# Kyaw-Thiha/animal-vision

Measured on AMD Instinct MI355X. Metric: megapixels/sec per-frame pipeline, higher is better.
Workload: dtype f16

## Files before the change

animal-vision_amd/_lib.py:

```python
from __future__ import annotations

import ctypes
import os

_HERE = os.path.dirname(os.path.abspath(__file__))
LIB_PATH = os.path.join(_HERE, "libavx.so")

AVX_OK = 0
AVX_ERR_INVALID, AVX_ERR_NO_DEVICE, AVX_ERR_HIP, AVX_ERR_UNSUPPORTED, AVX_ERR_NOMEM = -1, -2, -3, -4, -5
AVX_COLOR_MATRIX, AVX_COLOR_CAT_MERGE = 0, 1
AVX_POST_NONE, AVX_POST_GAUSS, AVX_POST_ROWGAIN, AVX_POST_STREAK = 0, 1, 2, 3
AVX_MAX_KSIZE = 33
AVX_PIX_FMTS = {"yuv420p": 0, "nv12": 1, "yuv422p": 2, "yuv444p": 3, "gray": 4, "yuv420p10le": 5, "yuv422p10le": 6, "yuv444p10le": 7,
                "p010le": 8}
AVX_TRANSFERS = {"pq": 1, "hlg": 2}
AVX_TONEMAPS = {"clip": 0, "mobius": 1}


class AvxError(RuntimeError):
    def __init__(self, code: int, msg: str):
        super().__init__(f"libavx error {code}: {msg}")
        self.code = code


# ... 163 lines not shown

class EwPlane(ctypes.Structure):
    _fields_ = [("ptr", ctypes.c_void_p), ("stride", ctypes.c_int32), ("kind", ctypes.c_int32)]


class EwProgram(ctypes.Structure):

    _fields_ = [
        ("struct_size", ctypes.c_uint32),
        ("H", ctypes.c_int32),
        ("W", ctypes.c_int32),
        ("n_insn", ctypes.c_int32),
        ("insn_host", ctypes.POINTER(EwInsn)),
        ("n_planes", ctypes.c_int32),
        ("planes_host", ctypes.POINTER(EwPlane)),
        ("n_acc", ctypes.c_int32),
        ("acc_host", ctypes.POINTER(ctypes.c_int32)),
        ("scalars_dev", ctypes.c_void_p),
        ("n_scalars", ctypes.c_int32),
    ]


AVX_EW_MAX_INSN, AVX_EW_MAX_PLANES, AVX_EW_MAX_REGS, AVX_EW_MAX_ACC = 384, 24, 32, 16
AVX_EW_MAX_FRAMES = 16
_EW_OPS = ("CONST SCALAR LOAD STORE ADD SUB MUL DIV MIN MAX POW ATAN2 NEG ABS SQRT EXP LOG SIN COS FLOOR CEIL CLIP01 TANH "
           "LT LE GT GE EQ AND OR NOT SELECT ACCMIN ACCMAX ACCSUM").split()
EW = {name: i + 1 for i, name in enumerate(_EW_OPS)}
EW_PLANE = {"f32": 0, "u8": 1, "u8_lut": 2, "col": 3, "row": 4, "u8_enc": 5}
EW_ACC = {"min": 0, "max": 1, "sum": 2, "mean": 3}

AVX_MAP = {"falsecolor": 0, "custom_matrix": 1, "opponent": 2, "uv_purple_yellow": 3, "falsecolor_uv_mixed": 4}

if not os.path.exists(LIB_PATH):
    raise ImportError(
        f"{LIB_PATH} not found: build it with `python -c 'import __graft_entry__ as g; g.build()'` "
        "or `make -C animal-vision_amd/csrc` (hipcc --offload-arch=gfx950). There is no CPU fallback."
    )


def _preload_torch_hip_runtime():
    import importlib.util

    try:
        spec = importlib.util.find_spec("torch")
    except (ImportError, ValueError):
        spec = None
    if spec is None or not spec.submodule_search_locations:
        return
    cand = os.path.join(list(spec.submodule_search_locations)[0], "lib", "libamdhip64.so")
    if os.path.exists(cand):
        try:
            ctypes.CDLL(cand, mode=ctypes.RTLD_GLOBAL)
        except OSError:
            pass


_preload_torch_hip_runtime()
lib = ctypes.CDLL(LIB_PATH)

_vp, _i, _sz = ctypes.c_void_p, ctypes.c_int, ctypes.c_size_t
_SIGS = {
    "avx_abi_version": (_i, []),
    "avx_device_count": (_i, []),
    "avx_init": (_i, [_i, ctypes.POINTER(_vp)]),
    "avx_destroy": (None, [_vp]),
    "avx_last_error": (ctypes.c_char_p, [_vp]),
    "avx_malloc": (_i, [_vp, _sz, ctypes.POINTER(_vp)]),
    "avx_free": (_i, [_vp, _vp]),
    "avx_host_alloc": (_i, [_vp, _sz, ctypes.POINTER(_vp)]),
    "avx_host_free": (_i, [_vp, _vp]),
    "avx_memcpy_h2d": (_i, [_vp, _vp, _vp, _sz, _vp]),
    "avx_memcpy_d2h": (_i, [_vp, _vp, _vp, _sz, _vp]),
    "avx_memcpy_d2d": (_i, [_vp, _vp, _vp, _sz, _vp]),
    "avx_memset": (_i, [_vp, _vp, _i, _sz, _vp]),
    "avx_stream_create": (_i, [_vp, ctypes.POINTER(_vp)]),
    "avx_stream_destroy": (_i, [_vp, _vp]),
    "avx_sync": (_i, [_vp, _vp]),
    "avx_stream_wait": (_i, [_vp, _vp, _vp]),
    "avx_device_sync": (_i, [_vp]),
    "avx_timer_start": (_i, [_vp, _vp]),
    "avx_timer_stop": (_i, [_vp, _vp, ctypes.POINTER(ctypes.c_float)]),
    "avx_dichromat_u8": (_i, [_vp, _vp, _vp, _i, _i, _i, ctypes.POINTER(DichromatDesc), _vp]),
    "avx_dichromat_last_launch": (_i, [_vp, ctypes.POINTER(DichromatLaunchInfo)]),
    "avx_get_table": (_i, [_i, _vp, _sz]),
    "avx_percentile": (_i, [_vp, _vp, _sz, ctypes.c_double, ctypes.POINTER(ctypes.c_double), _vp]),
    "avx_spectral_integrate": (_i, [_vp, _vp, _i, _i, _i, _i, _i, _vp, _i, _vp, _vp, _vp]),
    "avx_plane_stats": (_i, [_vp, _vp, _i, _sz, _i, ctypes.c_float, _vp, _vp]),
    "avx_planes_gaussian_blur": (_i, [_vp, _vp, _vp, _i, _i, _i, _i, _vp, _i, _vp]),
    "avx_planes_gaussian_blur_batch": (_i, [_vp, _vp, _sz, _vp, _sz, _i, _i, _i, _i, _i, _vp, _i, _vp]),
    "avx_streak_planes_f32": (_i, [_vp, _vp, _vp, _i, _i, _vp, _i, _vp]),
    "avx_rgb_to_hsi_lobes": (_i, [_vp, _vp, _i, _i, _i, _i, _vp, ctypes.c_float, _vp, _vp]),
    "avx_honeybee_u8": (_i, [_vp, _vp, _vp, _i, _i, _i, ctypes.POINTER(HoneybeeDesc), _vp, _vp]),
    "avx_catch_planes_up": (_i, [_vp, _vp, _i, _i, _vp, _i, _i, _vp, ctypes.POINTER(ctypes.c_int), _vp]),
    "avx_uv_front_u8": (_i, [_vp, _vp, _i, _i, _i, _vp, _vp, _vp]),
    "avx_uv_front_u8_batch": (_i, [_vp, _vp, _i, _sz, _i, _i, _i, _vp, _sz, _vp, _sz, _vp]),
    "avx_panorama_warp_f32": (_i, [_vp, _vp, _i, _i, _i, _vp, _vp]),
    "avx_band_stack": (_i, [_vp, _vp, _i, _i, ctypes.POINTER(BandStackDesc), _vp, _vp]),
    "avx_band_stack_batch": (_i, [_vp, _vp, _i, _sz, _i, _i, ctypes.POINTER(BandStackDesc), _vp, _sz, _vp]),
    "avx_percentile_dev": (_i, [_vp, _vp, _sz, ctypes.c_double, _vp, _vp]),
    "avx_percentiles_dev": (_i, [_vp, _i, ctypes.POINTER(ctypes.c_void_p), ctypes.POINTER(ctypes.c_size_t), ctypes.POINTER(ctypes.c_double),
                                 ctypes.POINTER(ctypes.c_void_p), _vp]),
    "avx_ew_run": (_i, [_vp, ctypes.POINTER(EwProgram), _vp]),
    "avx_ew_run_batch": (_i, [_vp, ctypes.POINTER(EwProgram), _i, ctypes.POINTER(ctypes.c_size_t), _sz, _vp]),
    "avx_ew_spec_stats": (_i, [ctypes.POINTER(ctypes.c_ulonglong), ctypes.POINTER(ctypes.c_ulonglong)]),
    "avx_mantis_u8": (_i, [_vp, _vp, _vp, _vp, _i, _i, ctypes.POINTER(MantisDesc), _vp]),
    "avx_mantis_u8_batch": (_i, [_vp, _vp, _vp, _vp, _i, _i, _i, ctypes.POINTER(MantisDesc), _vp]),
    "avx_resize_hwc": (_i, [_vp, _vp, _i, _i, _i, _i, _vp, _i, _i, _i, _vp]),
    "avx_binocular_warp_u8": (_i, [_vp, _vp, _i, _i, _vp, _vp, _vp, _vp, _vp, _i, _i, _vp, _vp]),
    "avx_cat_wide_u8": (_i, [_vp, _vp, _vp, _i, _i, _i, ctypes.POINTER(DichromatDesc), _vp, _vp, _vp, _vp, _vp, _vp]),
    "avx_center_zoom_u8": (_i, [_vp, _vp, _vp, _i, _i, _i, _i, _i, _i, _i, _vp]),
    "avx_split_compose_u8": (_i, [_vp, _vp, _vp, _vp, _i, _i, _i, _vp]),
    "avx_draw_label_u8": (_i, [_vp, _vp, _i, _i, ctypes.POINTER(ctypes.c_int), _fp, _i, ctypes.c_float, ctypes.c_float, _i, _vp]),
    "avx_gallery_compose_u8": (_i, [_vp, ctypes.POINTER(GalleryTile), _i, _fp, _i, _i, _i, _i, ctypes.POINTER(ctypes.c_int), _vp, _i, _i, _vp]),
    "avx_wall_max_tiles": (_i, []),
    "avx_wall_layout_create": (_i, [_vp, _i, _i, _i, _i, _i, ctypes.POINTER(ctypes.c_int), ctypes.POINTER(ctypes.c_int), _fp, _i, _i, _i, _i,
                                    ctypes.POINTER(ctypes.c_int), ctypes.POINTER(_vp)]),
    "avx_wall_layout_destroy": (_i, [_vp, _vp]),
    "avx_wall_canvas_size": (_i, [_vp, ctypes.POINTER(_i), ctypes.POINTER(_i)]),
    "avx_wall_layout_info": (_i, [_vp, ctypes.POINTER(_i), ctypes.POINTER(_i), ctypes.POINTER(_i), ctypes.POINTER(_sz)]),
    "avx_wall_compose_u8": (_i, [_vp, _vp, ctypes.POINTER(_vp), _sz, _i, _vp, _sz, _vp]),
    "avx_i420_to_rgb_u8": (_i, [_vp, _vp, _vp, _i, _i, _i, _i, _i, _vp]),
    "avx_rgb_to_i420_u8": (_i, [_vp, _vp, _vp, _i, _i, _i, _i, _i, _vp]),
    "avx_yuv_coefficients": (_i, [_i, _i, ctypes.POINTER(ctypes.c_int), ctypes.POINTER(ctypes.c_int)]),
    "avx_yuv_coefficients_d": (_i, [_i, _i, _i, ctypes.POINTER(ctypes.c_int), ctypes.POINTER(ctypes.c_int)]),
    "avx_yuv_frame_size": (_sz, [_i, _i, _i]),
    "avx_yuv_to_rgb_u8": (_i, [_vp, _i, _vp, _vp, _i, _i, _i, _i, _i, _vp]),
    "avx_rgb_to_yuv_u8": (_i, [_vp, _i, _vp, _vp, _i, _i, _i, _i, _i, _vp]),
    "avx_yuv_hdr_to_rgb_u8": (_i, [_vp, _i, _vp, _vp, _i, _i, _i, _i, _i, _i, ctypes.c_double, ctypes.c_double, _vp]),
    "avx_yuv_to_rgb_scaled_u8": (_i, [_vp, _i, _vp, _vp, _i, _i, _i, _i, _i, _i, _i, _vp]),
    "avx_yuv_hdr_to_rgb_scaled_u8": (_i, [_vp, _i, _vp, _vp, _i, _i, _i, _i, _i, _i, _i, _i, ctypes.c_double, ctypes.c_double, _vp]),
    "avx_frame_metrics_u8": (_i, [_vp, _vp, _vp, _i, _i, _i, _i, _vp, _vp]),
    "avx_plane_metrics": (_i, [_vp, _i, _vp, _i, _vp, _i, _i, _i, _i, _vp, _vp]),
    "avx_frame_metrics_ms_u8": (_i, [_vp, _vp, _vp, _i, _i, _i, _vp, _vp, _vp]),
    "avx_remap_linear_planes": (_i, [_vp, _vp, _i, _i, _i, _vp, _vp, _vp, ctypes.c_float, _vp]),
    "avx_sobel3_plane": (_i, [_vp, _vp, _i, _i, _vp, _vp, _vp]),
    "avx_mst_gram": (_i, [_vp, _vp, _i, _sz, _i, _i, _vp, _vp, _vp, _vp]),
    "avx_mst_qkv_gram": (_i, [_vp, _vp, _vp, _sz, _i, _vp, _vp, _vp, _vp, _vp]),
    "avx_mst_qkv_gram16": (_i, [_vp, _vp, _vp, _sz, _i, _vp, _vp, _vp, _vp, _vp]),
    "avx_mst_ln_gemm_gelu": (_i, [_vp, _vp, _vp, _vp, ctypes.c_float, _vp, _sz, _i, _vp, _vp]),
    "avx_mst_convt2x2": (_i, [_vp, _vp, _vp, _vp, _vp, _i, _i, _i, _i, _vp]),
    "avx_mst_convt2x2_fuse": (_i, [_vp, _vp, _vp, _vp, _vp, _vp, _vp, _i, _i, _i, _i, _vp]),
    "avx_mst_posemb": (_i, [_vp, _vp, _vp, _vp, _vp, _vp, _vp, _i, _i, _i, _i, _vp]),
    "avx_mst_conv3x3_add": (_i, [_vp, _vp, _vp, _vp, _vp, _i, _i, _i, _i, _vp]),
    "avx_mst_attn_pack": (_i, [_vp, _vp, _vp, _vp, _vp, _vp, _i, _vp, _vp]),
    "avx_mst_rowgemm_add": (_i, [_vp, _vp, _vp, _vp, _vp, _vp, _vp, _sz, _i, _vp]),
    "avx_mst_conv_in_u8": (_i, [_vp, _vp, _i, _i, _i, _i, _i, _i, _vp, _vp, _vp]),
    "avx_mst_conv3x3_lds": (_i, [_vp, _vp, _vp, _vp, _vp, _i, _i, _i, _i, _vp]),
    "avx_mst_down4x4": (_i, [_vp, _vp, _vp, _vp, _i, _i, _i, _i, _vp]),
    "avx_mst_conv3x3_lds_gram": (_i, [_vp, _vp, _vp, _vp, _vp, _i, _i, _i, _vp, _vp, _vp, _vp, _vp]),
    "avx_mst_convt2x2_fuse_gram": (_i, [_vp, _vp, _vp, _vp, _vp, _vp, _vp, _i, _i, _i, _vp, _vp, _vp, _vp, _vp]),
    "avx_mst_attn_pack16": (_i, [_vp, _vp, _vp, _vp, _vp, _vp, _i, _vp, _vp]),
    "avx_mst_attn_pack_mx": (_i, [_vp, _vp, _vp, _vp, _vp, _vp, _i, _vp, _vp]),
    "avx_mst_attn_tail_mx": (_i, [_vp, _vp, _vp, _vp, _vp, _vp, _vp, _vp, _i, _i, _i, _i, _vp]),
    "avx_mst_attn_tail": (_i, [_vp, _vp, _vp, _vp, _vp, _vp, _vp, _vp, _i, _i, _i, _i, _vp]),
    "avx_mst_attn_tail_x": (_i, [_vp, _vp, _vp, _vp, _vp, _vp, _vp, _vp, _i, _i, _i, _i, _vp]),
    "avx_mst_ffn_fused": (_i, [_vp, _vp, _vp, _vp, ctypes.c_float, _vp, _vp, _vp, _vp, _i, _i, _i, _i, _vp]),
    "avx_mst_conv3x3_lds_spectral": (_i, [_vp, _vp, _vp, _vp, _i, _i, _i, _fp, _i, _i, _i, _i, _vp, _vp, ctypes.POINTER(ctypes.c_int), _vp]),
    "avx_mst_ffn_fused_mx": (_i, [_vp, _vp, _vp, _vp, ctypes.c_float, _vp, _vp, _vp, _vp, _i, _i, _i, _i, _vp]),
    "avx_mst_gelu_prescale": (ctypes.c_float, []),
    "avx_mst_tile_order": (_i, [_i, _i, _i, _i, _i, ctypes.POINTER(ctypes.c_longlong), _i, ctypes.POINTER(ctypes.c_int)]),
    "avx_mst_dw_gemm_add": (_i, [_vp, _vp, _vp, _vp, _vp, _vp, _i, _i, _i, _i, _vp]),
    "avx_dwconv3x3_nhwc_add": (_i, [_vp, _vp, _vp, _vp, _i, _i, _i, _i, _i, _vp, _vp, _vp]),
    "avx_dwconv3x3_nhwc": (_i, [_vp, _vp, _vp, _vp, _i, _i, _i, _i, _i, _i, _vp]),
    "avx_layernorm_rows": (_i, [_vp, _vp, _vp, _vp, _vp, _i, _sz, _i, ctypes.c_float, _vp]),
    "avx_layernorm_rows_grouped": (_i, [_vp, _vp, _vp, _vp, _vp, _i, _sz, _i, ctypes.c_float, _i, _i, _vp]),
}
for _name, (_res, _args) in _SIGS.items():
    _fn = getattr(lib, _name)
    _fn.restype = _res
    _fn.argtypes = _args

if lib.avx_abi_version() != 1:
    raise ImportError(f"libavx.so ABI {lib.avx_abi_version()} != 1 expected by this package: rebuild")
```

animal-vision_amd/csrc/mst_fused.hip:

```cpp
#include <hip/hip_fp16.h>

#include <cstdio>
#include <cstdlib>
#include <cstring>

#include "avx_internal.h"
#include "mst_common.h"
#include "mst_tile_order.h"

namespace {

typedef float float4_t __attribute__((ext_vector_type(4)));
#ifndef AVX_FFN32_GM2
#define AVX_FFN32_GM2 1
#endif
constexpr int kFT = 512;
constexpr int TS = 16;
constexpr int HS = TS + 2;
#ifndef AVX_FFN_TH
#define AVX_FFN_TH 16
#endif
constexpr int kFfnTH = AVX_FFN_TH;
static_assert(kFfnTH == 14 || kFfnTH == 16, "FeedForward tile rows");
constexpr int kFfnNGRP = (HS * (kFfnTH + 2) + 31) / 32;

__device__ __forceinline__ float16_t mfma16(half8_t a, half8_t b, float16_t c) { return __builtin_amdgcn_mfma_f32_32x32x16_f16(a, b, c, 0, 0, 0); }

struct Tile { int x0, y0; long b; };
__device__ __forceinline__ Tile tile_at(const TileWalk& wk, int side_x, int side_y) { return Tile{wk.xi * side_x, wk.yi * side_y, (long)wk.b}; }
int mst_tile_order() {
    const char* e = getenv("AVX_MST_TILE_ORDER");
    return e && !strcmp(e, "raster") ? AVX_TILE_ORDER_RASTER : AVX_TILE_ORDER_XCD;
}

template <int C, int HPASS, int MINW, bool DWM, bool STAMP = false, int NW = 8>
__global__ __launch_bounds__(64 * NW, MINW) void k_mst_ffn_fused(const __half* __restrict__ x , const float* __restrict__ gamma, const float* __restrict__ beta,
                                                          float eps, const uint4* __restrict__ w1pack , const __half* __restrict__ taps ,
                                                          const uint4* __restrict__ w2pack , __half* __restrict__ out , int B,
                                                          int H, int W, const uint4* __restrict__ dwpack , unsigned long long* __restrict__ stamps , int order ) {
    constexpr int FTH = kFfnTH, HSY = FTH + 2, NHALO = HS * HSY, NGRP = (NHALO + 31) / 32;
    constexpr int HID = 4 * C, NPASS = HID / HPASS, KS1 = C / 16, KS2 = HPASS / 16, NT = C / 32, YPITCH = C * 2 + 16, LNV = C / 16;
    constexpr int HPITCH = HPASS * 2 + 16, RPITCH = (HS * HPITCH + 255) / 256 * 256 , NCT = HPASS / 32;
    static_assert(C == 32 || C == 64 || C == 128, "31-, 62- or 124-channel blocks (stored 32 / 64 / 128 wide)");
    constexpr int NTHR = 64 * NW, NGW = (NGRP + NW - 1) / NW;
    constexpr int NTW = NT / (NW / 8), NOCTW = HPASS / (8 * NW);
    static_assert((NW == 8 || NW == 16) && NT % (NW / 8) == 0 && (!DWM || HPASS % (8 * NW) == 0) && (DWM || NW == 8), "wave split");
    constexpr bool PREFETCH = C <= 64;
    extern __shared__ __align__(16) unsigned char smem[];
    unsigned char* yt = smem;
    unsigned char* ht = yt + (size_t)NGRP * 32 * YPITCH;
    __half* tapl = reinterpret_cast<__half*>(ht + (size_t)HSY * RPITCH);
    float* gl = reinterpret_cast<float*>(tapl + (DWM ? 0 : 9 * HID));
    constexpr bool W2LDS = NW == 16;
    uint4* w2l = reinterpret_cast<uint4*>(gl + 2 * C);
    const int tid = threadIdx.x, lane = tid & 63, wave = tid >> 6, p = lane & 31, h = lane >> 5;
    unsigned long long seg[8] = {0, 0, 0, 0, 0, 0, 0, 0}, tlast = 0;
    auto stamp = [&](int k) {
        if constexpr (STAMP) {
            const unsigned long long now = __builtin_readcyclecounter();
            seg[k] += now - tlast;
            tlast = now;
        }
    };
    if constexpr (STAMP) tlast = __builtin_readcyclecounter();
    if constexpr (!DWM)
        for (int i = tid; i < 9 * HID; i += NTHR) tapl[i] = taps[i];
    for (int i = tid; i < C; i += NTHR) { gl[i] = gamma[i]; gl[C + i] = beta[i]; }
    const int tx = (W + TS - 1) / TS, ty = (H + FTH - 1) / FTH;
    const float cnt = (float)(NT * 31);

    uint4 raw[NGW][LNV];
    unsigned f_rel[NGW];
#pragma unroll
    for (int gi = 0; gi < NGW; ++gi) {
        const int q = 32 * (wave + NW * gi) + p, qq = q < NHALO ? q : NHALO - 1;
        f_rel[gi] = (unsigned)(((qq / HS) * W + qq % HS) * C + h * (C / 2)) * 2u;
    }
    auto fetch = [&](const Tile& t) {
        if (t.y0 >= 1 && t.y0 + HSY - 1 <= H && t.x0 >= 1 && t.x0 + HS - 1 <= W) {
            const char* origin = reinterpret_cast<const char*>(x + ((t.b * H + t.y0 - 1) * (size_t)W + t.x0 - 1) * C);
#pragma unroll
            for (int gi = 0; gi < NGW; ++gi) {
                if (wave + NW * gi >= NGRP) break;
                unsigned o = f_rel[gi];
                asm volatile("" : "+v"(o));
                const uint4* src = reinterpret_cast<const uint4*>(origin + o);
#pragma unroll
                for (int v = 0; v < LNV; ++v) raw[gi][v] = src[v];
            }
            return;
        }
#pragma unroll
        for (int gi = 0; gi < NGW; ++gi) {
            const int g = wave + NW * gi;
            if (g >= NGRP) break;
            const int q = 32 * g + p, qq = q < NHALO ? q : NHALO - 1;
            int yy = t.y0 - 1 + qq / HS, xx = t.x0 - 1 + qq % HS;
            yy = yy < 0 ? 0 : (yy >= H ? H - 1 : yy);
            xx = xx < 0 ? 0 : (xx >= W ? W - 1 : xx);
            const uint4* src = reinterpret_cast<const uint4*>(x + ((t.b * H + yy) * (size_t)W + xx) * C + h * (C / 2));
#pragma unroll
            for (int v = 0; v < LNV; ++v) raw[gi][v] = src[v];
        }
    };
    auto layernorm = [&]() {
        if constexpr (DWM) {
#pragma unroll
            for (int gi = 0; gi < NGW; ++gi) {
                const int g = wave + NW * gi;
                if (g >= NGRP) break;
                typedef _Float16 half2v __attribute__((ext_vector_type(2)));
                constexpr unsigned kOnes = 0x3c003c00u;
                auto is_pad = [&](int i) { return ((h * (C / 2) + i) & 31) == 31; };
                auto word = [&](int i) { const uint4 u = raw[gi][i / 8]; const int k = (i / 2) & 3; return k == 0 ? u.x : k == 1 ? u.y : k == 2 ? u.z : u.w; };
                float s1 = 0.f;
#pragma unroll
                for (int i = 0; i < 8 * LNV; i += 2) s1 = __builtin_amdgcn_fdot2(__builtin_bit_cast(half2v, word(i)), __builtin_bit_cast(half2v, kOnes), s1, false);
                const float mean = (s1 + __shfl_xor(s1, 32)) / cnt, nmean = -mean;
                float d[8 * LNV], s2 = 0.f;
#pragma unroll
                for (int i = 0; i < 8 * LNV; ++i) {
                    const float t = (i & 1) ? fma_mix_hi_c(word(i), kOnes, nmean) : fma_mix_lo_c(word(i), kOnes, nmean);
                    d[i] = is_pad(i) ? 0.f : t;
                    s2 = __builtin_fmaf(d[i], d[i], s2);
                }
                const float rstd = rsqrtf((s2 + __shfl_xor(s2, 32)) / cnt + eps);
                unsigned char* dst = yt + (size_t)(32 * g + p) * YPITCH + h * C;
#pragma unroll
                for (int v = 0; v < LNV; ++v) {
                    unsigned o[4];
#pragma unroll
                    for (int j = 0; j < 8; j += 2) {
                        const int i = 8 * v + j;
                        const float2_t y2 = float2_t{d[i], d[i + 1]} * float2_t{rstd, rstd};
                        const float bq = (h * (C / 2) + i + 1) == 31 ? 1.0f : y2.y;
                        o[j / 2] = pack_f16(y2.x, bq);
                    }
                    *reinterpret_cast<uint4*>(dst + 16 * v) = uint4{o[0], o[1], o[2], o[3]};
                }
            }
            return;
        }
#pragma unroll
        for (int gi = 0; gi < NGW; ++gi) {
            const int g = wave + NW * gi;
            if (g >= NGRP) break;
            constexpr unsigned kOnes = 0x3c003c00u;
            auto is_pad = [&](int i) { return ((h * (C / 2) + i) & 31) == 31; };
            auto word = [&](int i) { const uint4 u = raw[gi][i / 8]; const int k = (i / 2) & 3; return k == 0 ? u.x : k == 1 ? u.y : k == 2 ? u.z : u.w; };
            float s1 = 0.f;
#pragma unroll
            for (int i = 0; i < 8 * LNV; ++i) {
                const float t = (i & 1) ? fma_mix_hi_c(word(i), kOnes, s1) : fma_mix_lo_c(word(i), kOnes, s1);
                s1 = is_pad(i) ? s1 : t;
            }
            const float mean = (s1 + __shfl_xor(s1, 32)) / cnt, nmean = -mean;
            float d[8 * LNV], s2 = 0.f;
#pragma unroll
            for (int i = 0; i < 8 * LNV; ++i) {
                const float t = (i & 1) ? fma_mix_hi_c(word(i), kOnes, nmean) : fma_mix_lo_c(word(i), kOnes, nmean);
                d[i] = is_pad(i) ? 0.f : t;
                s2 = __builtin_fmaf(d[i], d[i], s2);
            }
            const float rstd = rsqrtf((s2 + __shfl_xor(s2, 32)) / cnt + eps);
            unsigned char* dst = yt + (size_t)(32 * g + p) * YPITCH + h * C;
#pragma unroll
            for (int v = 0; v < LNV; ++v) {
                unsigned o[4];
#pragma unroll
                for (int j = 0; j < 8; j += 2) {
                    const int i = 8 * v + j, c = h * (C / 2) + i;
                    const float a = is_pad(i) ? 0.f : __builtin_fmaf(d[i] * rstd, gl[c], gl[C + c]);
                    const float bq = is_pad(i + 1) ? 0.f : __builtin_fmaf(d[i + 1] * rstd, gl[c + 1], gl[C + c + 1]);
                    o[j / 2] = pack_f16(a, bq);
                }
                *reinterpret_cast<uint4*>(dst + 16 * v) = uint4{o[0], o[1], o[2], o[3]};
            }
        }
    };

    const int n0 = (wave / 8) * NTW, w8 = wave % 8;
    half8_t w2f[W2LDS ? 1 : NTW * KS2];
    auto load_w2 = [&](int pass) {
#pragma unroll
        for (int n = 0; n < NTW; ++n)
#pragma unroll
            for (int s = 0; s < KS2; ++s) w2f[n * KS2 + s] = __builtin_bit_cast(half8_t, w2pack[((size_t)(n0 + n) * (HID / 16) + pass * KS2 + s) * 64 + lane]);
    };
    if constexpr (NPASS == 1 && !W2LDS) load_w2(0);
    half8_t w1f[KS1];
    auto load_w1 = [&](int pass) {
#pragma unroll
        for (int s = 0; s < KS1; ++s) w1f[s] = __builtin_bit_cast(half8_t, w1pack[((size_t)(pass * NCT + wave % NCT) * KS1 + s) * 64 + lane]);
    };
    constexpr bool W1AHEAD = DWM && C == 64 && NPASS > 1 && NW == 8;
    if constexpr (W1AHEAD) load_w1(0);
    constexpr int NITEM = (NGRP + NW / NCT - 1) / (NW / NCT);
    int p1_g[NITEM], p1_dst[NITEM], p1_dy[NITEM], p1_dx[NITEM];
#pragma unroll
    for (int j = 0; j < NITEM; ++j) {
        const int g = wave / NCT + j * (NW / NCT), q = 32 * g + p, qc = q < NHALO ? q : 0;
        p1_g[j] = g < NGRP ? g : -1;
        p1_dst[j] = (g < NGRP && q < NHALO) ? (qc / HS) * RPITCH + (qc % HS) * HPITCH + 32 * h : -1;
        p1_dy[j] = qc / HS - 1; p1_dx[j] = qc % HS - 1;
    }
    TileWalk ahead;
    ahead.init(blockIdx.x, gridDim.x, B, ty, tx, order);
    if (!ahead.live) return;
    Tile t = tile_at(ahead, TS, FTH);
    ahead.advance();
    fetch(t);
    __syncthreads();
    layernorm();
    for (;;) {
        const bool halo_inside = t.y0 >= 1 && t.y0 + HSY - 1 <= H && t.x0 >= 1 && t.x0 + HS - 1 <= W;
        float16_t D[NTW];
#pragma unroll
        for (int n = 0; n < NTW; ++n)
#pragma unroll
            for (int v = 0; v < 16; ++v) D[n][v] = 0.f;
#pragma unroll 1
        for (int pass = 0; pass < NPASS; ++pass) {
            stamp(pass == 0 ? 7 : 5);
            __syncthreads();
            stamp(0);
            if constexpr (W2LDS)
                for (int i = tid; i < NT * KS2 * 64; i += NTHR) w2l[i] = w2pack[((size_t)(i / (KS2 * 64)) * (HID / 16) + pass * KS2 + (i / 64) % KS2) * 64 + (i & 63)];
            half8_t af[DWM ? NOCTW : 1][3];
            if constexpr (DWM) {
#pragma unroll
                for (int o2 = 0; o2 < NOCTW; ++o2)
#pragma unroll
                    for (int i = 0; i < 3; ++i) af[o2][i] = __builtin_bit_cast(half8_t, dwpack[((size_t)(pass * (HPASS / 8) + NW * o2 + wave) * 3 + i) * 64 + lane]);
            }
            {
                const int ct = wave % NCT;
                if constexpr (!W1AHEAD) load_w1(pass);
#pragma unroll
                for (int j = 0; j < NITEM; ++j) {
                    if (p1_g[j] < 0) continue;
                    float16_t d;
#pragma unroll
                    for (int v = 0; v < 16; ++v) d[v] = 0.f;
                    const unsigned char* ysrc = yt + (size_t)(32 * p1_g[j] + p) * YPITCH + 16 * h;
#pragma unroll
                    for (int s = 0; s < KS1; ++s) d = mfma16(w1f[s], __builtin_bit_cast(half8_t, *reinterpret_cast<const uint4*>(ysrc + 32 * s)), d);
                    if (p1_dst[j] >= 0) {
                        uint32_t keep = 0xffffffffu;
                        if (!halo_inside) {
                            const int yy = t.y0 + p1_dy[j], xx = t.x0 + p1_dx[j];
                            keep = (yy >= 0 && yy < H && xx >= 0 && xx < W) ? 0xffffffffu : 0u;
                        }
                        constexpr int GP1 = (C == 64 && NW == 8) ? 4 : (C == 32 ? 2 : 1);
                        unsigned pk[8];
#pragma unroll
                        for (int v0 = 0; v0 < 8; v0 += GP1) {
                            float2_t gq[GP1];
#pragma unroll
                            for (int v = 0; v < GP1; ++v) gq[v] = float2_t{d[2 * (v0 + v)], d[2 * (v0 + v) + 1]};
                            if constexpr (DWM) gelu_mx<GP1>(gq); else gelu_multi<GP1>(gq);
#pragma unroll
                            for (int v = 0; v < GP1; ++v) pk[v0 + v] = pack_f16(gq[v].x, gq[v].y);
                        }
                        uint4 u0 = uint4{pk[0], pk[1], pk[2], pk[3]}, u1 = uint4{pk[4], pk[5], pk[6], pk[7]};
                        if (!halo_inside) { u0.x &= keep; u0.y &= keep; u0.z &= keep; u0.w &= keep; u1.x &= keep; u1.y &= keep; u1.z &= keep; u1.w &= keep; }
                        unsigned char* dst = ht + p1_dst[j] + 64 * ct;
                        reinterpret_cast<uint4*>(dst)[0] = u0;
                        reinterpret_cast<uint4*>(dst)[1] = u1;
                    }
                }
            }
            stamp(1);
            __syncthreads();
            stamp(2);
            if (PREFETCH && pass == NPASS - 1 && ahead.live) fetch(tile_at(ahead, TS, FTH));
            if constexpr (NPASS > 1 && !W2LDS) load_w2(pass);
            if constexpr (DWM) {
                constexpr int NOCT = NOCTW;
                const int n16 = lane & 15, q = lane >> 4;
                unsigned char* rbase = ht + (size_t)q * RPITCH + (size_t)n16 * HPITCH + 16 * wave;
                unsigned char* wbase = ht + (size_t)(q >> 1) * RPITCH + (size_t)n16 * HPITCH + 16 * wave + 8 * (q & 1);
                constexpr int NU = NOCT * (FTH / 2);
                uint4 bq[3];
                auto rd = [&](int u) {
                    const int o2 = u / (FTH / 2), pr = u % (FTH / 2);
#pragma unroll
                    for (int i = 0; i < 3; ++i) bq[i] = *reinterpret_cast<const uint4*>(rbase + (size_t)(2 * pr) * RPITCH + (size_t)i * HPITCH + 16 * NW * o2);
                };
                auto finish = [&](int u, float4_t a) {
                    const int o2 = u / (FTH / 2), pr = u % (FTH / 2);
                    float2_t gp[2] = {float2_t{a[0], a[1]}, float2_t{a[2], a[3]}};
                    if constexpr (C == 64 || (C == 32 && AVX_FFN32_GM2)) gelu_mx<2>(gp);
                    else { float2_t g0[1] = {gp[0]}, g1[1] = {gp[1]}; gelu_mx<1>(g0); gelu_mx<1>(g1); gp[0] = g0[0]; gp[1] = g1[0]; }
                    *reinterpret_cast<uint2*>(wbase + (size_t)(2 * pr) * RPITCH + 16 * NW * o2) = uint2{pack_f16(gp[0].x, gp[0].y), pack_f16(gp[1].x, gp[1].y)};
                };
#ifndef AVX_FFN_PIPE_ALL
#define AVX_FFN_PIPE_ALL 0
#endif
                constexpr bool PIPE = C == 64 || AVX_FFN_PIPE_ALL;
                if constexpr (PIPE) {
                    rd(0);
                    float4_t prev = {0.f, 0.f, 0.f, 0.f};
#pragma unroll
                    for (int u = 0; u < NU; ++u) {
                        const int o2 = u / (FTH / 2);
                        float4_t acc = {0.f, 0.f, 0.f, 0.f};
#pragma unroll
                        for (int i = 0; i < 3; ++i) acc = __builtin_amdgcn_mfma_f32_16x16x32_f16(af[o2][i], __builtin_bit_cast(half8_t, bq[i]), acc, 0, 0, 0);
                        if (u + 1 < NU) rd(u + 1);
                        __builtin_amdgcn_sched_barrier(0);
                        if (u > 0) finish(u - 1, prev);
                        __builtin_amdgcn_sched_barrier(0);
                        prev = acc;
                    }
                    finish(NU - 1, prev);
                } else {
#pragma unroll
                    for (int u = 0; u < NU; ++u) {
                        const int o2 = u / (FTH / 2);
                        rd(u);
                        float4_t acc = {0.f, 0.f, 0.f, 0.f};
#pragma unroll
                        for (int i = 0; i < 3; ++i) acc = __builtin_amdgcn_mfma_f32_16x16x32_f16(af[o2][i], __builtin_bit_cast(half8_t, bq[i]), acc, 0, 0, 0);
                        finish(u, acc);
                    }
                }
                stamp(3);
                __syncthreads();
                stamp(4);
                if constexpr (W1AHEAD) load_w1(pass + 1 < NPASS ? pass + 1 : 0);
                const int r = 2 * w8 + (p >> 4), c = p & 15;
                const unsigned char* zb = ht + (size_t)r * RPITCH + (size_t)c * HPITCH + 16 * h;
                if (2 * w8 < FTH) {
#pragma unroll
                for (int s = 0; s < KS2; ++s) {
                    const half8_t bf = __builtin_bit_cast(half8_t, *reinterpret_cast<const uint4*>(zb + 32 * s));
#pragma unroll
                    for (int n = 0; n < NTW; ++n) {
                        if constexpr (W2LDS) D[n] = mfma16(__builtin_bit_cast(half8_t, w2l[((n0 + n) * KS2 + s) * 64 + lane]), bf, D[n]);
                        else D[n] = mfma16(w2f[n * KS2 + s], bf, D[n]);
                    }
                }
                }
            } else
            if (2 * wave < FTH) {
                const int r = 2 * wave + (p >> 4), c = p & 15;
                const unsigned char* hbase = ht + (size_t)r * RPITCH + (size_t)c * HPITCH + 16 * h;
                const unsigned char* tbase = reinterpret_cast<const unsigned char*>(tapl) + (size_t)(pass * HPASS + 8 * h) * 2;
#pragma unroll
                for (int s = 0; s < KS2; ++s) {
                    float acc[8];
#pragma unroll
                    for (int j = 0; j < 8; ++j) acc[j] = 0.f;
#pragma unroll
                    for (int tap = 0; tap < 9; ++tap) {
                        const uint4 hv = *reinterpret_cast<const uint4*>(hbase + (size_t)(tap / 3) * RPITCH + (size_t)(tap % 3) * HPITCH + 32 * s);
                        const uint4 wv = *reinterpret_cast<const uint4*>(tbase + (size_t)tap * HID * 2 + 32 * s);
                        fma_mix_lo(acc[0], hv.x, wv.x); fma_mix_hi(acc[1], hv.x, wv.x);
                        fma_mix_lo(acc[2], hv.y, wv.y); fma_mix_hi(acc[3], hv.y, wv.y);
                        fma_mix_lo(acc[4], hv.z, wv.z); fma_mix_hi(acc[5], hv.z, wv.z);
                        fma_mix_lo(acc[6], hv.w, wv.w); fma_mix_hi(acc[7], hv.w, wv.w);
                    }
                    half8_t bf;
#pragma unroll
                    for (int j = 0; j < 8; j += 2) {
                        const float2_t gv = gelu_fast2(float2_t{acc[j], acc[j + 1]});
                        bf[j] = (_Float16)gv.x;
                        bf[j + 1] = (_Float16)gv.y;
                    }
#pragma unroll
                    for (int n = 0; n < NT; ++n)
                        D[n] = mfma16(w2f[n * KS2 + s], bf, D[n]);
                }
            }
        }
        stamp(5);
        {
            const int yo = t.y0 + 2 * w8 + (p >> 4), xo = t.x0 + (p & 15);
            if (2 * w8 < FTH && yo < H && xo < W) {
                const size_t off = ((t.b * H + yo) * (size_t)W + xo) * C + 16 * h + 32 * n0;
#pragma unroll
                for (int n = 0; n < NTW; ++n) {
                    const uint4 xa = reinterpret_cast<const uint4*>(x + off + 32 * n)[0], xb = reinterpret_cast<const uint4*>(x + off + 32 * n)[1];
                    const unsigned xw[8] = {xa.x, xa.y, xa.z, xa.w, xb.x, xb.y, xb.z, xb.w};
                    unsigned ow[8];
#pragma unroll
                    for (int j = 0; j < 8; ++j) {
                        float s0 = D[n][2 * j], s1 = D[n][2 * j + 1];
                        fma_mix_lo(s0, xw[j], 0x3c003c00u); fma_mix_hi(s1, xw[j], 0x3c003c00u);
                        ow[j] = pack_f16(s0, s1);
                    }
                    reinterpret_cast<uint4*>(out + off + 32 * n)[0] = uint4{ow[0], ow[1], ow[2], ow[3]};
                    reinterpret_cast<uint4*>(out + off + 32 * n)[1] = uint4{ow[4], ow[5], ow[6], ow[7]};
                }
            }
        }
        stamp(6);
        if (!ahead.live) break;
        t = tile_at(ahead, TS, FTH);
        ahead.advance();
        if (!PREFETCH) fetch(t);
        layernorm();
    }
    if constexpr (STAMP) {
        if (lane == 0 && stamps)
#pragma unroll
            for (int k = 0; k < 8; ++k) stamps[((size_t)blockIdx.x * NW + wave) * 8 + k] = seg[k];
    }
}


constexpr int VS = TS + 4, MS = TS + 2;

template <int C, int MINW>
__global__ __launch_bounds__(kFT, MINW) void k_mst_attn_tail(const __half* __restrict__ v , const __half* __restrict__ x ,
                                                             const uint4* __restrict__ mpack , const __half* __restrict__ taps1 ,
                                                             const __half* __restrict__ taps2 , const float* __restrict__ bias ,
                                                             __half* __restrict__ out, int B, int H, int W, const uint4* __restrict__ wvpack ) {
    constexpr int NO = C / 8, NS = C / 16, NT = C / 32, PP = C * 2 + 16;
    constexpr int VRP = (VS * PP + 255) / 256 * 256, MRP = VRP;
    constexpr int NFILL = (VS * VS * NO + kFT - 1) / kFT;
    extern __shared__ __align__(16) unsigned char smem[];
    unsigned char* vt = smem;
    unsigned char* mt = vt + (size_t)VS * VRP;
    const bool fromx = wvpack != nullptr;
    __half* t2l = reinterpret_cast<__half*>(mt + (size_t)VS * VRP);
    __half* t1l = t2l + 9 * C;
    float* bl = reinterpret_cast<float*>(t1l + 9 * C);
    const int tid = threadIdx.x, lane = tid & 63, wave = tid >> 6, p = lane & 31, h = lane >> 5;
    for (int i = tid; i < 9 * C; i += kFT) { t2l[i] = taps2[i]; t1l[i] = taps1[i]; }
    for (int i = tid; i < C; i += kFT) bl[i] = bias ? bias[i] : 0.f;
    const int tx = (W + TS - 1) / TS, ty = (H + TS - 1) / TS;
    const int oct = wave % NO, part = wave / NO, nparts = 8 / NO, per = (MS * MS + nparts - 1) / nparts;
    half8_t mf[NT * NS];
#pragma unroll
    for (int i = 0; i < NT * NS; ++i) mf[i] = __builtin_bit_cast(half8_t, mpack[(size_t)i * 64 + lane]);

    uint4 pre[NFILL];
    int f_lds[NFILL];
    unsigned f_rel[NFILL];
#pragma unroll
    for (int k = 0; k < NFILL; ++k) {
        const int it = tid + k * kFT, itc = it < VS * VS * NO ? it : 0, q = itc / NO, part16 = itc % NO;
        f_lds[k] = it < VS * VS * NO ? (q / VS) * VRP + (q % VS) * PP + 16 * part16 : -1;
        f_rel[k] = (unsigned)(((q / VS) * W + q % VS) * C + 8 * part16) * 2u;
    }
    auto fetch = [&](const Tile& t) {
        const __half* src = fromx ? x : v;
        if (t.y0 >= 2 && t.y0 + VS - 2 <= H && t.x0 >= 2 && t.x0 + VS - 2 <= W) {
            const char* origin = reinterpret_cast<const char*>(src + ((t.b * H + t.y0 - 2) * (size_t)W + t.x0 - 2) * C);
#pragma unroll
            for (int k = 0; k < NFILL; ++k) {
                unsigned o = f_rel[k];
                asm volatile("" : "+v"(o));
                pre[k] = *reinterpret_cast<const uint4*>(origin + o);
            }
            return;
        }
#pragma unroll
        for (int k = 0; k < NFILL; ++k) {
            const int fl = f_lds[k] < 0 ? 0 : f_lds[k], row = fl / VRP, col = (fl - row * VRP) / PP, f_off = (fl - row * VRP - col * PP) / 2;
            const int yy = t.y0 + row - 2, xx = t.x0 + col - 2;
            const bool ok = f_lds[k] >= 0 && yy >= 0 && yy < H && xx >= 0 && xx < W;
            const int yc = yy < 0 ? 0 : (yy >= H ? H - 1 : yy), xc = xx < 0 ? 0 : (xx >= W ? W - 1 : xx);
            uint4 r = *reinterpret_cast<const uint4*>(src + ((t.b * H + yc) * (size_t)W + xc) * C + f_off);
            r.x = ok ? r.x : 0u; r.y = ok ? r.y : 0u; r.z = ok ? r.z : 0u; r.w = ok ? r.w : 0u;
            pre[k] = r;
        }
    };
    auto fill = [&]() {
        unsigned char* dst = fromx ? mt : vt;
#pragma unroll
        for (int k = 0; k < NFILL; ++k)
            if (f_lds[k] >= 0) *reinterpret_cast<uint4*>(dst + f_lds[k]) = pre[k];
    };
    constexpr int NB = (((MS * MS + (8 / NO) - 1) / (8 / NO)) + 63) / 64;
// ... 12 lines not shown
    ahead.advance();
    fetch(t);
    for (;;) {
        fill();
        __syncthreads();
        if (fromx) {
            constexpr int NG = (VS * VS + 31) / 32;
            for (int task = wave; task < NG * NT; task += kFT / 64) {
                const int g = task / NT, nt = task % NT;
                const int q = 32 * g + p, qc = q < VS * VS ? q : VS * VS - 1;
                const int lo = (qc / VS) * VRP + (qc % VS) * PP;
                float16_t d;
#pragma unroll
                for (int vv = 0; vv < 16; ++vv) d[vv] = 0.f;
#pragma unroll
                for (int s2 = 0; s2 < NS; ++s2)
                    d = mfma16(__builtin_bit_cast(half8_t, wvpack[(size_t)(nt * NS + s2) * 64 + lane]),
                               __builtin_bit_cast(half8_t, *reinterpret_cast<const uint4*>(mt + lo + 32 * s2 + 16 * h)), d);
                if (q < VS * VS) {
                    half8_t o0, o1;
#pragma unroll
                    for (int vv = 0; vv < 8; ++vv) { o0[vv] = (_Float16)d[vv]; o1[vv] = (_Float16)d[8 + vv]; }
                    reinterpret_cast<uint4*>(vt + lo + 64 * nt + 32 * h)[0] = __builtin_bit_cast(uint4, o0);
                    reinterpret_cast<uint4*>(vt + lo + 64 * nt + 32 * h)[1] = __builtin_bit_cast(uint4, o1);
                }
            }
            __syncthreads();
        }
        constexpr bool HOIST = C == 64;
        uint4 wt1[HOIST ? 9 : 1];
        if constexpr (HOIST) {
#pragma unroll
            for (int tap = 0; tap < 9; ++tap) wt1[tap] = *reinterpret_cast<const uint4*>(reinterpret_cast<const unsigned char*>(t1l) + (size_t)tap * C * 2 + 16 * oct);
        }
        const bool mid_inside = t.y0 >= 1 && t.y0 + MS - 1 <= H && t.x0 >= 1 && t.x0 + MS - 1 <= W;
#pragma unroll
        for (int i = 0; i < NB; ++i) {
            if (b_src[i] < 0) continue;
            const unsigned char* src = vt + b_src[i];
            float acc[8];
#pragma unroll
            for (int j = 0; j < 8; ++j) acc[j] = 0.f;
#pragma unroll
            for (int tap = 0; tap < 9; ++tap) {
                const uint4 hv = *reinterpret_cast<const uint4*>(src + (tap / 3) * VRP + (tap % 3) * PP);
                const uint4 wv = HOIST ? wt1[HOIST ? tap : 0] : *reinterpret_cast<const uint4*>(reinterpret_cast<const unsigned char*>(t1l) + (size_t)tap * C * 2 + 16 * oct);
                fma_mix_lo(acc[0], hv.x, wv.x); fma_mix_hi(acc[1], hv.x, wv.x);
                fma_mix_lo(acc[2], hv.y, wv.y); fma_mix_hi(acc[3], hv.y, wv.y);
                fma_mix_lo(acc[4], hv.z, wv.z); fma_mix_hi(acc[5], hv.z, wv.z);
                fma_mix_lo(acc[6], hv.w, wv.w); fma_mix_hi(acc[7], hv.w, wv.w);
            }
            bool inside = true;
            if (!mid_inside) {
                const int my = b_src[i] / MRP, mx = (b_src[i] - my * MRP) / PP, yy = t.y0 + my - 1, xx = t.x0 + mx - 1;
                inside = yy >= 0 && yy < H && xx >= 0 && xx < W;
            }
            half8_t o;
#pragma unroll
            for (int j = 0; j < 8; j += 2) {
                const float2_t gv = gelu_fast2(float2_t{acc[j], acc[j + 1]});
                o[j] = (_Float16)gv.x;
                o[j + 1] = (_Float16)gv.y;
            }
            uint4 ov = __builtin_bit_cast(uint4, o);
            if (!mid_inside) {
                const uint32_t keep = inside ? 0xffffffffu : 0u;
                ov.x &= keep; ov.y &= keep; ov.z &= keep; ov.w &= keep;
            }
            *reinterpret_cast<uint4*>(mt + b_src[i]) = ov;
        }
        __syncthreads();
        if (ahead.live) fetch(tile_at(ahead, TS, TS));
        {
            const int r = 2 * wave + (p >> 4), c = p & 15;
            const int yo = t.y0 + r, xo = t.x0 + c;
            const bool live = yo < H && xo < W;
            const size_t off = ((t.b * H + (live ? yo : 0)) * (size_t)W + (live ? xo : 0)) * C + h * (C / 2);
            uint4 xr[2 * NT];
#pragma unroll
            for (int i = 0; i < 2 * NT; ++i) xr[i] = reinterpret_cast<const uint4*>(x + off)[i];
            float16_t D[NT];
#pragma unroll
            for (int n = 0; n < NT; ++n)
#pragma unroll
                for (int vv = 0; vv < 16; ++vv) D[n][vv] = 0.f;
            float pe[NS][8];
            const unsigned char* msrc = mt + (size_t)r * MRP + (size_t)c * PP + (size_t)h * C;
            const unsigned char* vsrc = vt + (size_t)(r + 2) * VRP + (size_t)(c + 2) * PP + (size_t)h * C;
            const unsigned char* tsrc = reinterpret_cast<const unsigned char*>(t2l) + (size_t)h * C;
#pragma unroll
            for (int s = 0; s < NS; ++s) {
#pragma unroll
                for (int j = 0; j < 8; ++j) pe[s][j] = 0.f;
#pragma unroll
                for (int tap = 0; tap < 9; ++tap) {
                    const uint4 hv = *reinterpret_cast<const uint4*>(msrc + (size_t)(tap / 3) * MRP + (size_t)(tap % 3) * PP + 16 * s);
                    const uint4 wv = *reinterpret_cast<const uint4*>(tsrc + (size_t)tap * C * 2 + 16 * s);
                    fma_mix_lo(pe[s][0], hv.x, wv.x); fma_mix_hi(pe[s][1], hv.x, wv.x);
                    fma_mix_lo(pe[s][2], hv.y, wv.y); fma_mix_hi(pe[s][3], hv.y, wv.y);
                    fma_mix_lo(pe[s][4], hv.z, wv.z); fma_mix_hi(pe[s][5], hv.z, wv.z);
                    fma_mix_lo(pe[s][6], hv.w, wv.w); fma_mix_hi(pe[s][7], hv.w, wv.w);
                }
                const half8_t bv = __builtin_bit_cast(half8_t, *reinterpret_cast<const uint4*>(vsrc + 16 * s));
#pragma unroll
                for (int n = 0; n < NT; ++n) D[n] = mfma16(mf[n * NS + s], bv, D[n]);
            }
            if (live) {
#pragma unroll
                for (int n = 0; n < NT; ++n) {
                    const float* bb = bl + h * (C / 2) + 16 * n;
                    constexpr unsigned kOnes = 0x3c003c00u;
                    const uint4 xa = xr[2 * n], xb = xr[2 * n + 1];
                    const unsigned xw[8] = {xa.x, xa.y, xa.z, xa.w, xb.x, xb.y, xb.z, xb.w};
                    unsigned ow[8];
#pragma unroll
                    for (int j = 0; j < 8; ++j) {
                        const float* pj = j < 4 ? &pe[2 * n][2 * j] : &pe[2 * n + 1][2 * j - 8];
                        const unsigned pk = pack_f16(pj[0], pj[1]);
                        float s0 = D[n][2 * j], s1 = D[n][2 * j + 1];
                        fma_mix_lo(s0, pk, kOnes); fma_mix_hi(s1, pk, kOnes);
                        s0 += bb[2 * j]; s1 += bb[2 * j + 1];
                        fma_mix_lo(s0, xw[j], kOnes); fma_mix_hi(s1, xw[j], kOnes);
                        ow[j] = pack_f16(s0, s1);
                    }
                    reinterpret_cast<uint4*>(out + off)[2 * n] = uint4{ow[0], ow[1], ow[2], ow[3]};
                    reinterpret_cast<uint4*>(out + off)[2 * n + 1] = uint4{ow[4], ow[5], ow[6], ow[7]};
                }
            }
        }
        if (!ahead.live) break;
        t = tile_at(ahead, TS, TS);
        ahead.advance();
        __syncthreads();
    }
}

template <int C, int MINW>
int launch_attn_tail(avx_ctx* ctx, const void* v, const void* x, const void* mpack, const void* taps1, const void* taps2, const float* bias, void* out, int B,
                     int H, int W, hipStream_t s, const void* wvpack) {
    constexpr int PP = C * 2 + 16, VRP = (VS * PP + 255) / 256 * 256, MRP = VRP;
    const size_t lds = (size_t)2 * VS * VRP + (size_t)2 * 9 * C * 2 + sizeof(float) * C;
    (void)MRP;
    const long total = (long)B * ((H + TS - 1) / TS) * ((W + TS - 1) / TS);
    const long cap = (long)ctx->num_cus * (MINW / 2);
    auto k = k_mst_attn_tail<C, MINW>;
    AVX_HIP(ctx, hipFuncSetAttribute((const void*)k, hipFuncAttributeMaxDynamicSharedMemorySize, (int)lds));
    hipLaunchKernelGGL(k, dim3((unsigned)(total < cap ? total : cap)), dim3(kFT), lds, s, (const __half*)v, (const __half*)x, (const uint4*)mpack,
                       (const __half*)taps1, (const __half*)taps2, bias, (__half*)out, B, H, W, (const uint4*)wvpack);
    AVX_HIP(ctx, hipGetLastError());
    return AVX_OK;
}


template <int C, int TR, int MINW, bool STAMP = false, int NW = 8>
__global__ __launch_bounds__(64 * NW, MINW) void k_mst_attn_tail_mx(const __half* __restrict__ x , const uint4* __restrict__ wvpack ,
                                                                const uint4* __restrict__ mpack , const uint4* __restrict__ dw1 ,
                                                                const uint4* __restrict__ dw2 , const float* __restrict__ bias ,
                                                                __half* __restrict__ out, int B, int H, int W, unsigned long long* __restrict__ stamps , int order ) {
    constexpr int TW = 14, VW = 18, VR = TR + 4, MR = TR + 2, NOCT = C / 8, NK = C / 16, NT = C / 32, NS = C / 16, LNV = C / 16;
    constexpr int PP = C * 2 + 16, RP = (VW * PP + 255) / 256 * 256, MP = 16 * PP;
    constexpr int NTHR = 64 * NW, NG = (VR * VW + 31) / 32, NGW = (NG + NW - 1) / NW;
    constexpr int WPO = NOCT >= NW ? 1 : NW / NOCT, OPW = NOCT > NW ? NOCT / NW : 1;
    constexpr int NOUT = (TR / 2) / WPO, NMID = NOUT + 1;
    static_assert(C == 32 || C == 64 || C == 128, "31-, 62- or 124-channel blocks");
    static_assert(MP % 256 == 0 && (NW % NOCT == 0 || NOCT % NW == 0) && (TR / 2) % WPO == 0, "pitches / row split");
    extern __shared__ __align__(16) unsigned char smem[];
    unsigned char* vt = smem;
    unsigned char* mt = vt + (size_t)VR * RP;
    uint4* wvl = reinterpret_cast<uint4*>(mt + (size_t)MR * MP);
    constexpr bool STASH = C <= 64 && NW == 8;
    unsigned char* xs = reinterpret_cast<unsigned char*>(wvl + NT * NS * 64);
    const int tid = threadIdx.x, lane = tid & 63, wave = tid >> 6, p = lane & 31, h = lane >> 5, n16 = lane & 15, q = lane >> 4;
    unsigned long long seg[8] = {0, 0, 0, 0, 0, 0, 0, 0}, tlast = 0;
    auto stamp = [&](int kk) {
        if constexpr (STAMP) {
            const unsigned long long now = __builtin_readcyclecounter();
            seg[kk] += now - tlast;
            tlast = now;
        }
    };
    if constexpr (STAMP) tlast = __builtin_readcyclecounter();
    const int tx = (W + TW - 1) / TW, ty = (H + TR - 1) / TR;
    for (int i = tid; i < NT * NS * 64; i += NTHR) wvl[i] = wvpack[i];
    const int o = wave % NOCT, rpo = (wave / NOCT) * NOUT;
    half8_t a1[3], a2[3], am[NK];
    float bs[4];
    auto load_frags = [&](int oc) {
#pragma unroll
        for (int i = 0; i < 3; ++i) {
            a1[i] = __builtin_bit_cast(half8_t, dw1[((size_t)oc * 3 + i) * 64 + lane]);
            a2[i] = __builtin_bit_cast(half8_t, dw2[((size_t)oc * 3 + i) * 64 + lane]);
        }
#pragma unroll
        for (int t2 = 0; t2 < NK; ++t2) am[t2] = __builtin_bit_cast(half8_t, mpack[((size_t)oc * NK + t2) * 64 + lane]);
#pragma unroll
        for (int j = 0; j < 4; ++j) bs[j] = bias ? bias[8 * oc + 4 * (q & 1) + j] : 0.f;
    };
    load_frags(o);
#pragma unroll
    for (int i = 0; i < 3; ++i) asm volatile("" ::"v"(a1[i]), "v"(a2[i]));
#pragma unroll
    for (int t2 = 0; t2 < NK; ++t2) asm volatile("" ::"v"(am[t2]));
    asm volatile("" ::"v"(bs[0]), "v"(bs[1]), "v"(bs[2]), "v"(bs[3]));
    const unsigned char* rbB = vt + (size_t)q * RP + (size_t)n16 * PP + 16 * o;
    unsigned char* wbB = mt + (size_t)(q >> 1) * MP + (size_t)n16 * PP + 16 * o + 8 * (q & 1);
    const unsigned char* rbC = mt + (size_t)q * MP + (size_t)n16 * PP + 16 * o;
    const unsigned char* rbG = vt + (size_t)(2 + (q & 1)) * RP + (size_t)(n16 + 2) * PP + 16 * (q >> 1);
    unsigned f_rel[NGW];
    int v_dst[NGW], p_row[NGW], p_col[NGW];
#pragma unroll
    for (int gi = 0; gi < NGW; ++gi) {
        const int g = wave + NW * gi, qq = 32 * g + p, qc = qq < VR * VW ? qq : VR * VW - 1;
        p_row[gi] = qc / VW; p_col[gi] = qc % VW;
        f_rel[gi] = (unsigned)((p_row[gi] * W + p_col[gi]) * C + h * (C / 2)) * 2u;
        v_dst[gi] = (g < NG && qq < VR * VW) ? p_row[gi] * RP + p_col[gi] * PP + 32 * h : -1;
    }
    uint4 pre[NGW][LNV];
    auto fetch = [&](const Tile& t) {
        if (t.y0 >= 2 && t.y0 + VR - 2 <= H && t.x0 >= 2 && t.x0 + VW - 2 <= W) {
            const char* origin = reinterpret_cast<const char*>(x + ((t.b * H + t.y0 - 2) * (size_t)W + t.x0 - 2) * C);
#pragma unroll
            for (int gi = 0; gi < NGW; ++gi) {
                if (wave + NW * gi >= NG) break;
                unsigned of = f_rel[gi];
                asm volatile("" : "+v"(of));
                const uint4* src = reinterpret_cast<const uint4*>(origin + of);
#pragma unroll
                for (int v = 0; v < LNV; ++v) pre[gi][v] = src[v];
            }
            return;
        }
#pragma unroll
        for (int gi = 0; gi < NGW; ++gi) {
            if (wave + NW * gi >= NG) break;
            const int yy = t.y0 - 2 + p_row[gi], xx = t.x0 - 2 + p_col[gi];
            const bool ok = yy >= 0 && yy < H && xx >= 0 && xx < W;
            const int yc = yy < 0 ? 0 : (yy >= H ? H - 1 : yy), xc = xx < 0 ? 0 : (xx >= W ? W - 1 : xx);
            const uint4* src = reinterpret_cast<const uint4*>(x + ((t.b * H + yc) * (size_t)W + xc) * C + h * (C / 2));
#pragma unroll
            for (int v = 0; v < LNV; ++v) {
                uint4 r = src[v];
                r.x = ok ? r.x : 0u; r.y = ok ? r.y : 0u; r.z = ok ? r.z : 0u; r.w = ok ? r.w : 0u;
                pre[gi][v] = r;
            }
        }
    };
    TileWalk ahead;
    ahead.init(blockIdx.x, gridDim.x, B, ty, tx, order);
    if (!ahead.live) return;
    Tile t = tile_at(ahead, TW, TR);
    ahead.advance();
    fetch(t);
    __syncthreads();
    for (;;) {
#pragma unroll
        for (int gi = 0; gi < NGW; ++gi) {
            if (wave + NW * gi >= NG) break;
#pragma unroll
            for (int nt = 0; nt < NT; ++nt) {
                float16_t d;
#pragma unroll
                for (int vv = 0; vv < 16; ++vv) d[vv] = 0.f;
#pragma unroll
                for (int s2 = 0; s2 < NS; ++s2) d = mfma16(__builtin_bit_cast(half8_t, wvl[(nt * NS + s2) * 64 + lane]), __builtin_bit_cast(half8_t, pre[gi][s2]), d);
                if (v_dst[gi] >= 0) {
                    half8_t w0, w1;
#pragma unroll
                    for (int vv = 0; vv < 8; ++vv) { w0[vv] = (_Float16)d[vv]; w1[vv] = (_Float16)d[8 + vv]; }
                    reinterpret_cast<uint4*>(vt + v_dst[gi] + 64 * nt)[0] = __builtin_bit_cast(uint4, w0);
                    reinterpret_cast<uint4*>(vt + v_dst[gi] + 64 * nt)[1] = __builtin_bit_cast(uint4, w1);
                }
            }
            if constexpr (STASH) {
                const unsigned sr = (unsigned)(p_row[gi] - 2), sc = (unsigned)(p_col[gi] - 2);
                if (v_dst[gi] >= 0 && sr < (unsigned)TR && sc < (unsigned)TW) {
                    unsigned char* dst = xs + (sr * TW + sc) * PP + h * C;
#pragma unroll
                    for (int v = 0; v < LNV; ++v) *reinterpret_cast<uint4*>(dst + 16 * v) = pre[gi][v];
                }
            }
        }
        stamp(0);
        __syncthreads();
        stamp(1);
        if (ahead.live) fetch(tile_at(ahead, TW, TR));
#pragma unroll
        for (int kk = 0; kk < OPW; ++kk) {
        const int oc = o + NW * kk, ob = 16 * NW * kk;
        if constexpr (OPW > 1) load_frags(oc);
        uint2 xr[STASH ? 1 : NOUT];
        const int yo0 = t.y0 + 2 * rpo + (q >> 1), xo = t.x0 + n16;
        const bool livex = n16 < TW && xo < W;
        const size_t e0 = ((t.b * H + (yo0 < H ? yo0 : 0)) * (size_t)W + (livex ? xo : 0)) * C + 8 * oc + 4 * (q & 1), estep = (size_t)2 * W * C;
        auto live = [&](int u) { return livex && yo0 + 2 * u < H; };
        if constexpr (!STASH) {
#pragma unroll
            for (int u = 0; u < NOUT; ++u) xr[u] = live(u) ? *reinterpret_cast<const uint2*>(x + e0 + u * estep) : uint2{0, 0};
        }
        {
            const bool mid_inside = t.y0 >= 1 && t.y0 + MR - 1 <= H && t.x0 >= 1 && t.x0 + 15 <= W;
            uint4 bq[3];
            auto rd = [&](int u) {
#pragma unroll
                for (int i = 0; i < 3; ++i) bq[i] = *reinterpret_cast<const uint4*>(rbB + (size_t)(2 * (rpo + u)) * RP + i * PP + ob);
            };
            auto finish = [&](int u, float4_t a) {
                float2_t gp[2] = {float2_t{a[0], a[1]}, float2_t{a[2], a[3]}};
                if constexpr (C >= 64) gelu_mx<2>(gp);
                else { float2_t g0[1] = {gp[0]}, g1[1] = {gp[1]}; gelu_mx<1>(g0); gelu_mx<1>(g1); gp[0] = g0[0]; gp[1] = g1[0]; }
                uint2 ov = uint2{pack_f16(gp[0].x, gp[0].y), pack_f16(gp[1].x, gp[1].y)};
                if (!mid_inside) {
                    const int yy = t.y0 - 1 + 2 * (rpo + u) + (q >> 1), xx = t.x0 - 1 + n16;
                    const unsigned keep = (yy >= 0 && yy < H && xx >= 0 && xx < W) ? 0xffffffffu : 0u;
                    ov.x &= keep; ov.y &= keep;
                }
                *reinterpret_cast<uint2*>(wbB + (size_t)(2 * (rpo + u)) * MP + ob) = ov;
            };
            rd(0);
            float4_t prev = {0.f, 0.f, 0.f, 0.f};
#pragma unroll
            for (int u = 0; u < NMID; ++u) {
                float4_t acc = {0.f, 0.f, 0.f, 0.f};
#pragma unroll
                for (int i = 0; i < 3; ++i) acc = __builtin_amdgcn_mfma_f32_16x16x32_f16(a1[i], __builtin_bit_cast(half8_t, bq[i]), acc, 0, 0, 0);
                if (u + 1 < NMID) rd(u + 1);
                __builtin_amdgcn_sched_barrier(0);
                if (u > 0) finish(u - 1, prev);
                __builtin_amdgcn_sched_barrier(0);
                prev = acc;
            }
            finish(NMID - 1, prev);
        }
        stamp(2);
        {
            uint4 bq[3], bg[NK];
            uint2 xn = uint2{0, 0};
            const unsigned char* rbX = xs + (size_t)((q >> 1) * TW + n16) * PP + 16 * o + 8 * (q & 1);
            auto rd = [&](int u) {
#pragma unroll
                for (int i = 0; i < 3; ++i) bq[i] = *reinterpret_cast<const uint4*>(rbC + (size_t)(2 * (rpo + u)) * MP + i * PP + ob);
#pragma unroll
                for (int t2 = 0; t2 < NK; ++t2) bg[t2] = *reinterpret_cast<const uint4*>(rbG + (size_t)(2 * (rpo + u)) * RP + 32 * t2);
                if constexpr (STASH) xn = *reinterpret_cast<const uint2*>(rbX + (size_t)(2 * (rpo + u)) * TW * PP);
            };
            auto finish = [&](int u, float4_t acc, uint2 xu) {
                if (live(u)) {
                    constexpr unsigned kOnes = 0x3c003c00u;
                    float s0 = acc[0] + bs[0], s1 = acc[1] + bs[1], s2 = acc[2] + bs[2], s3 = acc[3] + bs[3];
                    fma_mix_lo(s0, xu.x, kOnes); fma_mix_hi(s1, xu.x, kOnes);
                    fma_mix_lo(s2, xu.y, kOnes); fma_mix_hi(s3, xu.y, kOnes);
                    *reinterpret_cast<uint2*>(out + e0 + u * estep) = uint2{pack_f16(s0, s1), pack_f16(s2, s3)};
                }
            };
            rd(0);
#ifndef AVX_TAIL_PIPE2
#define AVX_TAIL_PIPE2 1
#endif
            if constexpr (STASH && (AVX_TAIL_PIPE2 == 2 || (AVX_TAIL_PIPE2 == 1 && C == 64))) {
                float4_t prev = {0.f, 0.f, 0.f, 0.f};
                uint2 xp = uint2{0, 0};
#pragma unroll
                for (int u = 0; u < NOUT; ++u) {
                    const uint2 xu = xn;
                    float4_t acc = {0.f, 0.f, 0.f, 0.f};
#pragma unroll
                    for (int i = 0; i < 3; ++i) acc = __builtin_amdgcn_mfma_f32_16x16x32_f16(a2[i], __builtin_bit_cast(half8_t, bq[i]), acc, 0, 0, 0);
#pragma unroll
                    for (int t2 = 0; t2 < NK; ++t2) acc = __builtin_amdgcn_mfma_f32_16x16x32_f16(am[t2], __builtin_bit_cast(half8_t, bg[t2]), acc, 0, 0, 0);
                    if (u + 1 < NOUT) rd(u + 1);
                    __builtin_amdgcn_sched_barrier(0);
                    if (u > 0) finish(u - 1, prev, xp);
                    __builtin_amdgcn_sched_barrier(0);
                    prev = acc; xp = xu;
                }
                finish(NOUT - 1, prev, xp);
            } else {
#pragma unroll
                for (int u = 0; u < NOUT; ++u) {
                    const uint2 xu = STASH ? xn : xr[STASH ? 0 : u];
                    float4_t acc = {0.f, 0.f, 0.f, 0.f};
#pragma unroll
                    for (int i = 0; i < 3; ++i) acc = __builtin_amdgcn_mfma_f32_16x16x32_f16(a2[i], __builtin_bit_cast(half8_t, bq[i]), acc, 0, 0, 0);
#pragma unroll
                    for (int t2 = 0; t2 < NK; ++t2) acc = __builtin_amdgcn_mfma_f32_16x16x32_f16(am[t2], __builtin_bit_cast(half8_t, bg[t2]), acc, 0, 0, 0);
                    if (u + 1 < NOUT) rd(u + 1);
                    finish(u, acc, xu);
                }
            }
        }
        }
        stamp(3);
        if (!ahead.live) break;
        t = tile_at(ahead, TW, TR);
        ahead.advance();
        __syncthreads();
        stamp(4);
    }
    if constexpr (STAMP) {
        if (lane == 0 && stamps)
#pragma unroll
            for (int kk = 0; kk < 8; ++kk) stamps[((size_t)blockIdx.x * NW + wave) * 8 + kk] = seg[kk];
    }
}

template <int C, int TR, int MINW, int NW = 8>
int launch_attn_tail_mx(avx_ctx* ctx, const void* x, const void* wvpack, const void* mpack, const void* dw1, const void* dw2, const float* bias, void* out, int B, int H, int W,
                        hipStream_t s) {
    constexpr int PP = C * 2 + 16, RP = (18 * PP + 255) / 256 * 256;
    const size_t lds = (size_t)(TR + 4) * RP + (size_t)(TR + 2) * 16 * PP + (size_t)(C / 32) * (C / 16) * 1024 + ((C <= 64 && NW == 8) ? (size_t)(TR * 14 + 2) * PP : 0) ;
    const long total = (long)B * ((H + TR - 1) / TR) * ((W + 13) / 14);
    const long cap = (long)ctx->num_cus * (NW == 16 ? 1 : MINW / 2);
    AVX_REQUIRE(ctx, total <= 0x7fffffffl, "avx_mst_attn_tail_mx: 2^31 tiles or more");
    const unsigned blocks = (unsigned)(total < cap ? total : cap);
    if (getenv("AVX_TAIL_STAMPS")) {
        auto ks = k_mst_attn_tail_mx<C, TR, MINW, true, NW>;
        unsigned long long* d_st = nullptr;
        const size_t n = (size_t)blocks * NW * 8;
        AVX_HIP(ctx, hipMalloc((void**)&d_st, n * sizeof(unsigned long long)));
        AVX_HIP(ctx, hipFuncSetAttribute((const void*)ks, hipFuncAttributeMaxDynamicSharedMemorySize, (int)lds));
        hipLaunchKernelGGL(ks, dim3(blocks), dim3(64 * NW), lds, s, (const __half*)x, (const uint4*)wvpack, (const uint4*)mpack, (const uint4*)dw1, (const uint4*)dw2, bias, (__half*)out, B, H, W, d_st, mst_tile_order());
        AVX_HIP(ctx, hipStreamSynchronize(s));
        unsigned long long* h_st = (unsigned long long*)malloc(n * sizeof(unsigned long long));
        AVX_HIP(ctx, hipMemcpy(h_st, d_st, n * sizeof(unsigned long long), hipMemcpyDeviceToHost));
        double tot[8] = {0}, all = 0;
        for (size_t i = 0; i < n; ++i) { tot[i & 7] += (double)h_st[i]; all += (double)h_st[i]; }
        const char* nm[8] = {"v from x", "bar1", "conv1+gelu", "conv2+proj+store", "bar2", "-", "-", "-"};
        fprintf(stderr, "[tail stamps C=%d] %u blocks, %ld tiles, mean cycles per wave %.0f:", C, blocks, total, all / (blocks * (double)NW));
        for (int k2 = 0; k2 < 8; ++k2) fprintf(stderr, "  %s %.1f%%", nm[k2], 100 * tot[k2] / all);
        fprintf(stderr, "\n");
        free(h_st);
        (void)hipFree(d_st);
        return AVX_OK;
    }
    auto k = k_mst_attn_tail_mx<C, TR, MINW, false, NW>;
    AVX_HIP(ctx, hipFuncSetAttribute((const void*)k, hipFuncAttributeMaxDynamicSharedMemorySize, (int)lds));
    hipLaunchKernelGGL(k, dim3(blocks), dim3(64 * NW), lds, s, (const __half*)x, (const uint4*)wvpack, (const uint4*)mpack, (const uint4*)dw1,
                       (const uint4*)dw2, bias, (__half*)out, B, H, W, (unsigned long long*)nullptr, mst_tile_order());
    AVX_HIP(ctx, hipGetLastError());
    return AVX_OK;
}


struct SpecStat3 { float mn, mx; double sum; };
template <int MINW, bool GRAM, bool SPEC = false>
__global__ __launch_bounds__(kFT, MINW) void k_mst_conv3x3_lds(const __half* __restrict__ x , const uint4* __restrict__ wpack ,
                                                               const __half* __restrict__ add , __half* __restrict__ out, int B, int H, int W,
                                                               const uint4* __restrict__ wqk , float* __restrict__ partial ,
                                                               const float* __restrict__ specw = nullptr ,
                                                               float* __restrict__ planes = nullptr , SpecStat3* __restrict__ spart = nullptr ,
                                                               int crop_t = 0, int crop_l = 0, int Hc = 0, int Wc = 0, int order = AVX_TILE_ORDER_RASTER ) {
    constexpr int C = 32, PP = C * 2 + 16, RP = (HS * PP + 255) / 256 * 256, NFILL = (HS * HS * 4 + kFT - 1) / kFT;
    __shared__ __align__(16) unsigned char xt[HS * RP];
    __shared__ uint4 wl[18 * 64];
    const int tid = threadIdx.x, lane = tid & 63, wave = tid >> 6, p = lane & 31, h = lane >> 5;
    for (int i = tid; i < 18 * 64; i += kFT) wl[i] = wpack[i];
    __shared__ uint4 wq[GRAM ? 4 * 64 : 1];
    float16_t G;
    float nq = 0.f, nk = 0.f;
    if constexpr (GRAM) {
        if (tid < 4 * 64) wq[tid] = wqk[tid];
#pragma unroll
        for (int v = 0; v < 16; ++v) G[v] = 0.f;
    }
    float smn[3] = {3.4e38f, 3.4e38f, 3.4e38f}, smx[3] = {-3.4e38f, -3.4e38f, -3.4e38f};
    double ssum[3] = {0.0, 0.0, 0.0};
    const int tx = (W + TS - 1) / TS, ty = (H + TS - 1) / TS;
    uint4 pre[NFILL];
    unsigned f_rel[NFILL];
#pragma unroll
    for (int k = 0; k < NFILL; ++k) {
        const int it = tid + k * kFT, itc = it < HS * HS * 4 ? it : 0, q = itc >> 2, part = itc & 3;
        f_rel[k] = (unsigned)(((q / HS) * W + q % HS) * C + 8 * part) * 2u;
    }
    auto fetch = [&](const Tile& t) {
        if (t.y0 >= 1 && t.y0 + HS - 1 <= H && t.x0 >= 1 && t.x0 + HS - 1 <= W) {
            const char* origin = reinterpret_cast<const char*>(x + ((t.b * H + t.y0 - 1) * (size_t)W + t.x0 - 1) * C);
#pragma unroll
            for (int k = 0; k < NFILL; ++k) {
                unsigned o = f_rel[k];
                asm volatile("" : "+v"(o));
                pre[k] = *reinterpret_cast<const uint4*>(origin + o);
            }
            return;
        }
#pragma unroll
        for (int k = 0; k < NFILL; ++k) {
            const int it = tid + k * kFT, q = it >> 2, part = it & 3;
            const int yy = t.y0 - 1 + q / HS, xx = t.x0 - 1 + q % HS;
            const bool ok = it < HS * HS * 4 && yy >= 0 && yy < H && xx >= 0 && xx < W;
            const int yc = yy < 0 ? 0 : (yy >= H ? H - 1 : yy), xc = xx < 0 ? 0 : (xx >= W ? W - 1 : xx);
            uint4 r = *reinterpret_cast<const uint4*>(x + ((t.b * H + yc) * (size_t)W + xc) * C + 8 * part);
            r.x = ok ? r.x : 0u; r.y = ok ? r.y : 0u; r.z = ok ? r.z : 0u; r.w = ok ? r.w : 0u;
            pre[k] = r;
        }
    };
    TileWalk ahead;
    ahead.init(blockIdx.x, gridDim.x, B, ty, tx, (GRAM || SPEC) ? (int)AVX_TILE_ORDER_RASTER : order);
    if (!ahead.live) return;
    Tile t = tile_at(ahead, TS, TS);
    ahead.advance();
    fetch(t);
    for (;;) {
#pragma unroll
        for (int k = 0; k < NFILL; ++k) {
            const int it = tid + k * kFT, q = it >> 2, part = it & 3;
            if (it < HS * HS * 4) *reinterpret_cast<uint4*>(xt + (size_t)(q / HS) * RP + (size_t)(q % HS) * PP + 16 * part) = pre[k];
        }
        __syncthreads();
        if (ahead.live) fetch(tile_at(ahead, TS, TS));
        {
            const int r = 2 * wave + (p >> 4), c = p & 15;
            const int yo = t.y0 + r, xo = t.x0 + c;
            const bool live = yo < H && xo < W;
            const size_t off = ((t.b * H + (live ? yo : 0)) * (size_t)W + (live ? xo : 0)) * C + 16 * h;
            uint4 ar[2] = {uint4{0, 0, 0, 0}, uint4{0, 0, 0, 0}};
            if (add) { ar[0] = reinterpret_cast<const uint4*>(add + off)[0]; ar[1] = reinterpret_cast<const uint4*>(add + off)[1]; }
            float16_t d;
#pragma unroll
            for (int v = 0; v < 16; ++v) d[v] = 0.f;
            const unsigned char* src = xt + (size_t)r * RP + (size_t)c * PP + 16 * h;
#pragma unroll
            for (int tap = 0; tap < 9; ++tap)
#pragma unroll
                for (int s2 = 0; s2 < 2; ++s2)
                    d = mfma16(__builtin_bit_cast(half8_t, wl[(2 * tap + s2) * 64 + lane]), __builtin_bit_cast(half8_t, *reinterpret_cast<const uint4*>(src + (size_t)(tap / 3) * RP + (size_t)(tap % 3) * PP + 32 * s2)), d);
            half8_t o0, o1;
            {
                const half8_t r0 = __builtin_bit_cast(half8_t, ar[0]), r1 = __builtin_bit_cast(half8_t, ar[1]);
#pragma unroll
                for (int v = 0; v < 8; ++v) { o0[v] = (_Float16)(d[v] + (float)r0[v]); o1[v] = (_Float16)(d[8 + v] + (float)r1[v]); }
            }
            if constexpr (SPEC) {
                float a3[3] = {0.f, 0.f, 0.f};
                auto chain = [&]() {
#pragma unroll
                    for (int j = 0; j < 16; ++j) {
                        const float v = (float)(j < 8 ? o0[j] : o1[j - 8]);
                        const float* wb = specw + (16 * h + j) * 4;
#pragma unroll
                        for (int k = 0; k < 3; ++k) a3[k] = __builtin_fmaf(v, wb[k], a3[k]);
                    }
                };
                if (h == 0) chain();
#pragma unroll
                for (int k = 0; k < 3; ++k) { const float lo = __shfl_xor(a3[k], 32); a3[k] = h ? lo : a3[k]; }
                if (h == 1) chain();
                const int yc = yo - crop_t, xc = xo - crop_l;
                if (h == 1 && live && yc >= 0 && yc < Hc && xc >= 0 && xc < Wc) {
#pragma unroll
                    for (int k = 0; k < 3; ++k) {
                        planes[(size_t)k * Hc * Wc + (size_t)yc * Wc + xc] = a3[k];
                        smn[k] = fminf(smn[k], a3[k]); smx[k] = fmaxf(smx[k], a3[k]); ssum[k] += (double)a3[k];
                    }
                }
            } else if (live) {
                reinterpret_cast<uint4*>(out + off)[0] = __builtin_bit_cast(uint4, o0);
                reinterpret_cast<uint4*>(out + off)[1] = __builtin_bit_cast(uint4, o1);
            }
            if constexpr (GRAM) {
                if (!live) { o0 = half8_t{0, 0, 0, 0, 0, 0, 0, 0}; o1 = o0; }
                float16_t dq, dk;
#pragma unroll
                for (int v = 0; v < 16; ++v) { dq[v] = 0.f; dk[v] = 0.f; }
                dq = mfma16(o0, __builtin_bit_cast(half8_t, wq[0 * 64 + lane]), dq);
                dq = mfma16(o1, __builtin_bit_cast(half8_t, wq[1 * 64 + lane]), dq);
                dk = mfma16(o0, __builtin_bit_cast(half8_t, wq[2 * 64 + lane]), dk);
                dk = mfma16(o1, __builtin_bit_cast(half8_t, wq[3 * 64 + lane]), dk);
                unsigned aq[8], ak[8];
#pragma unroll
                for (int j = 0; j < 8; ++j) {
                    aq[j] = pack_f16(dq[2 * j], dq[2 * j + 1]);
                    ak[j] = pack_f16(dk[2 * j], dk[2 * j + 1]);
                    fma_mix_lo(nq, aq[j], aq[j]); fma_mix_hi(nq, aq[j], aq[j]);
                    fma_mix_lo(nk, ak[j], ak[j]); fma_mix_hi(nk, ak[j], ak[j]);
                }
#pragma unroll
                for (int b2 = 0; b2 < 2; ++b2)
                    G = mfma16(__builtin_bit_cast(half8_t, uint4{ak[4 * b2], ak[4 * b2 + 1], ak[4 * b2 + 2], ak[4 * b2 + 3]}),
                               __builtin_bit_cast(half8_t, uint4{aq[4 * b2], aq[4 * b2 + 1], aq[4 * b2 + 2], aq[4 * b2 + 3]}), G);
            }
        }
        if (!ahead.live) break;
        t = tile_at(ahead, TS, TS);
        ahead.advance();
        __syncthreads();
    }
    if constexpr (SPEC) {
// ... 149 lines not shown
            };
            constexpr int AHEAD = 6;
            uint4 bq[AHEAD];
#pragma unroll
            for (int i = 0; i < AHEAD; ++i) bq[i] = frag(i);
#pragma unroll
            for (int i = 0; i < 32; ++i) {
                if (i & 1) d1 = mfma16(wf[i], __builtin_bit_cast(half8_t, bq[i % AHEAD]), d1);
                else d = mfma16(wf[i], __builtin_bit_cast(half8_t, bq[i % AHEAD]), d);
                if (i + AHEAD < 32) bq[i % AHEAD] = frag(i + AHEAD);
            }
            __builtin_amdgcn_sched_group_barrier(0x100, AHEAD, 0);
#pragma unroll
            for (int i = 0; i < 32; ++i) {
                __builtin_amdgcn_sched_group_barrier(0x008, 1, 0);
                if (i + AHEAD < 32) __builtin_amdgcn_sched_group_barrier(0x100, 1, 0);
            }
#pragma unroll
            for (int v = 0; v < 16; ++v) d[v] += d1[v];
            if constexpr (C == 64) {
                float4* part = reinterpret_cast<float4*>(lds + G::NBUF * G::BUF + ((g & 1) * 4 + nt) * 4096);
                if (kh == 1) {
#pragma unroll
                    for (int v4 = 0; v4 < 4; ++v4) part[v4 * 64 + lane] = float4{d[4 * v4], d[4 * v4 + 1], d[4 * v4 + 2], d[4 * v4 + 3]};
                }
                __syncthreads();
                if (kh == 1) continue;
#pragma unroll
                for (int v4 = 0; v4 < 4; ++v4) {
                    const float4 q = part[v4 * 64 + lane];
                    d[4 * v4] += q.x; d[4 * v4 + 1] += q.y; d[4 * v4 + 2] += q.z; d[4 * v4 + 3] += q.w;
                }
            }
            const int yo = t.oy0 + r, xo = t.ox0 + (p & 15);
            half8_t o0, o1;
#pragma unroll
            for (int v = 0; v < 8; ++v) { o0[v] = (_Float16)d[v]; o1[v] = (_Float16)d[8 + v]; }
            __half* dst = out + (((size_t)t.b * Ho + yo) * Wo + xo) * CO + 32 * nt + 16 * h;
            if (whole) {
                reinterpret_cast<uint4*>(dst)[0] = __builtin_bit_cast(uint4, o0);
                reinterpret_cast<uint4*>(dst)[1] = __builtin_bit_cast(uint4, o1);
            } else if (yo < Ho && xo < Wo) {
                reinterpret_cast<uint4*>(dst)[0] = __builtin_bit_cast(uint4, o0);
                reinterpret_cast<uint4*>(dst)[1] = __builtin_bit_cast(uint4, o1);
            }
        }
        plain_stores = whole ? (plain_stores < G::NBUF - 1 ? plain_stores + 1 : plain_stores) : 0;
        walk.advance();
        if (!walk.live) break;
        slot = slot + 1 == G::NBUF ? 0 : slot + 1;
    }
    asm volatile("s_waitcnt vmcnt(0)" ::: "memory");
}

__global__ __launch_bounds__(256) void k_mst_conv_in_u8(const uint8_t* __restrict__ frame , const float* __restrict__ w ,
                                                        __half* __restrict__ out , int H, int W, int pt, int pl, int Hp, int Wp) {
    __shared__ __align__(16) float wl[27 * 32];
    for (int i = threadIdx.x; i < 27 * 32; i += 256) wl[i] = w[i];
    __syncthreads();
    const size_t total = (size_t)Hp * Wp;
    for (size_t i = (size_t)blockIdx.x * 256 + threadIdx.x; i < total; i += (size_t)gridDim.x * 256) {
        const int y = (int)(i / Wp), x = (int)(i - (size_t)y * Wp);
        float in[27];
#pragma unroll
        for (int t = 0; t < 9; ++t) {
            const int yy = y + t / 3 - 1, xx = x + t % 3 - 1;
            const bool ok = yy >= 0 && yy < Hp && xx >= 0 && xx < Wp;
            int sy = (ok ? yy : 0) - pt, sx = (ok ? xx : 0) - pl;
            sy = sy < 0 ? -sy : (sy >= H ? 2 * (H - 1) - sy : sy);
            sx = sx < 0 ? -sx : (sx >= W ? 2 * (W - 1) - sx : sx);
            const uint8_t* q = frame + ((size_t)sy * W + sx) * 3;
#pragma unroll
            for (int c = 0; c < 3; ++c) in[3 * t + c] = ok ? (float)(_Float16)((float)q[c] / 255.0f) : 0.f;
        }
        uint4* dst = reinterpret_cast<uint4*>(out + i * 32);
#pragma unroll 1
        for (int v = 0; v < 4; ++v) {
            float acc[8];
#pragma unroll
            for (int j = 0; j < 8; ++j) acc[j] = 0.f;
#pragma unroll
            for (int k = 0; k < 27; ++k) {
                const float4 wa = *reinterpret_cast<const float4*>(wl + k * 32 + 8 * v), wb = *reinterpret_cast<const float4*>(wl + k * 32 + 8 * v + 4);
                acc[0] = __builtin_fmaf(in[k], wa.x, acc[0]); acc[1] = __builtin_fmaf(in[k], wa.y, acc[1]);
                acc[2] = __builtin_fmaf(in[k], wa.z, acc[2]); acc[3] = __builtin_fmaf(in[k], wa.w, acc[3]);
                acc[4] = __builtin_fmaf(in[k], wb.x, acc[4]); acc[5] = __builtin_fmaf(in[k], wb.y, acc[5]);
                acc[6] = __builtin_fmaf(in[k], wb.z, acc[6]); acc[7] = __builtin_fmaf(in[k], wb.w, acc[7]);
            }
            half8_t o8;
#pragma unroll
            for (int j = 0; j < 8; ++j) o8[j] = (_Float16)acc[j];
            dst[v] = __builtin_bit_cast(uint4, o8);
        }
    }
}

__global__ __launch_bounds__(256) void k_mst_conv_in_u8_mfma(const uint8_t* __restrict__ frame , const float* __restrict__ w ,
                                                             __half* __restrict__ out , int H, int W, int pt, int pl, int Hp, int Wp) {
    const int lane = threadIdx.x & 63, p = lane & 31, h = lane >> 5;
    const int col = 16 * ((p % 8) / 4) + 4 * (p / 8) + p % 4;
    const int tap0 = 5 * h, ntap = 5 - h;
    half8_t af[2];
#pragma unroll
    for (int s = 0; s < 2; ++s)
#pragma unroll
        for (int j = 0; j < 8; ++j) {
            const int q = 8 * s + j, k = 3 * tap0 + q;
            af[s][j] = q < 3 * ntap ? (_Float16)w[k * 32 + col] : (_Float16)0.f;
        }
    int dy[5], dx[5];
#pragma unroll
    for (int t = 0; t < 5; ++t) {
        const int tap = tap0 + (t < ntap ? t : 0);
        dy[t] = tap / 3 - 1; dx[t] = tap % 3 - 1;
    }
    const size_t total = (size_t)Hp * Wp, ngroups = (total + 31) / 32;
    const float inv255 = 1.0f / 255.0f;
    for (size_t g = (size_t)blockIdx.x * 4 + (threadIdx.x >> 6); g < ngroups; g += (size_t)gridDim.x * 4) {
        const size_t i = g * 32 + p, ic = i < total ? i : total - 1;
        const int y = (int)(ic / Wp), x = (int)(ic - (size_t)y * Wp);
        float v[16];
        v[15] = 0.f;
#pragma unroll
        for (int t = 0; t < 5; ++t) {
            const int yy = y + dy[t], xx = x + dx[t];
            const bool ok = t < ntap && yy >= 0 && yy < Hp && xx >= 0 && xx < Wp;
            int sy = (ok ? yy : 0) - pt, sx = (ok ? xx : 0) - pl;
            sy = sy < 0 ? -sy : (sy >= H ? 2 * (H - 1) - sy : sy);
            sx = sx < 0 ? -sx : (sx >= W ? 2 * (W - 1) - sx : sx);
            const uint8_t* q = frame + ((size_t)sy * W + sx) * 3;
#pragma unroll
            for (int c = 0; c < 3; ++c) v[3 * t + c] = ok ? (float)q[c] * inv255 : 0.f;
        }
        const half8_t b0 = __builtin_bit_cast(half8_t, uint4{pack_f16(v[0], v[1]), pack_f16(v[2], v[3]), pack_f16(v[4], v[5]), pack_f16(v[6], v[7])});
        const half8_t b1 = __builtin_bit_cast(half8_t, uint4{pack_f16(v[8], v[9]), pack_f16(v[10], v[11]), pack_f16(v[12], v[13]), pack_f16(v[14], v[15])});
        float16_t d;
#pragma unroll
        for (int vv = 0; vv < 16; ++vv) d[vv] = 0.f;
        d = mfma16(af[0], b0, d);
        d = mfma16(af[1], b1, d);
        if (i < total) {
            unsigned o[8];
#pragma unroll
            for (int vv = 0; vv < 8; ++vv) o[vv] = pack_f16(d[2 * vv], d[2 * vv + 1]);
            reinterpret_cast<uint4*>(out + i * 32 + 16 * h)[0] = uint4{o[0], o[1], o[2], o[3]};
            reinterpret_cast<uint4*>(out + i * 32 + 16 * h)[1] = uint4{o[4], o[5], o[6], o[7]};
        }
    }
}

}

static int ffn_fused_launch(avx_ctx* ctx, const void* x, const float* gamma, const float* beta, float eps, const void* w1pack, const void* taps_9xhid, const void* dwpack,
                            const void* w2pack, void* out, int B, int H, int W, int C, void* stream);

extern "C" float avx_mst_gelu_prescale(void) { return kGeluPrescale; }

extern "C" int avx_mst_tile_order(int frames, int ty, int tx, int nwg, int raster, long long* visit, int steps_cap, int* steps_out) {
    if (frames <= 0 || ty <= 0 || tx <= 0 || nwg <= 0 || (visit && steps_cap <= 0) || (long long)frames * ty * tx > 0x7fffffffll) return AVX_ERR_INVALID;
    int most = 0;
    for (int wg = 0; wg < nwg; ++wg) {
        TileWalk wk;
        wk.init((unsigned)wg, (unsigned)nwg, frames, ty, tx, raster ? AVX_TILE_ORDER_RASTER : AVX_TILE_ORDER_XCD);
        int k = 0;
        for (; wk.live; wk.advance(), ++k)
            if (visit && k < steps_cap) visit[(size_t)wg * steps_cap + k] = ((long long)wk.b * ty + wk.yi) * tx + wk.xi;
        if (visit)
            for (int r = k; r < steps_cap; ++r) visit[(size_t)wg * steps_cap + r] = -1;
        most = k > most ? k : most;
    }
    if (steps_out) *steps_out = most;
    return AVX_OK;
}

extern "C" int avx_mst_ffn_fused(avx_ctx* ctx, const void* x, const float* gamma, const float* beta, float eps, const void* w1pack, const void* taps_9xhid,
                                 const void* w2pack, void* out, int B, int H, int W, int C, void* stream) {
    if (!ctx) return AVX_ERR_INVALID;
    AVX_REQUIRE(ctx, taps_9xhid, "avx_mst_ffn_fused: NULL pointer");
    return ffn_fused_launch(ctx, x, gamma, beta, eps, w1pack, taps_9xhid, nullptr, w2pack, out, B, H, W, C, stream);
}

extern "C" int avx_mst_ffn_fused_mx(avx_ctx* ctx, const void* x, const float* gamma, const float* beta, float eps, const void* w1pack, const void* dwpack,
                                    const void* w2pack, void* out, int B, int H, int W, int C, void* stream) {
    if (!ctx) return AVX_ERR_INVALID;
    AVX_REQUIRE(ctx, dwpack && (((uintptr_t)dwpack) & 15u) == 0, "avx_mst_ffn_fused_mx: dwpack NULL or not 16-byte aligned");
    return ffn_fused_launch(ctx, x, gamma, beta, eps, w1pack, nullptr, dwpack, w2pack, out, B, H, W, C, stream);
}

static int ffn_fused_launch(avx_ctx* ctx, const void* x, const float* gamma, const float* beta, float eps, const void* w1pack, const void* taps_9xhid, const void* dwpack,
                            const void* w2pack, void* out, int B, int H, int W, int C, void* stream) {
    AVX_REQUIRE(ctx, x && gamma && beta && w1pack && w2pack && out && B > 0 && H > 0 && W > 0, "avx_mst_ffn_fused: NULL pointer or empty tensor");
    AVX_REQUIRE(ctx, C == 32 || C == 64 || C == 128, "avx_mst_ffn_fused: C=%d (32, 64 or 128: 31-channel groups stored 32 wide)", C);
    AVX_REQUIRE(ctx, ((((uintptr_t)x | (uintptr_t)w1pack | (uintptr_t)w2pack | (uintptr_t)out | (uintptr_t)taps_9xhid)) & 15u) == 0,
                "avx_mst_ffn_fused: pointers must be 16-byte aligned");
    AVX_REQUIRE(ctx, x != out, "avx_mst_ffn_fused: neighbouring tiles read each other's halo: the output cannot be the input");
    AVX_HIP(ctx, hipSetDevice(ctx->device));
    hipStream_t s = avx_pick_stream(ctx, stream);
    const long total = (long)B * ((H + kFfnTH - 1) / kFfnTH) * ((W + TS - 1) / TS);
    const char* hp = getenv("AVX_MST_FFN_HPASS");
    const bool small = C == 32 && !(hp && atoi(hp) == 128);
    const int hpass = (small || C == 128) ? 64 : 128, hpitch = hpass * 2 + 16, rpitch = (HS * hpitch + 255) / 256 * 256;
    const long cap = (long)ctx->num_cus * (small ? 2 : 1);
    const bool nw16 = C == 64 && dwpack && !(getenv("AVX_MST_FFN_NW") && atoi(getenv("AVX_MST_FFN_NW")) == 8);
    const size_t lds = (size_t)kFfnNGRP * 32 * (C * 2 + 16) + (size_t)(kFfnTH + 2) * rpitch + (dwpack ? 0 : (size_t)9 * 4 * C * 2) + sizeof(float) * 2 * C + (nw16 ? (size_t)(C / 32) * (hpass / 16) * 1024 : 0);
    AVX_REQUIRE(ctx, total <= 0x7fffffffl, "avx_mst_ffn_fused: 2^31 tiles or more");
    const dim3 grid((unsigned)(total < cap ? total : cap));
    const int order = mst_tile_order();
#define AVX_FFN1(CV, HP, MW, DW, NWV)                                                                                                            \
    {                                                                                                                                            \
        auto k = k_mst_ffn_fused<CV, HP, MW, DW, false, NWV>;                                                                                    \
        AVX_HIP(ctx, hipFuncSetAttribute((const void*)k, hipFuncAttributeMaxDynamicSharedMemorySize, (int)lds));                                 \
        hipLaunchKernelGGL(k, grid, dim3(64 * NWV), lds, s, (const __half*)x, gamma, beta, eps, (const uint4*)w1pack, (const __half*)taps_9xhid, \
                           (const uint4*)w2pack, (__half*)out, B, H, W, (const uint4*)dwpack, (unsigned long long*)nullptr, order);              \
    }
#define AVX_FFN(CV, HP, MW) { if (dwpack) AVX_FFN1(CV, HP, MW, true, 8) else AVX_FFN1(CV, HP, MW, false, 8) }
    if (dwpack && getenv("AVX_FFN_STAMPS") && ((C == 32 && small) || C == 64 || C == 128)) {
        unsigned long long* d_st = nullptr;
        const int nwv = nw16 ? 16 : 8;
        const size_t n = (size_t)grid.x * nwv * 8;
        AVX_HIP(ctx, hipMalloc((void**)&d_st, n * sizeof(unsigned long long)));
#define AVX_FFN_ST(CV, HP, MW, NWV)                                                                                                              \
    {                                                                                                                                            \
        auto k = k_mst_ffn_fused<CV, HP, MW, true, true, NWV>;                                                                                   \
        AVX_HIP(ctx, hipFuncSetAttribute((const void*)k, hipFuncAttributeMaxDynamicSharedMemorySize, (int)lds));                                 \
        hipLaunchKernelGGL(k, grid, dim3(64 * NWV), lds, s, (const __half*)x, gamma, beta, eps, (const uint4*)w1pack, (const __half*)taps_9xhid, \
                           (const uint4*)w2pack, (__half*)out, B, H, W, (const uint4*)dwpack, d_st, order);                                      \
    }
        if (C == 32) AVX_FFN_ST(32, 64, 4, 8) else if (nw16) AVX_FFN_ST(64, 128, 1, 16) else if (C == 64) AVX_FFN_ST(64, 128, 2, 8) else AVX_FFN_ST(128, 64, 2, 8)
#undef AVX_FFN_ST
        AVX_HIP(ctx, hipStreamSynchronize(s));
        unsigned long long* h_st = (unsigned long long*)malloc(n * sizeof(unsigned long long));
        AVX_HIP(ctx, hipMemcpy(h_st, d_st, n * sizeof(unsigned long long), hipMemcpyDeviceToHost));
        double tot[8] = {0}, w0[8] = {0}, w7[8] = {0};
        for (size_t i = 0; i < n; ++i) { tot[i & 7] += (double)h_st[i]; if (((i >> 3) % nwv) == 0) w0[i & 7] += (double)h_st[i]; if (((i >> 3) % nwv) == (size_t)nwv - 1) w7[i & 7] += (double)h_st[i]; }
        double all = 0;
        for (int k2 = 0; k2 < 8; ++k2) all += tot[k2];
        fprintf(stderr, "[ffn stamps C=%d] %u blocks x %d waves, mean cycles per wave %.0f; share per segment (all waves | first wave | last wave): ", C, grid.x, nwv, all / (grid.x * (double)nwv));
        const char* nm[8] = {"bar1", "phase1", "bar2", "phase2a", "bar3", "phase2b", "epilogue", "ln+fetch"};
        for (int k2 = 0; k2 < 8; ++k2) fprintf(stderr, "%s %.1f%% | %.1f%% | %.1f%%  ", nm[k2], 100 * tot[k2] / all, 100 * w0[k2] * nwv / all, 100 * w7[k2] * nwv / all);
        fprintf(stderr, "\n");
        free(h_st);
        (void)hipFree(d_st);
    } else if (C == 32 && small) AVX_FFN(32, 64, 4) else if (C == 32) AVX_FFN(32, 128, 2)
    else if (nw16) AVX_FFN1(64, 128, 1, true, 16)
    else if (C == 64) AVX_FFN(64, 128, 2) else AVX_FFN(128, 64, 2)
#undef AVX_FFN
#undef AVX_FFN1
    AVX_HIP(ctx, hipGetLastError());
    return AVX_OK;
}

extern "C" int avx_mst_attn_tail(avx_ctx* ctx, const void* v, const void* x, const void* mpack16, const void* taps1_9xc, const void* taps2_9xc, const float* bias,
                                 void* out, int B, int H, int W, int C, void* stream) {
    if (!ctx) return AVX_ERR_INVALID;
    AVX_REQUIRE(ctx, v && x && mpack16 && taps1_9xc && taps2_9xc && out && B > 0 && H > 0 && W > 0, "avx_mst_attn_tail: NULL pointer or empty tensor");
    AVX_REQUIRE(ctx, C == 32 || C == 64, "avx_mst_attn_tail: C=%d (32 or 64)", C);
    AVX_REQUIRE(ctx, ((((uintptr_t)v | (uintptr_t)x | (uintptr_t)mpack16 | (uintptr_t)out | (uintptr_t)taps1_9xc | (uintptr_t)taps2_9xc)) & 15u) == 0,
                "avx_mst_attn_tail: pointers must be 16-byte aligned");
    AVX_REQUIRE(ctx, v != out, "avx_mst_attn_tail: tiles read their neighbours' rows of v: the output cannot be v (it may be x)");
    AVX_HIP(ctx, hipSetDevice(ctx->device));
    hipStream_t s = avx_pick_stream(ctx, stream);
    if (C == 32) return launch_attn_tail<32, 4>(ctx, v, x, mpack16, taps1_9xc, taps2_9xc, bias, out, B, H, W, s, nullptr);
    return launch_attn_tail<64, 2>(ctx, v, x, mpack16, taps1_9xc, taps2_9xc, bias, out, B, H, W, s, nullptr);
}

extern "C" int avx_mst_attn_tail_x(avx_ctx* ctx, const void* x, const void* wvpack16, const void* mpack16, const void* taps1_9xc, const void* taps2_9xc,
                                   const float* bias, void* out, int B, int H, int W, int C, void* stream) {
    if (!ctx) return AVX_ERR_INVALID;
    AVX_REQUIRE(ctx, x && wvpack16 && mpack16 && taps1_9xc && taps2_9xc && out && B > 0 && H > 0 && W > 0, "avx_mst_attn_tail_x: NULL pointer or empty tensor");
    AVX_REQUIRE(ctx, C == 32 || C == 64, "avx_mst_attn_tail_x: C=%d (32 or 64)", C);
    AVX_REQUIRE(ctx, ((((uintptr_t)x | (uintptr_t)wvpack16 | (uintptr_t)mpack16 | (uintptr_t)out | (uintptr_t)taps1_9xc | (uintptr_t)taps2_9xc)) & 15u) == 0,
                "avx_mst_attn_tail_x: pointers must be 16-byte aligned");
    AVX_REQUIRE(ctx, x != out, "avx_mst_attn_tail_x: tiles read their neighbours' rows of x: the output cannot be x");
    AVX_HIP(ctx, hipSetDevice(ctx->device));
    hipStream_t s = avx_pick_stream(ctx, stream);
    if (C == 32) return launch_attn_tail<32, 4>(ctx, x, x, mpack16, taps1_9xc, taps2_9xc, bias, out, B, H, W, s, wvpack16);
    return launch_attn_tail<64, 2>(ctx, x, x, mpack16, taps1_9xc, taps2_9xc, bias, out, B, H, W, s, wvpack16);
}

extern "C" int avx_mst_attn_tail_mx(avx_ctx* ctx, const void* x, const void* wvpack16, const void* mpack_mx, const void* dw1pack, const void* dw2pack,
                                    const float* bias, void* out, int B, int H, int W, int C, void* stream) {
    if (!ctx) return AVX_ERR_INVALID;
    AVX_REQUIRE(ctx, x && wvpack16 && mpack_mx && dw1pack && dw2pack && out && B > 0 && H > 0 && W > 0, "avx_mst_attn_tail_mx: NULL pointer or empty tensor");
    AVX_REQUIRE(ctx, C == 32 || C == 64 || C == 128, "avx_mst_attn_tail_mx: C=%d (32, 64 or 128)", C);
    AVX_REQUIRE(ctx, ((((uintptr_t)x | (uintptr_t)wvpack16 | (uintptr_t)mpack_mx | (uintptr_t)out | (uintptr_t)dw1pack | (uintptr_t)dw2pack)) & 15u) == 0,
                "avx_mst_attn_tail_mx: pointers must be 16-byte aligned");
    AVX_REQUIRE(ctx, x != out, "avx_mst_attn_tail_mx: tiles read their neighbours' rows of x: the output cannot be x");
    AVX_HIP(ctx, hipSetDevice(ctx->device));
    hipStream_t s = avx_pick_stream(ctx, stream);
    if (C == 32) return launch_attn_tail_mx<32, 16, 4>(ctx, x, wvpack16, mpack_mx, dw1pack, dw2pack, bias, out, B, H, W, s);
    if (C == 128) return launch_attn_tail_mx<128, 8, 2>(ctx, x, wvpack16, mpack_mx, dw1pack, dw2pack, bias, out, B, H, W, s);
    if (getenv("AVX_MST_TAIL_NW") && atoi(getenv("AVX_MST_TAIL_NW")) == 16) return launch_attn_tail_mx<64, 16, 1, 16>(ctx, x, wvpack16, mpack_mx, dw1pack, dw2pack, bias, out, B, H, W, s);
    return launch_attn_tail_mx<64, 16, 2>(ctx, x, wvpack16, mpack_mx, dw1pack, dw2pack, bias, out, B, H, W, s);
}

extern "C" int avx_mst_conv3x3_lds(avx_ctx* ctx, const void* x, const void* wpack16, const void* add, void* out, int B, int H, int W, int C, void* stream) {
    if (!ctx) return AVX_ERR_INVALID;
    AVX_REQUIRE(ctx, x && wpack16 && out && B > 0 && H > 0 && W > 0, "avx_mst_conv3x3_lds: NULL pointer or empty tensor");
    AVX_REQUIRE(ctx, C == 32, "avx_mst_conv3x3_lds: C=%d (32: the 31-channel full-resolution convs)", C);
    AVX_REQUIRE(ctx, ((((uintptr_t)x | (uintptr_t)wpack16 | (uintptr_t)add | (uintptr_t)out)) & 15u) == 0, "avx_mst_conv3x3_lds: pointers must be 16-byte aligned");
    AVX_REQUIRE(ctx, x != out, "avx_mst_conv3x3_lds: in-place convolution is not possible");
    AVX_HIP(ctx, hipSetDevice(ctx->device));
    hipStream_t s = avx_pick_stream(ctx, stream);
    const long total = (long)B * ((H + TS - 1) / TS) * ((W + TS - 1) / TS);
    const long cap = (long)ctx->num_cus * 3;
    AVX_REQUIRE(ctx, total <= 0x7fffffffl, "avx_mst_conv3x3_lds: 2^31 tiles or more");
    hipLaunchKernelGGL((k_mst_conv3x3_lds<6, false>), dim3((unsigned)(total < cap ? total : cap)), dim3(kFT), 0, s, (const __half*)x, (const uint4*)wpack16, (const __half*)add,
                       (__half*)out, B, H, W, (const uint4*)nullptr, (float*)nullptr, (const float*)nullptr, (float*)nullptr, (SpecStat3*)nullptr, 0, 0, 0, 0, mst_tile_order());
    AVX_HIP(ctx, hipGetLastError());
    return AVX_OK;
}

extern "C" int avx_mst_conv3x3_lds_spectral(avx_ctx* ctx, const void* x, const void* wpack16, const void* add, int H, int W, int C, const float* weights_host, int crop_t,
                                            int crop_l, int Hc, int Wc, float* planes_out, void* partials_out, int* n_partials, void* stream) {
    if (!ctx) return AVX_ERR_INVALID;
    AVX_REQUIRE(ctx, x && wpack16 && weights_host && planes_out && partials_out && n_partials && H > 0 && W > 0, "avx_mst_conv3x3_lds_spectral: NULL pointer or empty tensor");
    AVX_REQUIRE(ctx, C == 32, "avx_mst_conv3x3_lds_spectral: C=%d (32: the 31-band cube as stored)", C);
    AVX_REQUIRE(ctx, crop_t >= 0 && crop_l >= 0 && Hc > 0 && Wc > 0 && crop_t + Hc <= H && crop_l + Wc <= W, "avx_mst_conv3x3_lds_spectral: the crop window must lie inside the frame");
    AVX_REQUIRE(ctx, ((((uintptr_t)x | (uintptr_t)wpack16 | (uintptr_t)add | (uintptr_t)partials_out)) & 15u) == 0, "avx_mst_conv3x3_lds_spectral: pointers must be 16-byte aligned");
    AVX_HIP(ctx, hipSetDevice(ctx->device));
    hipStream_t s = avx_pick_stream(ctx, stream);
    avx_ws* ws = avx_workspace(ctx, s);
    if (!ws) return AVX_ERR_NOMEM;
    float wT[32 * 4];
    for (int b = 0; b < 32; ++b)
        for (int k = 0; k < 4; ++k) wT[b * 4 + k] = k < 3 ? weights_host[(size_t)k * 32 + b] : 0.0f;
    float* dwT = nullptr;
    int rc = avx_const_upload(ctx, ws, 2, wT, sizeof(wT), s, (void**)&dwT);
    if (rc) return rc;
    const long total = (long)((H + TS - 1) / TS) * ((W + TS - 1) / TS);
    const long cap = (long)ctx->num_cus * 2;
    const long blocks = total < cap ? total : cap;
    *n_partials = (int)blocks;
    hipLaunchKernelGGL((k_mst_conv3x3_lds<4, false, true>), dim3((unsigned)blocks), dim3(kFT), 0, s, (const __half*)x, (const uint4*)wpack16, (const __half*)add, (__half*)nullptr, 1, H, W,
                       (const uint4*)nullptr, (float*)nullptr, (const float*)dwT, planes_out, (SpecStat3*)partials_out, crop_t, crop_l, Hc, Wc);
    AVX_HIP(ctx, hipGetLastError());
    return AVX_OK;
}

extern "C" int avx_mst_conv3x3_lds_gram(avx_ctx* ctx, const void* x, const void* wpack16, const void* add, void* out, int H, int W, int C, const void* wqk16, float* gram,
                                        float* nq, float* nk, void* stream) {
    if (!ctx) return AVX_ERR_INVALID;
    AVX_REQUIRE(ctx, x && wpack16 && out && wqk16 && gram && nq && nk && H > 0 && W > 0, "avx_mst_conv3x3_lds_gram: NULL pointer or empty tensor");
    AVX_REQUIRE(ctx, C == 32, "avx_mst_conv3x3_lds_gram: C=%d (32: the 31-channel full-resolution convs)", C);
    AVX_REQUIRE(ctx, ((((uintptr_t)x | (uintptr_t)wpack16 | (uintptr_t)add | (uintptr_t)out | (uintptr_t)wqk16)) & 15u) == 0, "avx_mst_conv3x3_lds_gram: pointers must be 16-byte aligned");
    AVX_REQUIRE(ctx, x != out, "avx_mst_conv3x3_lds_gram: in-place convolution is not possible");
    AVX_HIP(ctx, hipSetDevice(ctx->device));
    hipStream_t s = avx_pick_stream(ctx, stream);
    avx_ws* ws = avx_workspace(ctx, s);
    if (!ws) return AVX_ERR_NOMEM;
    const long total = (long)((H + TS - 1) / TS) * ((W + TS - 1) / TS);
    const long cap = (long)ctx->num_cus * 2;
    const long blocks = total < cap ? total : cap;
    int rc = avx_ensure_scratch(ctx, ws, sizeof(float) * (size_t)blocks * 34 * 32);
    if (rc) return rc;
    float* partial = (float*)ws->d_scratch;
    hipLaunchKernelGGL((k_mst_conv3x3_lds<4, true>), dim3((unsigned)blocks), dim3(kFT), 0, s, (const __half*)x, (const uint4*)wpack16, (const __half*)add, (__half*)out, 1, H, W,
                       (const uint4*)wqk16, partial);
    AVX_HIP(ctx, hipGetLastError());
    return avx_mst_qkv_final_launch(ctx, partial, (int)blocks, 1, gram, nq, nk, s);
}

extern "C" int avx_mst_conv_in_u8(avx_ctx* ctx, const uint8_t* frame_hwc, int H, int W, int pad_top, int pad_bottom, int pad_left, int pad_right,
                                  const float* w_27x32_dev, void* out, void* stream) {
    if (!ctx) return AVX_ERR_INVALID;
    AVX_REQUIRE(ctx, frame_hwc && w_27x32_dev && out && H > 1 && W > 1, "avx_mst_conv_in_u8: NULL pointer or a frame too small to reflect");
    AVX_REQUIRE(ctx, pad_top >= 0 && pad_bottom >= 0 && pad_left >= 0 && pad_right >= 0 && pad_top < H && pad_bottom < H && pad_left < W && pad_right < W,
                "avx_mst_conv_in_u8: reflect padding must be smaller than the frame");
    AVX_REQUIRE(ctx, ((uintptr_t)out & 15u) == 0, "avx_mst_conv_in_u8: out must be 16-byte aligned");
    AVX_HIP(ctx, hipSetDevice(ctx->device));
    hipStream_t s = avx_pick_stream(ctx, stream);
    const int Hp = H + pad_top + pad_bottom, Wp = W + pad_left + pad_right;
    const size_t total = (size_t)Hp * Wp;
    const size_t want = (total + 255) / 256, cap = (size_t)ctx->num_cus * 16;
    if (getenv("AVX_MST_CONV_IN_VALU"))
        hipLaunchKernelGGL(k_mst_conv_in_u8, dim3((unsigned)(want < cap ? want : cap)), dim3(256), 0, s, frame_hwc, w_27x32_dev, (__half*)out, H, W, pad_top, pad_left, Hp, Wp);
    else {
        const size_t wantm = (total + 127) / 128;
        hipLaunchKernelGGL(k_mst_conv_in_u8_mfma, dim3((unsigned)(wantm < cap ? wantm : cap)), dim3(256), 0, s, frame_hwc, w_27x32_dev, (__half*)out, H, W, pad_top,
                           pad_left, Hp, Wp);
    }
    AVX_HIP(ctx, hipGetLastError());
    return AVX_OK;
}

extern "C" int avx_mst_down4x4(avx_ctx* ctx, const void* x, const void* wpack16, void* out, int B, int H, int W, int C, void* stream) {
    if (!ctx) return AVX_ERR_INVALID;
    AVX_REQUIRE(ctx, x && wpack16 && out && B > 0 && H > 0 && W > 0, "avx_mst_down4x4: NULL pointer or empty tensor");
    AVX_REQUIRE(ctx, C == 32 || C == 64, "avx_mst_down4x4: C=%d (32 or 64: the encoder steps 31 -> 62 and 62 -> 124 channels as stored)", C);
    AVX_REQUIRE(ctx, H % 2 == 0 && W % 2 == 0, "avx_mst_down4x4: H and W must be even (the model pads frames to multiples of 8)");
    AVX_REQUIRE(ctx, (long)B * H * W * C * 2 < (1l << 31), "avx_mst_down4x4: input larger than 2 GiB");
    AVX_REQUIRE(ctx, ((((uintptr_t)x | (uintptr_t)wpack16 | (uintptr_t)out)) & 15u) == 0, "avx_mst_down4x4: pointers must be 16-byte aligned");
    AVX_HIP(ctx, hipSetDevice(ctx->device));
    hipStream_t s = avx_pick_stream(ctx, stream);
    const long cap = (long)ctx->num_cus;
    if (C == 32) {
        using G = DownGeo<32>;
        const long total = (long)B * ((H / 2 + G::OH - 1) / G::OH) * ((W / 2 + G::OW - 1) / G::OW);
        hipLaunchKernelGGL(k_mst_down4x4_dma<32>, dim3((unsigned)(total < cap ? total : cap)), dim3(kFT), 0, s, (const __half*)x, (const uint4*)wpack16, (__half*)out, (const void*)ctx->d_zero, B, H, W, mst_tile_order());
    } else {
        using G = DownGeo<64>;
        const long total = (long)B * ((H / 2 + G::OH - 1) / G::OH) * ((W / 2 + G::OW - 1) / G::OW);
        hipLaunchKernelGGL(k_mst_down4x4_dma<64>, dim3((unsigned)(total < cap ? total : cap)), dim3(kFT), 0, s, (const __half*)x, (const uint4*)wpack16, (__half*)out, (const void*)ctx->d_zero, B, H, W, mst_tile_order());
    }
    AVX_HIP(ctx, hipGetLastError());
    return AVX_OK;
}
```

animal-vision_amd/ml/mst_plus_plus.py:

```python
from __future__ import annotations

from typing import Dict, List

import torch
import torch.nn.functional as F

DIM = 31
PAD = 32


def padded(n: int) -> int:
    assert n % DIM == 0
    return n // DIM * PAD


def pad_index(n: int, device=None) -> torch.Tensor:
    i = torch.arange(n, device=device)
    return (i // DIM) * PAD + i % DIM


def pad_channels(t: torch.Tensor, dims) -> torch.Tensor:
    for d in dims:
        n = t.shape[d]
        shape = list(t.shape)
        shape[d] = padded(n)
        out = torch.zeros(shape, dtype=t.dtype, device=t.device)
        out.index_copy_(d, pad_index(n, t.device), t)
        t = out
    return t


def pack_fragments(w_kn: torch.Tensor, transposed: bool) -> torch.Tensor:
    K, N = w_kn.shape
    assert K % 32 == 0 and N % 32 == 0
    dev = w_kn.device
    key = (K, N, transposed, str(dev))
    idx = _FRAG_INDEX.get(key)
    if idx is None:
        lane = torch.arange(64, device=dev)
        c, h = lane % 32, lane // 32
        if transposed:
            c = 16 * ((c % 8) // 4) + 4 * (c // 8) + c % 4
        s = torch.arange(K // 8, device=dev)
        j = torch.arange(4, device=dev)
        k = (h[None, :, None] * (K // 2) + 4 * s[:, None, None] + j[None, None, :])[None]
        col = 32 * torch.arange(N // 32, device=dev)[:, None, None, None] + c[None, None, :, None]
        idx = (k * N + col).contiguous()
        _FRAG_INDEX[key] = idx
    return torch.take(w_kn.contiguous(), idx)


_FRAG_INDEX: Dict[tuple, torch.Tensor] = {}


def pack_fragments16(w_kn: torch.Tensor, halfrow: bool = False) -> torch.Tensor:
    K, N = w_kn.shape
    assert K % 16 == 0 and N % 32 == 0
    dev = w_kn.device
    key = (K, N, "k16h" if halfrow else "k16", str(dev))
    idx = _FRAG_INDEX.get(key)
    if idx is None:
        lane = torch.arange(64, device=dev)
        m, h = lane % 32, lane // 32
        col = 16 * ((m % 8) // 4) + 4 * (m // 8) + m % 4
        s = torch.arange(K // 16, device=dev)
        j = torch.arange(8, device=dev)
        if halfrow:
            k = (8 * s[:, None, None] + (K // 2) * h[None, :, None] + j[None, None, :])[None]
        else:
            k = (16 * s[:, None, None] + 8 * h[None, :, None] + j[None, None, :])[None]
        n = 32 * torch.arange(N // 32, device=dev)[:, None, None, None] + col[None, None, :, None]
        idx = (k * N + n).contiguous()
        _FRAG_INDEX[key] = idx
    return torch.take(w_kn.contiguous(), idx)


def pack_qkv16(wqkv: torch.Tensor) -> torch.Tensor:
    K, N = wqkv.shape
    assert N == 3 * K and K % 32 == 0
    dev = wqkv.device
    key = (K, N, "qkv16", str(dev))
    idx = _FRAG_INDEX.get(key)
    if idx is None:
        lane = torch.arange(64, device=dev)
        m, h = lane % 32, lane // 32
        perm = 16 * ((m % 8) // 4) + 4 * (m // 8) + m % 4
        t = torch.arange(N // 32, device=dev)
        col = 32 * t[:, None] + torch.where(t[:, None] >= 2 * (K // 32), perm[None, :], m[None, :])
        q = torch.arange(K // 16, device=dev)
        j = torch.arange(8, device=dev)
        k = h[None, :, None] * (K // 2) + 8 * q[:, None, None] + j[None, None, :]
        idx = (k[None] * N + col[:, None, :, None]).contiguous()
        _FRAG_INDEX[key] = idx
    return torch.take(wqkv.contiguous(), idx)


def pack_dw_mfma(w: torch.Tensor) -> torch.Tensor:
    ch = w.shape[0]
    assert ch % 8 == 0 and tuple(w.shape[1:]) == (1, 3, 3)
    dev = w.device
    lane = torch.arange(64, device=dev)
    m, q = lane % 16, lane // 16
    s_, c = m // 8, m % 8
    dy = q - s_
    ok = (dy >= 0) & (dy <= 2)
    w8 = w.reshape(ch // 8, 8, 3, 3)
    vals = w8[:, c, dy.clamp(0, 2), :]
    vals = torch.where(ok[None, :, None], vals, torch.zeros_like(vals))
    out = torch.zeros((ch // 8, 3, 64, 8), dtype=w.dtype, device=dev)
    out[:, :, lane, c] = vals.permute(0, 2, 1)
    return out.contiguous()


def fold_layernorm(w1_kn: torch.Tensor, gamma: torch.Tensor, beta: torch.Tensor, scale: float) -> torch.Tensor:
    w = w1_kn.float()
    out = w * gamma.float()[:, None]
    out[31, :] = beta.float() @ w
    return (out / scale).contiguous()


def pack_down4x4(w: torch.Tensor) -> torch.Tensor:
    return torch.stack([pack_fragments16(w[:, :, t // 4, t % 4].t().contiguous()) for t in range(16)]).contiguous()


class _AvxOps:

    def __init__(self):
        import os

        self.enabled = os.environ.get("AVX_MST_TORCH_ONLY", "") == ""
        self._mfma = os.environ.get("AVX_MST_NO_MFMA", "") == ""
        self._ffn2 = os.environ.get("AVX_MST_NO_FFN2", "") == ""
        self._posemb = os.environ.get("AVX_MST_NO_POSEMB", "") == ""
        self._conv_lds = os.environ.get("AVX_MST_NO_CONV_LDS", "") == ""
        self._conv_in = os.environ.get("AVX_MST_NO_CONV_IN", "") == ""
        self._upfuse = os.environ.get("AVX_MST_NO_UPFUSE", "") == ""
        self._tail = os.environ.get("AVX_MST_NO_TAIL", "") == ""
        self._tailx = os.environ.get("AVX_MST_NO_TAILX", "") == ""
        self._down = os.environ.get("AVX_MST_NO_DOWN4X4", "") == ""
        self._qkv16 = os.environ.get("AVX_MST_NO_QKV16", "") == ""
        self._convgram = os.environ.get("AVX_MST_NO_CONVGRAM", "") == ""
        self._ffn = os.environ.get("AVX_MST_NO_FFN_FUSED", "") == ""
        self._gelu_pre = None
        self._dwmx = os.environ.get("AVX_MST_NO_DW_MFMA", "") == ""
        self._specfuse = os.environ.get("AVX_MST_NO_SPEC_FUSE", "") == ""
        self.FFN_FUSED_C = tuple(int(v) for v in os.environ.get("AVX_MST_FFN_FUSED_C", "32,64,128").split(",") if v)
        self._ctx = {}

    def ctx(self, device: torch.device):
        from ..runtime import get_context

        idx = device.index if device.index is not None else torch.cuda.current_device()
        c = get_context(idx)
        if c.device != idx:
            raise RuntimeError(f"libavx context is on device {c.device}, tensor on cuda:{idx} (one process per GPU)")
        return c

    @staticmethod
    def _dt(t: torch.Tensor) -> int:
        if t.dtype == torch.float32:
            return 0
        if t.dtype == torch.float16:
            return 1
        raise TypeError(f"csrc/mst.hip kernels take float32/float16, got {t.dtype}")

    def gram(self, qkv: torch.Tensor, heads: int):
        from .._lib import lib

        b, n, c3 = qkv.shape
        c = c3 // 3
        d = c // heads
        ctx = self.ctx(qkv.device)
        g = torch.empty((b, heads, 32, 32), dtype=torch.float32, device=qkv.device)
        nq = torch.empty((b, c), dtype=torch.float32, device=qkv.device)
        nk = torch.empty((b, c), dtype=torch.float32, device=qkv.device)
        st = torch.cuda.current_stream(qkv.device).cuda_stream
        for i in range(b):
            ctx._check(lib.avx_mst_gram(ctx._h, qkv[i].data_ptr(), self._dt(qkv), n, c, heads, g[i].data_ptr(), nq[i].data_ptr(), nk[i].data_ptr(), st))
        return g[:, :, :d, :d], nq, nk

    def gelu_prescale(self) -> float:
        if self._gelu_pre is None:
            from .. import _lib
            self._gelu_pre = float(_lib.lib.avx_mst_gelu_prescale())
        return self._gelu_pre

    def fused_ok(self, x: torch.Tensor) -> bool:
        return self.enabled and x.is_cuda and x.dtype == torch.float16 and x.shape[-1] in (32, 64, 128) and self._mfma

    def qkv_gram(self, x2: torch.Tensor, wpack: torch.Tensor, heads: int, want_v: bool = True, k16: bool = False):
        from .._lib import lib

        b, n, c = x2.shape
        x2 = x2.contiguous()
        ctx = self.ctx(x2.device)
        v = torch.empty_like(x2) if want_v else None
        g = torch.empty((b, heads, 32, 32), dtype=torch.float32, device=x2.device)
        nq = torch.empty((b, c), dtype=torch.float32, device=x2.device)
        nk = torch.empty((b, c), dtype=torch.float32, device=x2.device)
        st = torch.cuda.current_stream(x2.device).cuda_stream
        fn = lib.avx_mst_qkv_gram16 if k16 else lib.avx_mst_qkv_gram
        for i in range(b):
            ctx._check(fn(ctx._h, x2[i].data_ptr(), wpack.data_ptr(), n, c, v[i].data_ptr() if want_v else None, g[i].data_ptr(), nq[i].data_ptr(), nk[i].data_ptr(), st))
        return v, g, nq, nk

    def ln_gemm_gelu(self, x2: torch.Tensor, gamma: torch.Tensor, beta: torch.Tensor, wpack: torch.Tensor, eps: float = 1e-5) -> torch.Tensor:
        from .._lib import lib

        rows, c = x2.shape
        x2 = x2.contiguous()
        ctx = self.ctx(x2.device)
        out = torch.empty((rows, 4 * c), dtype=torch.float16, device=x2.device)
        ctx._check(lib.avx_mst_ln_gemm_gelu(ctx._h, x2.data_ptr(), gamma.data_ptr(), beta.data_ptr(), eps, wpack.data_ptr(), rows, c, out.data_ptr(),
                                            torch.cuda.current_stream(x2.device).cuda_stream))
        return out

    def convt2x2(self, x: torch.Tensor, wpack: torch.Tensor, bias: torch.Tensor, skip: torch.Tensor = None, wskip: torch.Tensor = None) -> torch.Tensor:
        from .._lib import lib

        b, h, w, c = x.shape
        x = x.contiguous()
        out = torch.empty((b, 2 * h, 2 * w, c // 2), dtype=torch.float16, device=x.device)
        ctx = self.ctx(x.device)
        st = torch.cuda.current_stream(x.device).cuda_stream
        if skip is None:
            ctx._check(lib.avx_mst_convt2x2(ctx._h, x.data_ptr(), wpack.data_ptr(), bias.data_ptr(), out.data_ptr(), b, h, w, c, st))
        else:
            assert skip.is_contiguous() and skip.shape == out.shape
            ctx._check(lib.avx_mst_convt2x2_fuse(ctx._h, x.data_ptr(), wpack.data_ptr(), bias.data_ptr(), skip.data_ptr(), wskip.data_ptr(), out.data_ptr(), b, h, w, c, st))
        return out

    def convt2x2_gram(self, x: torch.Tensor, wpack: torch.Tensor, bias: torch.Tensor, skip: torch.Tensor, wskip: torch.Tensor, wqk16: torch.Tensor):
        from .._lib import lib

        b, h, w, c = x.shape
        assert c == 64 and skip.is_contiguous() and skip.shape == (b, 2 * h, 2 * w, 32)
        x = x.contiguous()
        out = torch.empty((b, 2 * h, 2 * w, 32), dtype=torch.float16, device=x.device)
        g = torch.empty((b, 1, 32, 32), dtype=torch.float32, device=x.device)
        nq = torch.empty((b, 32), dtype=torch.float32, device=x.device)
        nk = torch.empty((b, 32), dtype=torch.float32, device=x.device)
        ctx = self.ctx(x.device)
        st = torch.cuda.current_stream(x.device).cuda_stream
        for i in range(b):
            ctx._check(lib.avx_mst_convt2x2_fuse_gram(ctx._h, x[i].data_ptr(), wpack.data_ptr(), bias.data_ptr(), skip[i].data_ptr(), wskip.data_ptr(), out[i].data_ptr(), h, w, c,
                                                      wqk16.data_ptr(), g[i].data_ptr(), nq[i].data_ptr(), nk[i].data_ptr(), st))
        return out, g, nq, nk

    def posemb(self, v: torch.Tensor, w1_c9: torch.Tensor, w2_c9: torch.Tensor, residual: torch.Tensor = None, bias: torch.Tensor = None) -> torch.Tensor:
        from .._lib import lib

        b, h, w, c = v.shape
        v = v.contiguous()
        residual = residual.contiguous() if residual is not None else None
        out = torch.empty_like(v)
        ctx = self.ctx(v.device)
        ctx._check(lib.avx_mst_posemb(ctx._h, v.data_ptr(), w1_c9.data_ptr(), w2_c9.data_ptr(), residual.data_ptr() if residual is not None else None,
                                      bias.data_ptr() if bias is not None else None, out.data_ptr(), b, h, w, c, torch.cuda.current_stream(v.device).cuda_stream))
        return out

    def conv3x3(self, x: torch.Tensor, wpack: torch.Tensor, add: torch.Tensor = None) -> torch.Tensor:
        from .._lib import lib

        b, h, w, c = x.shape
        x = x.contiguous()
        add = add.contiguous() if add is not None else None
        out = torch.empty_like(x)
        ctx = self.ctx(x.device)
        ctx._check(lib.avx_mst_conv3x3_add(ctx._h, x.data_ptr(), wpack.data_ptr(), add.data_ptr() if add is not None else None, out.data_ptr(), b, h, w, c,
                                           torch.cuda.current_stream(x.device).cuda_stream))
        return out

    def conv_in_u8(self, frame: torch.Tensor, pads, w_27x32: torch.Tensor) -> torch.Tensor:
        from .._lib import lib

        H, W, _ = frame.shape
        t, b, l, r = pads
        frame = frame.contiguous()
        out = torch.empty((1, H + t + b, W + l + r, 32), dtype=torch.float16, device=frame.device)
        ctx = self.ctx(frame.device)
        ctx._check(lib.avx_mst_conv_in_u8(ctx._h, frame.data_ptr(), H, W, t, b, l, r, w_27x32.data_ptr(), out.data_ptr(),
                                          torch.cuda.current_stream(frame.device).cuda_stream))
        return out

    def down4x4(self, x: torch.Tensor, wpack16: torch.Tensor) -> torch.Tensor:
        from .._lib import lib

        b, h, w, c = x.shape
        assert x.is_contiguous() and c in (32, 64) and h % 2 == 0 and w % 2 == 0
        out = torch.empty((b, h // 2, w // 2, 2 * c), dtype=torch.float16, device=x.device)
        ctx = self.ctx(x.device)
        st = torch.cuda.current_stream(x.device).cuda_stream
        per = max(1, (2**31 - 1) // (h * w * c * 2))
        for i in range(0, b, per):
            ctx._check(lib.avx_mst_down4x4(ctx._h, x[i : i + per].data_ptr(), wpack16.data_ptr(), out[i : i + per].data_ptr(), min(per, b - i), h, w, c, st))
        return out

    def conv3x3_lds_gram(self, x: torch.Tensor, wpack16: torch.Tensor, add: torch.Tensor, wqk16: torch.Tensor):
        from .._lib import lib

        b, h, w, c = x.shape
        x = x.contiguous()
        add = add.contiguous() if add is not None else None
        out = torch.empty_like(x)
        g = torch.empty((b, 1, 32, 32), dtype=torch.float32, device=x.device)
        nq = torch.empty((b, c), dtype=torch.float32, device=x.device)
        nk = torch.empty((b, c), dtype=torch.float32, device=x.device)
        ctx = self.ctx(x.device)
        st = torch.cuda.current_stream(x.device).cuda_stream
        for i in range(b):
            ctx._check(lib.avx_mst_conv3x3_lds_gram(ctx._h, x[i].data_ptr(), wpack16.data_ptr(), add[i].data_ptr() if add is not None else None, out[i].data_ptr(), h, w, c,
                                                    wqk16.data_ptr(), g[i].data_ptr(), nq[i].data_ptr(), nk[i].data_ptr(), st))
        return out, g, nq, nk

    def conv3x3_lds_spectral(self, x: torch.Tensor, wpack16: torch.Tensor, add: torch.Tensor, weights, crop):
        import ctypes

        import numpy as np

        from .._lib import lib

        b, h, w, c = x.shape
        assert b == 1 and c == 32 and x.is_contiguous() and (add is None or add.is_contiguous())
        t, l, H, W = crop
        ctx = self.ctx(x.device)
        planes = torch.empty((3, H, W), dtype=torch.float32, device=x.device)
        ncu = torch.cuda.get_device_properties(x.device).multi_processor_count
        partials = torch.empty((ncu * 3, 3, 2), dtype=torch.float64, device=x.device)
        wh = np.ascontiguousarray(weights, dtype=np.float32)
        assert wh.shape == (3, 32)
        n = ctypes.c_int(0)
        ctx._check(lib.avx_mst_conv3x3_lds_spectral(ctx._h, x.data_ptr(), wpack16.data_ptr(), add.data_ptr() if add is not None else None, h, w, c,
                                                    wh.ctypes.data_as(ctypes.POINTER(ctypes.c_float)), t, l, H, W, planes.data_ptr(), partials.data_ptr(), ctypes.byref(n),
                                                    torch.cuda.current_stream(x.device).cuda_stream))
        return planes, partials, int(n.value)

    def conv3x3_lds(self, x: torch.Tensor, wpack16: torch.Tensor, add: torch.Tensor = None) -> torch.Tensor:
        from .._lib import lib

        b, h, w, c = x.shape
        x = x.contiguous()
        add = add.contiguous() if add is not None else None
        out = torch.empty_like(x)
        ctx = self.ctx(x.device)
        ctx._check(lib.avx_mst_conv3x3_lds(ctx._h, x.data_ptr(), wpack16.data_ptr(), add.data_ptr() if add is not None else None, out.data_ptr(), b, h, w, c,
                                           torch.cuda.current_stream(x.device).cuda_stream))
        return out

    def attn_pack(self, gram: torch.Tensor, nq: torch.Tensor, nk: torch.Tensor, rescale: torch.Tensor, wproj_t: torch.Tensor) -> torch.Tensor:
        from .._lib import lib

        c = nq.numel()
        ctx = self.ctx(gram.device)
        out = torch.empty((c // 32, c // 8, 64, 4), dtype=torch.float16, device=gram.device)
        ctx._check(lib.avx_mst_attn_pack(ctx._h, gram.data_ptr(), nq.data_ptr(), nk.data_ptr(), rescale.data_ptr(), wproj_t.data_ptr(), c, out.data_ptr(),
                                         torch.cuda.current_stream(gram.device).cuda_stream))
        return out

    def attn_pack16(self, gram: torch.Tensor, nq: torch.Tensor, nk: torch.Tensor, rescale: torch.Tensor, wproj_t: torch.Tensor) -> torch.Tensor:
        from .._lib import lib

        c = nq.numel()
        ctx = self.ctx(gram.device)
        out = torch.empty((c // 32, c // 16, 64, 8), dtype=torch.float16, device=gram.device)
        ctx._check(lib.avx_mst_attn_pack16(ctx._h, gram.data_ptr(), nq.data_ptr(), nk.data_ptr(), rescale.data_ptr(), wproj_t.data_ptr(), c, out.data_ptr(),
                                           torch.cuda.current_stream(gram.device).cuda_stream))
        return out

    def attn_pack_mx(self, gram: torch.Tensor, nq: torch.Tensor, nk: torch.Tensor, rescale: torch.Tensor, wproj_t: torch.Tensor) -> torch.Tensor:
        from .._lib import lib

        c = nq.numel()
        ctx = self.ctx(gram.device)
        out = torch.empty((c // 8, c // 16, 64, 8), dtype=torch.float16, device=gram.device)
        ctx._check(lib.avx_mst_attn_pack_mx(ctx._h, gram.data_ptr(), nq.data_ptr(), nk.data_ptr(), rescale.data_ptr(), wproj_t.data_ptr(), c, out.data_ptr(),
                                            torch.cuda.current_stream(gram.device).cuda_stream))
        return out

    def attn_tail_mx(self, x: torch.Tensor, wvpack16: torch.Tensor, mpack_mx: torch.Tensor, dw1: torch.Tensor, dw2: torch.Tensor, bias: torch.Tensor,
                     out: torch.Tensor = None) -> torch.Tensor:
        from .._lib import lib

        h, w, c = x.shape
        assert x.is_contiguous()
        out = torch.empty_like(x) if out is None else out
        ctx = self.ctx(x.device)
        ctx._check(lib.avx_mst_attn_tail_mx(ctx._h, x.data_ptr(), wvpack16.data_ptr(), mpack_mx.data_ptr(), dw1.data_ptr(), dw2.data_ptr(), bias.data_ptr(),
                                            out.data_ptr(), 1, h, w, c, torch.cuda.current_stream(x.device).cuda_stream))
        return out

    def attn_tail(self, v: torch.Tensor, x: torch.Tensor, mpack16: torch.Tensor, taps1: torch.Tensor, taps2: torch.Tensor, bias: torch.Tensor,
                  out: torch.Tensor = None) -> torch.Tensor:
        from .._lib import lib

        h, w, c = v.shape
        assert v.is_contiguous() and x.is_contiguous() and x.shape == v.shape
        out = torch.empty_like(v) if out is None else out
        ctx = self.ctx(v.device)
        ctx._check(lib.avx_mst_attn_tail(ctx._h, v.data_ptr(), x.data_ptr(), mpack16.data_ptr(), taps1.data_ptr(), taps2.data_ptr(), bias.data_ptr(), out.data_ptr(),
                                         1, h, w, c, torch.cuda.current_stream(v.device).cuda_stream))
        return out

    def attn_tail_x(self, x: torch.Tensor, wvpack16: torch.Tensor, mpack16: torch.Tensor, taps1: torch.Tensor, taps2: torch.Tensor, bias: torch.Tensor,
                    out: torch.Tensor = None) -> torch.Tensor:
        from .._lib import lib

        h, w, c = x.shape
        assert x.is_contiguous()
        out = torch.empty_like(x) if out is None else out
        ctx = self.ctx(x.device)
        ctx._check(lib.avx_mst_attn_tail_x(ctx._h, x.data_ptr(), wvpack16.data_ptr(), mpack16.data_ptr(), taps1.data_ptr(), taps2.data_ptr(), bias.data_ptr(),
                                           out.data_ptr(), 1, h, w, c, torch.cuda.current_stream(x.device).cuda_stream))
        return out

    def rowgemm_add(self, a: torch.Tensor, wpack: torch.Tensor, add: torch.Tensor = None, a2: torch.Tensor = None, wpack2: torch.Tensor = None) -> torch.Tensor:
        from .._lib import lib

        rows, c = a.shape
        assert a.is_contiguous() and (add is None or (add.is_contiguous() and add.shape == a.shape)) and (a2 is None or (a2.is_contiguous() and a2.shape == a.shape))
        out = add if add is not None else torch.empty_like(a)
        ctx = self.ctx(a.device)
        ctx._check(lib.avx_mst_rowgemm_add(ctx._h, a.data_ptr(), wpack.data_ptr(), a2.data_ptr() if a2 is not None else None,
                                           wpack2.data_ptr() if a2 is not None else None, add.data_ptr() if add is not None else None, out.data_ptr(), rows, c,
                                           torch.cuda.current_stream(a.device).cuda_stream))
        return out

    def ffn_fused(self, x: torch.Tensor, gamma: torch.Tensor, beta: torch.Tensor, w1p: torch.Tensor, taps: torch.Tensor, w2p: torch.Tensor,
                  eps: float = 1e-5, dwpack: torch.Tensor = None) -> torch.Tensor:
        from .._lib import lib

        b, h, w, c = x.shape
        x = x.contiguous()
        out = torch.empty_like(x)
        ctx = self.ctx(x.device)
        st = torch.cuda.current_stream(x.device).cuda_stream
        if dwpack is not None:
            ctx._check(lib.avx_mst_ffn_fused_mx(ctx._h, x.data_ptr(), gamma.data_ptr(), beta.data_ptr(), eps, w1p.data_ptr(), dwpack.data_ptr(), w2p.data_ptr(),
                                                out.data_ptr(), b, h, w, c, st))
        else:
            ctx._check(lib.avx_mst_ffn_fused(ctx._h, x.data_ptr(), gamma.data_ptr(), beta.data_ptr(), eps, w1p.data_ptr(), taps.data_ptr(), w2p.data_ptr(),
                                             out.data_ptr(), b, h, w, c, st))
        return out

    def dw_gemm_add(self, hidden: torch.Tensor, w_c9: torch.Tensor, w2pack: torch.Tensor, x: torch.Tensor) -> torch.Tensor:
        from .._lib import lib

        b, h, w, c = x.shape
        assert hidden.is_contiguous() and x.is_contiguous() and hidden.shape == (b, h, w, 4 * c)
        ctx = self.ctx(x.device)
        ctx._check(lib.avx_mst_dw_gemm_add(ctx._h, hidden.data_ptr(), w_c9.data_ptr(), w2pack.data_ptr(), x.data_ptr(), x.data_ptr(), b, h, w, c,
                                           torch.cuda.current_stream(x.device).cuda_stream))
        return x

    def dwconv(self, x: torch.Tensor, w_c9: torch.Tensor, gelu: bool, residual: torch.Tensor = None, bias: torch.Tensor = None) -> torch.Tensor:
        from .._lib import lib

        b, h, w, c = x.shape
        x = x.contiguous()
        y = torch.empty_like(x)
        ctx = self.ctx(x.device)
        if residual is not None or bias is not None:
            residual = residual.contiguous() if residual is not None else None
            ctx._check(lib.avx_dwconv3x3_nhwc_add(ctx._h, x.data_ptr(), w_c9.data_ptr(), y.data_ptr(), b, h, w, c, 1 if gelu else 0,
                                                  residual.data_ptr() if residual is not None else None, bias.data_ptr() if bias is not None else None,
                                                  torch.cuda.current_stream(x.device).cuda_stream))
            return y
        ctx._check(lib.avx_dwconv3x3_nhwc(ctx._h, x.data_ptr(), w_c9.data_ptr(), y.data_ptr(), self._dt(x), b, h, w, c, 1 if gelu else 0,
                                          torch.cuda.current_stream(x.device).cuda_stream))
        return y

    def layernorm(self, x: torch.Tensor, gamma: torch.Tensor, beta: torch.Tensor, eps: float = 1e-5, group: int = 0, real: int = 0) -> torch.Tensor:
        from .._lib import lib

        c = x.shape[-1]
        x = x.contiguous()
        y = torch.empty_like(x)
        ctx = self.ctx(x.device)
        ctx._check(lib.avx_layernorm_rows_grouped(ctx._h, x.data_ptr(), gamma.data_ptr(), beta.data_ptr(), y.data_ptr(), self._dt(x), x.numel() // c, c, eps,
                                                  group or c, real or c, torch.cuda.current_stream(x.device).cuda_stream))
        return y


_AVX = _AvxOps()


def _msab_keys(prefix: str, dim: int) -> Dict[str, tuple]:
    a, f = f"{prefix}.blocks.0.0", f"{prefix}.blocks.0.1"
    return {
        f"{a}.to_q.weight": (dim, dim), f"{a}.to_k.weight": (dim, dim), f"{a}.to_v.weight": (dim, dim),
        f"{a}.rescale": (dim // DIM, 1, 1), f"{a}.proj.weight": (dim, dim), f"{a}.proj.bias": (dim,),
        f"{a}.pos_emb.0.weight": (dim, 1, 3, 3), f"{a}.pos_emb.2.weight": (dim, 1, 3, 3),
        f"{f}.fn.net.0.weight": (4 * dim, dim, 1, 1), f"{f}.fn.net.2.weight": (4 * dim, 1, 3, 3),
        f"{f}.fn.net.4.weight": (dim, 4 * dim, 1, 1), f"{f}.norm.weight": (dim,), f"{f}.norm.bias": (dim,),
    }


def reference_key_names(stage: int = 3) -> Dict[str, tuple]:
    keys: Dict[str, tuple] = {"conv_in.weight": (DIM, 3, 3, 3)}
    for s in range(stage):
        p = f"body.{s}"
        keys[f"{p}.embedding.weight"] = (DIM, DIM, 3, 3)
        d = DIM
        for i in range(2):
            keys.update(_msab_keys(f"{p}.encoder_layers.{i}.0", d))
            keys[f"{p}.encoder_layers.{i}.1.weight"] = (2 * d, d, 4, 4)
            d *= 2
        keys.update(_msab_keys(f"{p}.bottleneck", d))
        for i in range(2):
            keys[f"{p}.decoder_layers.{i}.0.weight"] = (d, d // 2, 2, 2)
            keys[f"{p}.decoder_layers.{i}.0.bias"] = (d // 2,)
            keys[f"{p}.decoder_layers.{i}.1.weight"] = (d // 2, d, 1, 1)
            keys.update(_msab_keys(f"{p}.decoder_layers.{i}.2", d // 2))
            d //= 2
        keys[f"{p}.mapping.weight"] = (DIM, DIM, 3, 3)
    keys["conv_out.weight"] = (DIM, DIM, 3, 3)
    return keys


class MSTPlusPlus(torch.nn.Module):
    def __init__(self, stage: int = 3):
        super().__init__()
        self.stage = stage
        self._shapes = reference_key_names(stage)
        self.w = torch.nn.ParameterDict({self._pk(k): torch.nn.Parameter(torch.zeros(s), requires_grad=False) for k, s in self._shapes.items()})
        self._prepared: Dict[str, torch.Tensor] = {}
        self.capture_attn = None

    def _capture(self, gram: torch.Tensor, nq: torch.Tensor, nk: torch.Tensor, p: str, heads: int):
        b = gram.shape[0]
        a = gram[:, :, :DIM, :DIM].float() / (nk.reshape(b, heads, PAD, 1)[:, :, :DIM].clamp_min(1e-12) * nq.reshape(b, heads, 1, PAD)[..., :DIM].clamp_min(1e-12))
        a = a * self._p(p + ".rescale").float().reshape(1, heads, 1, 1)
        self.capture_attn.append(a.softmax(dim=-1).cpu())

    @staticmethod
    def _pk(k: str) -> str:
        return k.replace(".", "__")

    def load_reference_state_dict(self, sd: Dict[str, torch.Tensor], strict: bool = True) -> "MSTPlusPlus":
        if "state_dict" in sd and not any(k.endswith(".weight") for k in sd):
            sd = sd["state_dict"]
        sd = {k.replace("module.", "", 1) if k.startswith("module.") else k: v for k, v in sd.items()}
        missing = [k for k in self._shapes if k not in sd]
        extra = [k for k in sd if k not in self._shapes]
        if strict and (missing or extra):
            raise KeyError(f"state_dict mismatch: missing {missing[:3]}..., unexpected {extra[:3]}...")
        with torch.no_grad():
            for k, shape in self._shapes.items():
                if k in sd:
                    t = torch.as_tensor(sd[k])
                    if tuple(t.shape) != tuple(shape):
                        raise ValueError(f"{k}: shape {tuple(t.shape)} != {shape}")
                    self.w[self._pk(k)].copy_(t.to(self.w[self._pk(k)].dtype))
        self._prepared.clear()
        return self

    def reference_state_dict(self) -> Dict[str, torch.Tensor]:
        return {k: self.w[self._pk(k)].detach() for k in self._shapes}

    def init_seeded(self, seed: int = 0) -> "MSTPlusPlus":
        g = torch.Generator().manual_seed(seed)
        with torch.no_grad():
            for k, shape in self._shapes.items():
                p = self.w[self._pk(k)]
                if k.endswith("norm.weight") or k.endswith("rescale"):
                    p.fill_(1.0)
                elif k.endswith("bias"):
                    p.zero_()
                elif len(shape) == 2:
                    p.copy_(torch.randn(shape, generator=g) * 0.02)
                else:
                    fan_in = shape[1] * shape[2] * shape[3]
                    bound = (1.0 / fan_in) ** 0.5
                    p.copy_((torch.rand(shape, generator=g) * 2 - 1) * bound)
        self._prepared.clear()
        return self

    def _p(self, k: str) -> torch.Tensor:
        return self.w[self._pk(k)]

    def _prep(self, name: str, build):
        ref = self._p("conv_in.weight")
        key = f"{name}|{ref.dtype}|{ref.device}"
        t = self._prepared.get(key)
        if t is None:
            t = build()
            self._prepared[key] = t
        return t

    def _w(self, k: str, dims) -> torch.Tensor:
        return self._prep(k + ".pad" + "".join(map(str, dims)), lambda: pad_channels(self._p(k), dims).contiguous())

    def _conv3(self, x: torch.Tensor, key: str, add: torch.Tensor = None) -> torch.Tensor:
        if _AVX.fused_ok(x) and x.shape[-1] == 32 and _AVX._conv_lds:
            wq = self._prep(key + ".frag9k16", lambda: torch.stack([pack_fragments16(self._w(key, (0, 1))[:, :, t // 3, t % 3].t().contiguous()) for t in range(9)]).contiguous())
            return _AVX.conv3x3_lds(x, wq, add)
        if _AVX.fused_ok(x) and x.shape[-1] == 32:
            wp = self._prep(key + ".frag9", lambda: torch.stack([pack_fragments(self._w(key, (0, 1))[:, :, t // 3, t % 3].t().contiguous(), True) for t in range(9)]).contiguous())
            return _AVX.conv3x3(x, wp, add)
        y = self._conv_nhwc(x, self._w(key, (0, 1)), padding=1)
        return y + add if add is not None else y

    def _conv_nhwc(self, x: torch.Tensor, w: torch.Tensor, **kw) -> torch.Tensor:
        y = F.conv2d(x.permute(0, 3, 1, 2), w, **kw)
        return y.permute(0, 2, 3, 1)

    def _ms_msa(self, x: torch.Tensor, p: str, heads: int, pre=None) -> torch.Tensor:
        b, h, w, c = x.shape
        n = h * w
        x2 = x.reshape(b, n, c)
        wqkv = self._prep(p + ".qkv", lambda: torch.cat([self._w(p + ".to_q.weight", (0, 1)), self._w(p + ".to_k.weight", (0, 1)),
                                                         self._w(p + ".to_v.weight", (0, 1))], 0).t().contiguous())
        d = c // heads
        if _AVX.fused_ok(x):
            tailx = _AVX._tail and _AVX._tailx and (c in (32, 64) or (c == 128 and _AVX._dwmx))
            if _AVX._qkv16:
                wpk = self._prep(p + ".qkv.frag16", lambda: pack_qkv16(wqkv))
            else:
                wpk = self._prep(p + ".qkv.frag", lambda: torch.cat([pack_fragments(wqkv[:, : 2 * c], False), pack_fragments(wqkv[:, 2 * c :], True)], 0).contiguous())
            if pre is not None and tailx:
                v, (gram, nq, nk) = None, pre
            else:
                v, gram, nq, nk = _AVX.qkv_gram(x2, wpk, heads, want_v=not tailx, k16=_AVX._qkv16)
            if self.capture_attn is not None:
                self._capture(gram, nq, nk, p, heads)
            resc = self._prep(p + ".rescale32", lambda: self._p(p + ".rescale").float().reshape(heads).contiguous())
            wpt = self._prep(p + ".proj.t32", lambda: self._w(p + ".proj.weight", (0, 1)).t().float().contiguous())
            bias32 = self._prep(p + ".proj.bias32", lambda: self._w(p + ".proj.bias", (0,)).float().contiguous())
            vi = v.reshape(b, h, w, c) if v is not None else None
            if _AVX._tail and (c in (32, 64) or tailx):
                k1, k2 = p + ".pos_emb.0.weight", p + ".pos_emb.2.weight"
                t1 = self._prep(k1 + ".t9h", lambda: self._w(k1, (0,)).reshape(c, 9).t().contiguous())
                t2 = self._prep(k2 + ".t9h", lambda: self._w(k2, (0,)).reshape(c, 9).t().contiguous())
                xc = x.contiguous()
                out = torch.empty_like(xc)
                if tailx and _AVX._dwmx:
                    wv16 = self._prep(p + ".wv.frag16h", lambda: pack_fragments16(wqkv[:, 2 * c :].contiguous(), halfrow=True))
                    gs = _AVX.gelu_prescale()
                    d1 = self._prep(k1 + f".dwmx/{gs}", lambda: pack_dw_mfma((self._w(k1, (0,)).float() / gs).to(x.dtype)))
                    d2 = self._prep(k2 + f".dwmx*{gs}", lambda: pack_dw_mfma((self._w(k2, (0,)).float() * gs).to(x.dtype)))
                    for i in range(b):
                        _AVX.attn_tail_mx(xc[i], wv16, _AVX.attn_pack_mx(gram[i], nq[i], nk[i], resc, wpt), d1, d2, bias32, out[i])
                    return out
                if tailx:
                    wv16 = self._prep(p + ".wv.frag16", lambda: pack_fragments16(wqkv[:, 2 * c :].contiguous()))
                    for i in range(b):
                        _AVX.attn_tail_x(xc[i], wv16, _AVX.attn_pack16(gram[i], nq[i], nk[i], resc, wpt), t1, t2, bias32, out[i])
                    return out
                for i in range(b):
                    _AVX.attn_tail(vi[i], xc[i], _AVX.attn_pack16(gram[i], nq[i], nk[i], resc, wpt), t1, t2, bias32, out[i])
                return out
            if _AVX._posemb:
                k1, k2 = p + ".pos_emb.0.weight", p + ".pos_emb.2.weight"
                w91 = self._prep(k1 + ".c9f32", lambda: self._w(k1, (0,)).reshape(c, 9).float().contiguous())
                w92 = self._prep(k2 + ".c9f32", lambda: self._w(k2, (0,)).reshape(c, 9).float().contiguous())
                pe = _AVX.posemb(vi, w91, w92, x, bias32)
            else:
                pe = self._dw(self._dw(vi, p + ".pos_emb.0.weight", gelu=True), p + ".pos_emb.2.weight", gelu=False, residual=x, bias=bias32)
            for i in range(b):
                _AVX.rowgemm_add(v[i], _AVX.attn_pack(gram[i], nq[i], nk[i], resc, wpt), pe[i].reshape(n, c))
            return pe
        qkv = x2 @ wqkv
        q, k, v = qkv[..., :c], qkv[..., c : 2 * c], qkv[..., 2 * c :]
        if x.is_cuda and _AVX.enabled:
            gram, nq, nk = _AVX.gram(qkv, heads)
            nq = nq.reshape(b, heads, 1, d).clamp_min(1e-12)
            nk = nk.reshape(b, heads, d, 1).clamp_min(1e-12)
        else:
            qh = q.reshape(b, n, heads, d).permute(0, 2, 1, 3)
            kh = k.reshape(b, n, heads, d).permute(0, 2, 1, 3)
            gram = torch.matmul(kh.transpose(-2, -1), qh).float()
            nq = torch.linalg.vector_norm(q.float(), dim=1).reshape(b, heads, 1, d).clamp_min(1e-12)
            nk = torch.linalg.vector_norm(k.float(), dim=1).reshape(b, heads, d, 1).clamp_min(1e-12)
        attn = gram / (nk * nq)
        attn = attn * self._p(p + ".rescale").float().reshape(1, heads, 1, 1)
        attn[..., DIM:] = float("-inf")
        attn = attn.softmax(dim=-1)
        if self.capture_attn is not None:
            self.capture_attn.append(attn[:, :, :DIM, :DIM].float().cpu())
        wp = self._w(p + ".proj.weight", (0, 1))
        wp_h = wp.t().reshape(heads, d, c).float()
        M = torch.matmul(attn.transpose(-2, -1), wp_h.unsqueeze(0)).reshape(b, c, c).to(x.dtype)
        vi = v.reshape(b, h, w, c)
        out_c = torch.baddbmm(self._w(p + ".proj.bias", (0,)).to(x.dtype).reshape(1, 1, c), v, M).reshape(b, h, w, c)
        pe = self._dw(self._dw(vi, p + ".pos_emb.0.weight", gelu=True), p + ".pos_emb.2.weight", gelu=False)
        return out_c + pe + x

    def _dw(self, x: torch.Tensor, key: str, gelu: bool, residual: torch.Tensor = None, bias: torch.Tensor = None) -> torch.Tensor:
        c = x.shape[-1]
        if x.is_cuda and _AVX.enabled:
            w9 = self._prep(key + ".c9f32", lambda: self._w(key, (0,)).reshape(c, 9).float().contiguous())
            return _AVX.dwconv(x, w9, gelu, residual, bias)
        y = self._conv_nhwc(x, self._w(key, (0,)), padding=1, groups=c)
        y = F.gelu(y) if gelu else y
        if residual is not None:
            y = y + residual
        return y + bias.to(y.dtype) if bias is not None else y

    def _ffn(self, x: torch.Tensor, p: str) -> torch.Tensor:
        b, h, w, c = x.shape
        g32 = self._prep(p + ".g32", lambda: self._w(p + ".norm.weight", (0,)).float().contiguous())
        b32 = self._prep(p + ".b32", lambda: self._w(p + ".norm.bias", (0,)).float().contiguous())
        w2 = self._prep(p + ".w2", lambda: self._w(p + ".fn.net.4.weight", (0, 1)).reshape(c, 4 * c).t().contiguous())
        if _AVX.fused_ok(x) and _AVX._ffn and c in _AVX.FFN_FUSED_C:
            key = p + ".fn.net.2.weight"
            if _AVX._dwmx:
                gs = _AVX.gelu_prescale()
                w1s = self._prep(p + f".w1.frag16.ln/{gs}", lambda: pack_fragments16(fold_layernorm(self._w(p + ".fn.net.0.weight", (0, 1)).reshape(4 * c, c).t(), g32, b32, gs).to(x.dtype)))
                w2s = self._prep(p + f".w2.frag16*{gs}", lambda: pack_fragments16((w2.float() * gs).to(x.dtype).contiguous()))
                return _AVX.ffn_fused(x, g32, b32, w1s, None, w2s, dwpack=self._prep(key + ".dwmx", lambda: pack_dw_mfma(self._w(key, (0,)))))
            w1q = self._prep(p + ".w1.frag16", lambda: pack_fragments16(self._w(p + ".fn.net.0.weight", (0, 1)).reshape(4 * c, c).t().contiguous()))
            w2q = self._prep(p + ".w2.frag16", lambda: pack_fragments16(w2))
            t9 = self._prep(key + ".t9h", lambda: self._w(key, (0,)).reshape(4 * c, 9).t().contiguous())
            return _AVX.ffn_fused(x, g32, b32, w1q, t9, w2q)
        if _AVX.fused_ok(x):
            w1p = self._prep(p + ".w1.frag", lambda: pack_fragments(self._w(p + ".fn.net.0.weight", (0, 1)).reshape(4 * c, c).t().contiguous(), True))
            y = _AVX.ln_gemm_gelu(x.reshape(b * h * w, c), g32, b32, w1p).reshape(b, h, w, 4 * c)
            if c in (32, 64) and x.is_contiguous() and _AVX._ffn2:
                key = p + ".fn.net.2.weight"
                w9 = self._prep(key + ".c9f32", lambda: self._w(key, (0,)).reshape(4 * c, 9).float().contiguous())
                w2p = self._prep(p + ".w2.frag", lambda: pack_fragments(w2, True))
                return _AVX.dw_gemm_add(y, w9, w2p, x)
            y = self._dw(y, p + ".fn.net.2.weight", gelu=True)
            return x.reshape(b * h * w, c).addmm_(y.reshape(b * h * w, 4 * c), w2).reshape(b, h, w, c)
        if x.is_cuda and _AVX.enabled:
            y = _AVX.layernorm(x, g32, b32, group=PAD, real=DIM)
        else:
            real = self._prep(p + ".real", lambda: pad_index(c // PAD * DIM, x.device))
            yr = F.layer_norm(x.float().index_select(-1, real), (real.numel(),), g32.index_select(0, real), b32.index_select(0, real))
            y = torch.zeros_like(x, dtype=torch.float32).index_copy_(-1, real, yr).to(x.dtype)
        w1 = self._prep(p + ".w1", lambda: self._w(p + ".fn.net.0.weight", (0, 1)).reshape(4 * c, c).t().contiguous())
        y = F.gelu(y.reshape(b, h * w, c) @ w1).reshape(b, h, w, 4 * c)
        y = self._dw(y, p + ".fn.net.2.weight", gelu=True)
        return (y.reshape(b, h * w, 4 * c) @ w2).reshape(b, h, w, c) + x

    def _msab(self, x: torch.Tensor, p: str, heads: int, pre=None) -> torch.Tensor:
        x = self._ms_msa(x, p + ".blocks.0.0", heads, pre)
        return self._ffn(x, p + ".blocks.0.1")

    def _mst(self, x: torch.Tensor, p: str) -> torch.Tensor:
        pre = None
        ekey, a0 = p + ".embedding.weight", f"{p}.encoder_layers.0.0.blocks.0.0"
        if _AVX.fused_ok(x) and x.shape[-1] == 32 and _AVX._conv_lds and _AVX._convgram and _AVX._qkv16 and _AVX._tail and _AVX._tailx:
            wq = self._prep(ekey + ".frag9k16", lambda: torch.stack([pack_fragments16(self._w(ekey, (0, 1))[:, :, t // 3, t % 3].t().contiguous()) for t in range(9)]).contiguous())
            wqkv = self._prep(a0 + ".qkv", lambda: torch.cat([self._w(a0 + ".to_q.weight", (0, 1)), self._w(a0 + ".to_k.weight", (0, 1)),
                                                              self._w(a0 + ".to_v.weight", (0, 1))], 0).t().contiguous())
            wqk = self._prep(a0 + ".qkv.frag16", lambda: pack_qkv16(wqkv))
            fea, g, nq, nk = _AVX.conv3x3_lds_gram(x, wq, None, wqk)
            pre = (g, nq, nk)
        else:
            fea = self._conv3(x, ekey)
        skips: List[torch.Tensor] = []
        heads = 1
        for i in range(2):
            fea = self._msab(fea, f"{p}.encoder_layers.{i}.0", heads, pre if i == 0 else None)
            skips.append(fea)
            dkey = f"{p}.encoder_layers.{i}.1.weight"
            if _AVX.fused_ok(fea) and _AVX._down and fea.shape[-1] in (32, 64) and fea.is_contiguous():
                fea = _AVX.down4x4(fea, self._prep(dkey + ".frag16", lambda: pack_down4x4(self._w(dkey, (0, 1)))))
            else:
                fea = self._conv_nhwc(fea, self._w(dkey, (0, 1)), stride=2, padding=1)
            heads *= 2
        fea = self._msab(fea, p + ".bottleneck", heads)
        for i in range(2):
            kw = f"{p}.decoder_layers.{i}.0.weight"
            if _AVX.fused_ok(fea) and fea.shape[-1] in (64, 128) and _AVX._upfuse:
                ch = fea.shape[-1] // 2
                wfk = f"{p}.fuse{i}"
                wf_ = self._prep(wfk, lambda: self._w(f"{p}.decoder_layers.{i}.1.weight", (0, 1)).reshape(ch, 2 * ch).t().contiguous())
                gt = self._prep(kw + ".upfuse4", lambda: torch.stack([pack_fragments((self._w(kw, (0, 1))[:, :, t // 2, t % 2].float() @ wf_[:ch].float()).half().contiguous(), True)
                                                                     for t in range(4)]).contiguous())
                gb = self._prep(kw + ".upfuse.bias", lambda: (self._w(f"{p}.decoder_layers.{i}.0.bias", (0,)).float() @ wf_[:ch].float()).contiguous())
                wbot_ = self._prep(f"{p}.fuse{i}.bot", lambda: pack_fragments(wf_[ch:].contiguous(), True))
                heads //= 2
                a2 = f"{p}.decoder_layers.{i}.2.blocks.0.0"
                if ch == 32 and _AVX._convgram and _AVX._qkv16 and _AVX._tail and _AVX._tailx:
                    wqkv2 = self._prep(a2 + ".qkv", lambda: torch.cat([self._w(a2 + ".to_q.weight", (0, 1)), self._w(a2 + ".to_k.weight", (0, 1)),
                                                                       self._w(a2 + ".to_v.weight", (0, 1))], 0).t().contiguous())
                    wqk2 = self._prep(a2 + ".qkv.frag16", lambda: pack_qkv16(wqkv2))
                    fea, g2, nq2, nk2 = _AVX.convt2x2_gram(fea, gt, gb, skips[1 - i].contiguous(), wbot_, wqk2)
                    fea = self._msab(fea, f"{p}.decoder_layers.{i}.2", heads, (g2, nq2, nk2))
                    continue
                fea = _AVX.convt2x2(fea, gt, gb, skips[1 - i].contiguous(), wbot_)
                fea = self._msab(fea, f"{p}.decoder_layers.{i}.2", heads)
                continue
            if _AVX.fused_ok(fea) and fea.shape[-1] in (64, 128):
                wt = self._prep(kw + ".frag4", lambda: torch.stack([pack_fragments(self._w(kw, (0, 1))[:, :, t // 2, t % 2].contiguous(), True) for t in range(4)]).contiguous())
                bt = self._prep(kw + ".bias32", lambda: self._w(f"{p}.decoder_layers.{i}.0.bias", (0,)).float().contiguous())
                up = _AVX.convt2x2(fea, wt, bt)
            else:
                up = F.conv_transpose2d(fea.permute(0, 3, 1, 2), self._w(kw, (0, 1)), self._w(f"{p}.decoder_layers.{i}.0.bias", (0,)), stride=2).permute(0, 2, 3, 1)
            heads //= 2
            skip = skips[1 - i]
            b, h, w, ch = up.shape
            c2 = 2 * ch
            wf = self._prep(f"{p}.fuse{i}", lambda: self._w(f"{p}.decoder_layers.{i}.1.weight", (0, 1)).reshape(c2 // 2, c2).t().contiguous())
            if _AVX.fused_ok(skip):
                up, skip = up.contiguous(), skip.contiguous()
                wtop = self._prep(f"{p}.fuse{i}.top", lambda: pack_fragments(wf[:ch].contiguous(), True))
                wbot = self._prep(f"{p}.fuse{i}.bot", lambda: pack_fragments(wf[ch:].contiguous(), True))
                fea = _AVX.rowgemm_add(up.reshape(b * h * w, ch), wtop, None, skip.reshape(b * h * w, ch), wbot).reshape(b, h, w, ch)
            else:
                cat = torch.cat([up, skip], dim=-1)
                fea = (cat.reshape(b, h * w, c2) @ wf).reshape(b, h, w, c2 // 2)
            fea = self._msab(fea, f"{p}.decoder_layers.{i}.2", heads)
        return self._conv3(fea, p + ".mapping.weight", add=x)

    @torch.no_grad()
    def forward_from_u8(self, frame: torch.Tensor, pads, spectral=None):
        w27 = self._prep("conv_in.w27x32", lambda: self._w("conv_in.weight", (0,)).permute(2, 3, 1, 0).reshape(27, PAD).float().contiguous())
        x = _AVX.conv_in_u8(frame, pads, w27)
        assert x.shape[1] % 8 == 0 and x.shape[2] % 8 == 0, "pad the frame to a multiple of 8 (predict_torch.py pads to 16)"
        if spectral is None:
            return self._body(x)
        H, W, _ = frame.shape
        return self._body(x, spectral=(spectral, (pads[0], pads[2], H, W)))

    def can_fuse_spectral(self) -> bool:
        return self.can_fuse_conv_in() and _AVX._conv_lds and _AVX._specfuse

    def _body(self, x: torch.Tensor, spectral=None):
        hfe = x
        for s in range(self.stage):
            hfe = self._mst(hfe, f"body.{s}")
        if spectral is not None:
            key = "conv_out.weight"
            wq = self._prep(key + ".frag9k16", lambda: torch.stack([pack_fragments16(self._w(key, (0, 1))[:, :, t // 3, t % 3].t().contiguous()) for t in range(9)]).contiguous())
            return _AVX.conv3x3_lds_spectral(hfe.contiguous(), wq, x.contiguous(), spectral[0], spectral[1])
        return self._conv3(hfe, "conv_out.weight", add=x)

    def can_fuse_conv_in(self) -> bool:
        ref = self._p("conv_in.weight")
        return _AVX.enabled and _AVX._mfma and _AVX._conv_in and ref.is_cuda and ref.dtype == torch.float16

    @torch.no_grad()
    def forward_nhwc(self, x: torch.Tensor) -> torch.Tensor:
        b, c, h_inp, w_inp = x.shape
        pad_h, pad_w = (8 - h_inp % 8) % 8, (8 - w_inp % 8) % 8
        if pad_h or pad_w:
            x = F.pad(x, [0, pad_w, 0, pad_h], mode="reflect")
        x = x.to(self._p("conv_in.weight").dtype).contiguous(memory_format=torch.channels_last).permute(0, 2, 3, 1)
        x = self._conv_nhwc(x, self._w("conv_in.weight", (0,)), padding=1)
        return self._body(x)[:, :h_inp, :w_inp, :]

    @torch.no_grad()
    def forward(self, x: torch.Tensor) -> torch.Tensor:
        return self.forward_nhwc(x)[..., :DIM].permute(0, 3, 1, 2)


def hbm_bytes_per_px(stage: int = 3) -> float:

    def msab(c: int) -> float:
        t = 2.0 * c
        if _AVX._tail and _AVX._tailx and (c in (32, 64) or (c == 128 and _AVX._dwmx)):
            b = t
            b += 2 * t
            return b + ((2 * t) if (_AVX._ffn and c in _AVX.FFN_FUSED_C) else (t + 4 * t + ((4 * t + 2 * t) if _AVX._ffn2 else (4 * t + 4 * t + 4 * t + 2 * t))))
        b = 2 * t
        if _AVX._tail and c in (32, 64):
            b += 3 * t
        else:
            b += (3 * t if _AVX._posemb else 5 * t)
# ... 22 lines not shown
```

include/avx.h:

```cpp
#ifndef AVX_H
#define AVX_H

#include <stddef.h>
#include <stdint.h>

#ifdef __cplusplus
extern "C" {
#endif

#define AVX_ABI_VERSION 1

typedef struct avx_ctx avx_ctx;

typedef enum avx_status {
    AVX_OK = 0,
    AVX_ERR_INVALID = -1,
    AVX_ERR_NO_DEVICE = -2,
    AVX_ERR_HIP = -3,
    AVX_ERR_UNSUPPORTED = -4,
    AVX_ERR_NOMEM = -5
} avx_status;

int avx_abi_version(void);
int avx_device_count(void);
// ... 179 lines not shown

typedef struct avx_frame_metrics {
    uint32_t abs_hist[3][256];
    double   ssim[3];
} avx_frame_metrics;

int avx_frame_metrics_u8(avx_ctx* ctx, const uint8_t* a_hwc, const uint8_t* b_hwc, int n_frames, int H, int W,
                         int with_ssim, avx_frame_metrics* out_dev, void* stream);

typedef struct avx_plane_metrics_rec {
    uint32_t abs_hist[3][1024];
    double   ssim[3];
} avx_plane_metrics_rec;

int avx_plane_metrics(avx_ctx* ctx, int fmt_a, const uint8_t* a, int fmt_b, const uint8_t* b, int n_frames, int H, int W,
                      int with_ssim, avx_plane_metrics_rec* out_dev, void* stream);

typedef struct avx_ms_ssim_rec {
    double cs[3][5];
    double ssim[3][5];
} avx_ms_ssim_rec;

int avx_frame_metrics_ms_u8(avx_ctx* ctx, const uint8_t* a_hwc, const uint8_t* b_hwc, int n_frames, int H, int W,
                            avx_frame_metrics* out_dev, avx_ms_ssim_rec* ms_out_dev, void* stream);

int avx_remap_linear_planes(avx_ctx* ctx, const float* src_planes, int K, int H, int W, const float* mapx_dev,
                            const float* mapy_dev, float* dst_planes, float border_value, void* stream);

int avx_sobel3_plane(avx_ctx* ctx, const float* plane, int H, int W, float* gx, float* gy, void* stream);

typedef struct avx_mantis_desc {
    uint32_t struct_size;
    int32_t n_bands;
    const float* band_matrix_host;
    const float* band_lut_host;
    int32_t n_wavelengths;
    const float* lobe_gains_host;
    float lobe_denom;
    const float* band_weights_host;
    int32_t pano_new_w;
    int32_t hsi_small_h, hsi_small_w;
    float red_keep;
    float haze, haze_keep, haze_tint[3];
    int32_t pre_soft_ksize; const double* pre_soft_taps_host;
    float cos2_global, sin2_global;
    float orientation_mix, pol_linear_strength, pol_linear_gamma, pol_circular_strength;
    int32_t unsharp_ksize; const double* unsharp_taps_host; float unsharp_amount;
    float barcode_saturation, barcode_opacity, winner_take_most;
    const float* rows_host;
    float scan_row_gain; int32_t scan_ksize; const double* scan_taps_host;
    int32_t periph_ksize; const double* periph_taps_host;
    const float* xx_host; const float* yy_host;
    float periph_radius, periph_softness;
    const float* lin_hwc_in;
    int32_t out_float;
} avx_mantis_desc;

int avx_mantis_u8(avx_ctx* ctx, const uint8_t* in_hwc, uint8_t* out_baseline_hwc, uint8_t* out_hwc, int H, int W,
                  const avx_mantis_desc* desc, void* stream);
int avx_mantis_u8_batch(avx_ctx* ctx, const uint8_t* in_hwc, uint8_t* out_baseline_hwc, uint8_t* out_hwc, int n_frames, int H, int W,
                        const avx_mantis_desc* desc, void* stream);

int avx_uv_front_u8(avx_ctx* ctx, const uint8_t* in_hwc, int H, int W, int pano_new_w, float* lin_hwc_out,
                    uint8_t* baseline_hwc_out, void* stream);
int avx_panorama_warp_f32(avx_ctx* ctx, const float* src_hwc, int H, int W, int new_w, float* dst_hwc, void* stream);
typedef struct avx_band_stack_desc {
    uint32_t struct_size;
    int32_t n_bands;
    const float* band_matrix_host;
    int32_t n_wavelengths;
    const float* lobe_gains_host;
    float lobe_denom;
    const float* band_weights_host;
    int32_t small_h, small_w;
} avx_band_stack_desc;
int avx_band_stack(avx_ctx* ctx, const float* lin_hwc, int H, int W, const avx_band_stack_desc* desc,
                   float* stack_hwk_out, void* stream);
int avx_uv_front_u8_batch(avx_ctx* ctx, const uint8_t* in_hwc, int n_frames, size_t in_frame_stride, int H, int W, int pano_new_w,
                          float* lin_hwc_out, size_t lin_frame_stride, uint8_t* baseline_hwc_out, size_t baseline_frame_stride,
                          void* stream);
int avx_band_stack_batch(avx_ctx* ctx, const float* lin_hwc, int n_frames, size_t lin_frame_stride, int H, int W,
                         const avx_band_stack_desc* desc, float* stack_hwk_out, size_t stack_frame_stride, void* stream);
int avx_percentile_dev(avx_ctx* ctx, const float* data_dev, size_t n, double q, double* out_dev, void* stream);
int avx_percentiles_dev(avx_ctx* ctx, int count, const float* const* data_dev, const size_t* n, const double* q,
                        double* const* out_dev, void* stream);

enum { AVX_EW_MAX_INSN = 384, AVX_EW_MAX_PLANES = 24, AVX_EW_MAX_REGS = 32, AVX_EW_MAX_ACC = 16 };
enum {
    AVX_EW_CONST = 1, AVX_EW_SCALAR, AVX_EW_LOAD, AVX_EW_STORE,
    AVX_EW_ADD, AVX_EW_SUB, AVX_EW_MUL, AVX_EW_DIV, AVX_EW_MIN, AVX_EW_MAX, AVX_EW_POW, AVX_EW_ATAN2,
    AVX_EW_NEG, AVX_EW_ABS, AVX_EW_SQRT, AVX_EW_EXP, AVX_EW_LOG, AVX_EW_SIN, AVX_EW_COS, AVX_EW_FLOOR, AVX_EW_CEIL,
    AVX_EW_CLIP01, AVX_EW_TANH,
    AVX_EW_LT, AVX_EW_LE, AVX_EW_GT, AVX_EW_GE, AVX_EW_EQ, AVX_EW_AND, AVX_EW_OR, AVX_EW_NOT,
    AVX_EW_SELECT,
    AVX_EW_ACCMIN, AVX_EW_ACCMAX, AVX_EW_ACCSUM
};
enum { AVX_EW_OPCODE_MASK = 0x3f, AVX_EW_IMM_A = 0x40, AVX_EW_IMM_B = 0x80 };
enum {
    AVX_EW_PLANE_F32 = 0,
    AVX_EW_PLANE_U8,
    AVX_EW_PLANE_U8_LUT,
    AVX_EW_PLANE_COL,
    AVX_EW_PLANE_ROW,
    AVX_EW_PLANE_U8_ENC
};
enum { AVX_EW_ACC_MIN = 0, AVX_EW_ACC_MAX, AVX_EW_ACC_SUM, AVX_EW_ACC_MEAN };
typedef struct avx_ew_insn { uint8_t op, dst, a, b; uint32_t imm; } avx_ew_insn;
typedef struct avx_ew_plane { void* ptr; int32_t stride; int32_t kind; } avx_ew_plane;
typedef struct avx_ew_program {
    uint32_t struct_size;
    int32_t H, W;
    int32_t n_insn; const avx_ew_insn* insn_host;
    int32_t n_planes; const avx_ew_plane* planes_host;
    int32_t n_acc; const int32_t* acc_host;
    double* scalars_dev; int32_t n_scalars;
} avx_ew_program;
int avx_ew_run(avx_ctx* ctx, const avx_ew_program* program, void* stream);
enum { AVX_EW_MAX_FRAMES = 16 };
int avx_ew_run_batch(avx_ctx* ctx, const avx_ew_program* program, int n_frames, const size_t* plane_frame_stride_bytes_host,
                     size_t scalars_frame_stride, void* stream);
int avx_ew_spec_stats(unsigned long long* hits, unsigned long long* misses);


int avx_mst_gram(avx_ctx* ctx, const void* qkv, int dtype, size_t n_pix, int C, int heads, float* gram, float* nq, float* nk, void* stream);

int avx_mst_qkv_gram(avx_ctx* ctx, const void* x, const void* wpack, size_t n_pix, int C, void* v_out, float* gram, float* nq, float* nk,
                     void* stream);
int avx_mst_qkv_gram16(avx_ctx* ctx, const void* x, const void* wpack16, size_t n_pix, int C, void* v_out, float* gram, float* nq, float* nk,
                       void* stream);
int avx_mst_ln_gemm_gelu(avx_ctx* ctx, const void* x, const float* gamma, const float* beta, float eps, const void* wpack, size_t rows, int C,
                         void* out, void* stream);

int avx_mst_dw_gemm_add(avx_ctx* ctx, const void* hidden, const float* w_c9, const void* w2pack, const void* residual, void* out, int B, int H,
                        int W, int C, void* stream);

int avx_mst_conv_in_u8(avx_ctx* ctx, const uint8_t* frame_hwc, int H, int W, int pad_top, int pad_bottom, int pad_left, int pad_right,
                       const float* w_27x32_dev, void* out, void* stream);

int avx_mst_conv3x3_lds(avx_ctx* ctx, const void* x, const void* wpack16, const void* add, void* out, int B, int H, int W, int C, void* stream);
int avx_mst_conv3x3_lds_gram(avx_ctx* ctx, const void* x, const void* wpack16, const void* add, void* out, int H, int W, int C, const void* wqk16, float* gram,
                             float* nq, float* nk, void* stream);
int avx_mst_convt2x2_fuse_gram(avx_ctx* ctx, const void* x, const void* wpack, const float* bias, const void* skip, const void* wskip, void* out, int H, int W, int C,
                               const void* wqk16, float* gram, float* nq, float* nk, void* stream);
int avx_mst_down4x4(avx_ctx* ctx, const void* x, const void* wpack16, void* out, int B, int H, int W, int C, void* stream);

int avx_mst_attn_pack16(avx_ctx* ctx, const float* gram, const float* nq, const float* nk, const float* rescale, const float* wproj_t, int C, void* mpack,
                        void* stream);
int avx_mst_attn_tail(avx_ctx* ctx, const void* v, const void* x, const void* mpack16, const void* taps1_9xc, const void* taps2_9xc, const float* bias,
                      void* out, int B, int H, int W, int C, void* stream);
int avx_mst_attn_tail_x(avx_ctx* ctx, const void* x, const void* wvpack16, const void* mpack16, const void* taps1_9xc, const void* taps2_9xc,
                        const float* bias, void* out, int B, int H, int W, int C, void* stream);
int avx_mst_attn_tail_mx(avx_ctx* ctx, const void* x, const void* wvpack16, const void* mpack_mx, const void* dw1pack, const void* dw2pack,
                         const float* bias, void* out, int B, int H, int W, int C, void* stream);
int avx_mst_attn_pack_mx(avx_ctx* ctx, const float* gram, const float* nq, const float* nk, const float* rescale, const float* wproj_t, int C, void* mpack,
                         void* stream);


int avx_mst_conv3x3_lds_spectral(avx_ctx* ctx, const void* x, const void* wpack16, const void* add, int H, int W, int C, const float* weights_host, int crop_t,
                                 int crop_l, int Hc, int Wc, float* planes_out, void* partials_out, int* n_partials, void* stream);

int avx_mst_ffn_fused(avx_ctx* ctx, const void* x, const float* gamma, const float* beta, float eps, const void* w1pack, const void* taps_9xhid,
                      const void* w2pack, void* out, int B, int H, int W, int C, void* stream);
int avx_mst_ffn_fused_mx(avx_ctx* ctx, const void* x, const float* gamma, const float* beta, float eps, const void* w1pack, const void* dwpack,
                         const void* w2pack, void* out, int B, int H, int W, int C, void* stream);
float avx_mst_gelu_prescale(void);

int avx_mst_tile_order(int frames, int ty, int tx, int nwg, int raster, long long* visit, int steps_cap, int* steps_out);

int avx_mst_rowgemm_add(avx_ctx* ctx, const void* a, const void* wpack, const void* a2, const void* wpack2, const void* add, void* out, size_t rows,
                        int C, void* stream);

int avx_mst_attn_pack(avx_ctx* ctx, const float* gram, const float* nq, const float* nk, const float* rescale, const float* wproj_t, int C,
                      void* mpack, void* stream);

int avx_mst_conv3x3_add(avx_ctx* ctx, const void* x, const void* wpack, const void* add, void* out, int B, int H, int W, int C, void* stream);

int avx_mst_posemb(avx_ctx* ctx, const void* v, const float* w1_c9, const float* w2_c9, const void* residual, const float* bias, void* out, int B,
                   int H, int W, int C, void* stream);

int avx_mst_convt2x2(avx_ctx* ctx, const void* x, const void* wpack, const float* bias, void* out, int B, int H, int W, int C, void* stream);
int avx_mst_convt2x2_fuse(avx_ctx* ctx, const void* x, const void* wpack, const float* bias, const void* skip, const void* wskip, void* out, int B, int H,
                          int W, int C, void* stream);

int avx_dwconv3x3_nhwc(avx_ctx* ctx, const void* x, const float* w_c9, void* y, int dtype, int B, int H, int W, int C, int gelu_out, void* stream);
int avx_dwconv3x3_nhwc_add(avx_ctx* ctx, const void* x, const float* w_c9, void* y, int B, int H, int W, int C, int gelu_out,
                           const void* residual, const float* bias, void* stream);

int avx_layernorm_rows(avx_ctx* ctx, const void* x, const float* gamma, const float* beta, void* y, int dtype, size_t rows, int C, float eps, void* stream);
int avx_layernorm_rows_grouped(avx_ctx* ctx, const void* x, const float* gamma, const float* beta, void* y, int dtype, size_t rows, int C, float eps,
                               int group, int real, void* stream);

int avx_get_table(int which, void* dst_host, size_t capacity);

#ifdef __cplusplus
}
#endif
#endif
```

Baseline: 425.6.

## Use sparse smfmac for depthwise 3x3 conv in FFN and attention tail

Measured after the change: 433.6 (median of 6 runs). +1.9%, better.

```diff
diff --git a/animal-vision_amd/_lib.py b/animal-vision_amd/_lib.py
--- a/animal-vision_amd/_lib.py
+++ b/animal-vision_amd/_lib.py
@@ -339,11 +339,13 @@
     "avx_mst_attn_pack16": (_i, [_vp, _vp, _vp, _vp, _vp, _vp, _i, _vp, _vp]),
     "avx_mst_attn_pack_mx": (_i, [_vp, _vp, _vp, _vp, _vp, _vp, _i, _vp, _vp]),
     "avx_mst_attn_tail_mx": (_i, [_vp, _vp, _vp, _vp, _vp, _vp, _vp, _vp, _i, _i, _i, _i, _vp]),
+    "avx_mst_attn_tail_sp": (_i, [_vp, _vp, _vp, _vp, _vp, _vp, _vp, _vp, _i, _i, _i, _i, _vp]),
     "avx_mst_attn_tail": (_i, [_vp, _vp, _vp, _vp, _vp, _vp, _vp, _vp, _i, _i, _i, _i, _vp]),
     "avx_mst_attn_tail_x": (_i, [_vp, _vp, _vp, _vp, _vp, _vp, _vp, _vp, _i, _i, _i, _i, _vp]),
     "avx_mst_ffn_fused": (_i, [_vp, _vp, _vp, _vp, ctypes.c_float, _vp, _vp, _vp, _vp, _i, _i, _i, _i, _vp]),
     "avx_mst_conv3x3_lds_spectral": (_i, [_vp, _vp, _vp, _vp, _i, _i, _i, _fp, _i, _i, _i, _i, _vp, _vp, ctypes.POINTER(ctypes.c_int), _vp]),
     "avx_mst_ffn_fused_mx": (_i, [_vp, _vp, _vp, _vp, ctypes.c_float, _vp, _vp, _vp, _vp, _i, _i, _i, _i, _vp]),
+    "avx_mst_ffn_fused_sp": (_i, [_vp, _vp, _vp, _vp, ctypes.c_float, _vp, _vp, _vp, _vp, _i, _i, _i, _i, _vp]),
     "avx_mst_gelu_prescale": (ctypes.c_float, []),
     "avx_mst_tile_order": (_i, [_i, _i, _i, _i, _i, ctypes.POINTER(ctypes.c_longlong), _i, ctypes.POINTER(ctypes.c_int)]),
     "avx_mst_dw_gemm_add": (_i, [_vp, _vp, _vp, _vp, _vp, _vp, _i, _i, _i, _i, _vp]),
diff --git a/animal-vision_amd/csrc/mst_fused.hip b/animal-vision_amd/csrc/mst_fused.hip
--- a/animal-vision_amd/csrc/mst_fused.hip
+++ b/animal-vision_amd/csrc/mst_fused.hip
@@ -33,7 +33,27 @@
     return e && !strcmp(e, "raster") ? AVX_TILE_ORDER_RASTER : AVX_TILE_ORDER_XCD;
 }
 
-template <int C, int HPASS, int MINW, bool DWM, bool STAMP = false, int NW = 8>
+typedef _Float16 half16_t __attribute__((ext_vector_type(16)));
+template <bool DWS>
+__device__ __forceinline__ float4_t dw_unit(const half8_t (&a)[3], const uint4 (&bq)[3]) {
+    float4_t acc = {0.f, 0.f, 0.f, 0.f};
+    if constexpr (DWS) {
+        const half8_t b0 = __builtin_bit_cast(half8_t, bq[0]), b1 = __builtin_bit_cast(half8_t, bq[1]);
+        acc = __builtin_amdgcn_mfma_f32_16x16x32_f16(a[1], __builtin_bit_cast(half8_t, bq[2]), acc, 0, 0, 0);
+        acc = __builtin_amdgcn_smfmac_f32_16x16x64_f16(a[0], __builtin_shufflevector(b0, b1, 0, 1, 2, 3, 4, 5, 6, 7, 8, 9, 10, 11, 12, 13, 14, 15), acc,
+                                                       (int)__builtin_bit_cast(uint4, a[2]).x, 0, 0);
+    } else {
+#pragma unroll
+        for (int i = 0; i < 3; ++i) acc = __builtin_amdgcn_mfma_f32_16x16x32_f16(a[i], __builtin_bit_cast(half8_t, bq[i]), acc, 0, 0, 0);
+    }
+    return acc;
+}
+template <bool DWS>
+__device__ __forceinline__ half8_t dw_frag(const uint4* p, int i) {
+    if (DWS && i == 2) return __builtin_bit_cast(half8_t, uint4{*reinterpret_cast<const unsigned*>(p), 0u, 0u, 0u});
+    return __builtin_bit_cast(half8_t, *p);
+}
+template <int C, int HPASS, int MINW, bool DWM, bool STAMP = false, int NW = 8, bool DWS = false>
 __global__ __launch_bounds__(64 * NW, MINW) void k_mst_ffn_fused(const __half* __restrict__ x , const float* __restrict__ gamma, const float* __restrict__ beta,
                                                           float eps, const uint4* __restrict__ w1pack , const __half* __restrict__ taps ,
                                                           const uint4* __restrict__ w2pack , __half* __restrict__ out , int B,
@@ -44,7 +64,7 @@
     static_assert(C == 32 || C == 64 || C == 128, "31-, 62- or 124-channel blocks (stored 32 / 64 / 128 wide)");
     constexpr int NTHR = 64 * NW, NGW = (NGRP + NW - 1) / NW;
     constexpr int NTW = NT / (NW / 8), NOCTW = HPASS / (8 * NW);
-    static_assert((NW == 8 || NW == 16) && NT % (NW / 8) == 0 && (!DWM || HPASS % (8 * NW) == 0) && (DWM || NW == 8), "wave split");
+    static_assert((NW == 8 || NW == 16) && NT % (NW / 8) == 0 && (!DWM || HPASS % (8 * NW) == 0) && (DWM || NW == 8) && (DWM || !DWS), "wave split");
     constexpr bool PREFETCH = C <= 64;
     extern __shared__ __align__(16) unsigned char smem[];
     unsigned char* yt = smem;
@@ -231,7 +251,7 @@
 #pragma unroll
                 for (int o2 = 0; o2 < NOCTW; ++o2)
 #pragma unroll
-                    for (int i = 0; i < 3; ++i) af[o2][i] = __builtin_bit_cast(half8_t, dwpack[((size_t)(pass * (HPASS / 8) + NW * o2 + wave) * 3 + i) * 64 + lane]);
+                    for (int i = 0; i < 3; ++i) af[o2][i] = dw_frag<DWS>(dwpack + ((size_t)(pass * (HPASS / 8) + NW * o2 + wave) * 3 + i) * 64 + lane, i);
             }
             {
                 const int ct = wave % NCT;
@@ -304,9 +324,7 @@
 #pragma unroll
                     for (int u = 0; u < NU; ++u) {
                         const int o2 = u / (FTH / 2);
-                        float4_t acc = {0.f, 0.f, 0.f, 0.f};
-#pragma unroll
-                        for (int i = 0; i < 3; ++i) acc = __builtin_amdgcn_mfma_f32_16x16x32_f16(af[o2][i], __builtin_bit_cast(half8_t, bq[i]), acc, 0, 0, 0);
+                        const float4_t acc = dw_unit<DWS>(af[o2], bq);
                         if (u + 1 < NU) rd(u + 1);
                         __builtin_amdgcn_sched_barrier(0);
                         if (u > 0) finish(u - 1, prev);
@@ -319,9 +337,7 @@
                     for (int u = 0; u < NU; ++u) {
                         const int o2 = u / (FTH / 2);
                         rd(u);
-                        float4_t acc = {0.f, 0.f, 0.f, 0.f};
-#pragma unroll
-                        for (int i = 0; i < 3; ++i) acc = __builtin_amdgcn_mfma_f32_16x16x32_f16(af[o2][i], __builtin_bit_cast(half8_t, bq[i]), acc, 0, 0, 0);
+                        const float4_t acc = dw_unit<DWS>(af[o2], bq);
                         finish(u, acc);
                     }
                 }
@@ -640,7 +656,7 @@
 }
 
 
-template <int C, int TR, int MINW, bool STAMP = false, int NW = 8>
+template <int C, int TR, int MINW, bool STAMP = false, int NW = 8, bool DWS = false>
 __global__ __launch_bounds__(64 * NW, MINW) void k_mst_attn_tail_mx(const __half* __restrict__ x , const uint4* __restrict__ wvpack ,
                                                                 const uint4* __restrict__ mpack , const uint4* __restrict__ dw1 ,
                                                                 const uint4* __restrict__ dw2 , const float* __restrict__ bias ,
@@ -676,8 +692,8 @@
     auto load_frags = [&](int oc) {
 #pragma unroll
         for (int i = 0; i < 3; ++i) {
-            a1[i] = __builtin_bit_cast(half8_t, dw1[((size_t)oc * 3 + i) * 64 + lane]);
-            a2[i] = __builtin_bit_cast(half8_t, dw2[((size_t)oc * 3 + i) * 64 + lane]);
+            a1[i] = dw_frag<DWS>(dw1 + ((size_t)oc * 3 + i) * 64 + lane, i);
+            a2[i] = dw_frag<DWS>(dw2 + ((size_t)oc * 3 + i) * 64 + lane, i);
         }
 #pragma unroll
         for (int t2 = 0; t2 < NK; ++t2) am[t2] = __builtin_bit_cast(half8_t, mpack[((size_t)oc * NK + t2) * 64 + lane]);
@@ -808,9 +824,7 @@
             float4_t prev = {0.f, 0.f, 0.f, 0.f};
 #pragma unroll
             for (int u = 0; u < NMID; ++u) {
-                float4_t acc = {0.f, 0.f, 0.f, 0.f};
-#pragma unroll
-                for (int i = 0; i < 3; ++i) acc = __builtin_amdgcn_mfma_f32_16x16x32_f16(a1[i], __builtin_bit_cast(half8_t, bq[i]), acc, 0, 0, 0);
+                const float4_t acc = dw_unit<DWS>(a1, bq);
                 if (u + 1 < NMID) rd(u + 1);
                 __builtin_amdgcn_sched_barrier(0);
                 if (u > 0) finish(u - 1, prev);
@@ -850,9 +864,7 @@
 #pragma unroll
                 for (int u = 0; u < NOUT; ++u) {
                     const uint2 xu = xn;
-                    float4_t acc = {0.f, 0.f, 0.f, 0.f};
-#pragma unroll
-                    for (int i = 0; i < 3; ++i) acc = __builtin_amdgcn_mfma_f32_16x16x32_f16(a2[i], __builtin_bit_cast(half8_t, bq[i]), acc, 0, 0, 0);
+                    float4_t acc = dw_unit<DWS>(a2, bq);
 #pragma unroll
                     for (int t2 = 0; t2 < NK; ++t2) acc = __builtin_amdgcn_mfma_f32_16x16x32_f16(am[t2], __builtin_bit_cast(half8_t, bg[t2]), acc, 0, 0, 0);
                     if (u + 1 < NOUT) rd(u + 1);
@@ -866,9 +878,7 @@
 #pragma unroll
                 for (int u = 0; u < NOUT; ++u) {
                     const uint2 xu = STASH ? xn : xr[STASH ? 0 : u];
-                    float4_t acc = {0.f, 0.f, 0.f, 0.f};
-#pragma unroll
-                    for (int i = 0; i < 3; ++i) acc = __builtin_amdgcn_mfma_f32_16x16x32_f16(a2[i], __builtin_bit_cast(half8_t, bq[i]), acc, 0, 0, 0);
+                    float4_t acc = dw_unit<DWS>(a2, bq);
 #pragma unroll
                     for (int t2 = 0; t2 < NK; ++t2) acc = __builtin_amdgcn_mfma_f32_16x16x32_f16(am[t2], __builtin_bit_cast(half8_t, bg[t2]), acc, 0, 0, 0);
                     if (u + 1 < NOUT) rd(u + 1);
@@ -891,7 +901,7 @@
     }
 }
 
-template <int C, int TR, int MINW, int NW = 8>
+template <int C, int TR, int MINW, int NW = 8, bool DWS = false>
 int launch_attn_tail_mx(avx_ctx* ctx, const void* x, const void* wvpack, const void* mpack, const void* dw1, const void* dw2, const float* bias, void* out, int B, int H, int W,
                         hipStream_t s) {
     constexpr int PP = C * 2 + 16, RP = (18 * PP + 255) / 256 * 256;
@@ -901,7 +911,7 @@
     AVX_REQUIRE(ctx, total <= 0x7fffffffl, "avx_mst_attn_tail_mx: 2^31 tiles or more");
     const unsigned blocks = (unsigned)(total < cap ? total : cap);
     if (getenv("AVX_TAIL_STAMPS")) {
-        auto ks = k_mst_attn_tail_mx<C, TR, MINW, true, NW>;
+        auto ks = k_mst_attn_tail_mx<C, TR, MINW, true, NW, DWS>;
         unsigned long long* d_st = nullptr;
         const size_t n = (size_t)blocks * NW * 8;
         AVX_HIP(ctx, hipMalloc((void**)&d_st, n * sizeof(unsigned long long)));
@@ -920,7 +930,7 @@
         (void)hipFree(d_st);
         return AVX_OK;
     }
-    auto k = k_mst_attn_tail_mx<C, TR, MINW, false, NW>;
+    auto k = k_mst_attn_tail_mx<C, TR, MINW, false, NW, DWS>;
     AVX_HIP(ctx, hipFuncSetAttribute((const void*)k, hipFuncAttributeMaxDynamicSharedMemorySize, (int)lds));
     hipLaunchKernelGGL(k, dim3(blocks), dim3(64 * NW), lds, s, (const __half*)x, (const uint4*)wvpack, (const uint4*)mpack, (const uint4*)dw1,
                        (const uint4*)dw2, bias, (__half*)out, B, H, W, (unsigned long long*)nullptr, mst_tile_order());
@@ -1376,7 +1386,7 @@
 }
 
 static int ffn_fused_launch(avx_ctx* ctx, const void* x, const float* gamma, const float* beta, float eps, const void* w1pack, const void* taps_9xhid, const void* dwpack,
-                            const void* w2pack, void* out, int B, int H, int W, int C, void* stream);
+                            const void* w2pack, void* out, int B, int H, int W, int C, void* stream, bool sparse = false);
 
 extern "C" float avx_mst_gelu_prescale(void) { return kGeluPrescale; }
 
@@ -1411,8 +1421,15 @@
     return ffn_fused_launch(ctx, x, gamma, beta, eps, w1pack, nullptr, dwpack, w2pack, out, B, H, W, C, stream);
 }
 
+extern "C" int avx_mst_ffn_fused_sp(avx_ctx* ctx, const void* x, const float* gamma, const float* beta, float eps, const void* w1pack, const void* dwpack,
+                                    const void* w2pack, void* out, int B, int H, int W, int C, void* stream) {
+    if (!ctx) return AVX_ERR_INVALID;
+    AVX_REQUIRE(ctx, dwpack && (((uintptr_t)dwpack) & 15u) == 0, "avx_mst_ffn_fused_sp: dwpack NULL or not 16-byte aligned");
+    return ffn_fused_launch(ctx, x, gamma, beta, eps, w1pack, nullptr, dwpack, w2pack, out, B, H, W, C, stream, true);
+}
+
 static int ffn_fused_launch(avx_ctx* ctx, const void* x, const float* gamma, const float* beta, float eps, const void* w1pack, const void* taps_9xhid, const void* dwpack,
-                            const void* w2pack, void* out, int B, int H, int W, int C, void* stream) {
+                            const void* w2pack, void* out, int B, int H, int W, int C, void* stream, bool sparse) {
     AVX_REQUIRE(ctx, x && gamma && beta && w1pack && w2pack && out && B > 0 && H > 0 && W > 0, "avx_mst_ffn_fused: NULL pointer or empty tensor");
     AVX_REQUIRE(ctx, C == 32 || C == 64 || C == 128, "avx_mst_ffn_fused: C=%d (32, 64 or 128: 31-channel groups stored 32 wide)", C);
     AVX_REQUIRE(ctx, ((((uintptr_t)x | (uintptr_t)w1pack | (uintptr_t)w2pack | (uintptr_t)out | (uintptr_t)taps_9xhid)) & 15u) == 0,
@@ -1430,28 +1447,31 @@
     AVX_REQUIRE(ctx, total <= 0x7fffffffl, "avx_mst_ffn_fused: 2^31 tiles or more");
     const dim3 grid((unsigned)(total < cap ? total : cap));
     const int order = mst_tile_order();
-#define AVX_FFN1(CV, HP, MW, DW, NWV)                                                                                                            \
+#define AVX_FFN1S(CV, HP, MW, DW, NWV, SP)                                                                                                       \
     {                                                                                                                                            \
-        auto k = k_mst_ffn_fused<CV, HP, MW, DW, false, NWV>;                                                                                    \
+        auto k = k_mst_ffn_fused<CV, HP, MW, DW, false, NWV, SP>;                                                                                \
         AVX_HIP(ctx, hipFuncSetAttribute((const void*)k, hipFuncAttributeMaxDynamicSharedMemorySize, (int)lds));                                 \
         hipLaunchKernelGGL(k, grid, dim3(64 * NWV), lds, s, (const __half*)x, gamma, beta, eps, (const uint4*)w1pack, (const __half*)taps_9xhid, \
                            (const uint4*)w2pack, (__half*)out, B, H, W, (const uint4*)dwpack, (unsigned long long*)nullptr, order);              \
     }
-#define AVX_FFN(CV, HP, MW) { if (dwpack) AVX_FFN1(CV, HP, MW, true, 8) else AVX_FFN1(CV, HP, MW, false, 8) }
+#define AVX_FFN1(CV, HP, MW, DW, NWV) AVX_FFN1S(CV, HP, MW, DW, NWV, false)
+#define AVX_FFN(CV, HP, MW) { if (dwpack && sparse) AVX_FFN1S(CV, HP, MW, true, 8, true) else if (dwpack) AVX_FFN1(CV, HP, MW, true, 8) else AVX_FFN1(CV, HP, MW, false, 8) }
     if (dwpack && getenv("AVX_FFN_STAMPS") && ((C == 32 && small) || C == 64 || C == 128)) {
         unsigned long long* d_st = nullptr;
         const int nwv = nw16 ? 16 : 8;
         const size_t n = (size_t)grid.x * nwv * 8;
         AVX_HIP(ctx, hipMalloc((void**)&d_st, n * sizeof(unsigned long long)));
-#define AVX_FFN_ST(CV, HP, MW, NWV)                                                                                                              \
+#define AVX_FFN_ST1(CV, HP, MW, NWV, SP)                                                                                                         \
     {                                                                                                                                            \
-        auto k = k_mst_ffn_fused<CV, HP, MW, true, true, NWV>;                                                                                   \
+        auto k = k_mst_ffn_fused<CV, HP, MW, true, true, NWV, SP>;                                                                               \
         AVX_HIP(ctx, hipFuncSetAttribute((const void*)k, hipFuncAttributeMaxDynamicSharedMemorySize, (int)lds));                                 \
         hipLaunchKernelGGL(k, grid, dim3(64 * NWV), lds, s, (const __half*)x, gamma, beta, eps, (const uint4*)w1pack, (const __half*)taps_9xhid, \
                            (const uint4*)w2pack, (__half*)out, B, H, W, (const uint4*)dwpack, d_st, order);                                      \
     }
+#define AVX_FFN_ST(CV, HP, MW, NWV) { if (sparse) AVX_FFN_ST1(CV, HP, MW, NWV, true) else AVX_FFN_ST1(CV, HP, MW, NWV, false) }
         if (C == 32) AVX_FFN_ST(32, 64, 4, 8) else if (nw16) AVX_FFN_ST(64, 128, 1, 16) else if (C == 64) AVX_FFN_ST(64, 128, 2, 8) else AVX_FFN_ST(128, 64, 2, 8)
 #undef AVX_FFN_ST
+#undef AVX_FFN_ST1
         AVX_HIP(ctx, hipStreamSynchronize(s));
         unsigned long long* h_st = (unsigned long long*)malloc(n * sizeof(unsigned long long));
         AVX_HIP(ctx, hipMemcpy(h_st, d_st, n * sizeof(unsigned long long), hipMemcpyDeviceToHost));
@@ -1466,10 +1486,12 @@
         free(h_st);
         (void)hipFree(d_st);
     } else if (C == 32 && small) AVX_FFN(32, 64, 4) else if (C == 32) AVX_FFN(32, 128, 2)
+    else if (nw16 && sparse) AVX_FFN1S(64, 128, 1, true, 16, true)
     else if (nw16) AVX_FFN1(64, 128, 1, true, 16)
     else if (C == 64) AVX_FFN(64, 128, 2) else AVX_FFN(128, 64, 2)
 #undef AVX_FFN
 #undef AVX_FFN1
+#undef AVX_FFN1S
     AVX_HIP(ctx, hipGetLastError());
     return AVX_OK;
 }
@@ -1502,9 +1524,9 @@
     return launch_attn_tail<64, 2>(ctx, x, x, mpack16, taps1_9xc, taps2_9xc, bias, out, B, H, W, s, wvpack16);
 }
 
-extern "C" int avx_mst_attn_tail_mx(avx_ctx* ctx, const void* x, const void* wvpack16, const void* mpack_mx, const void* dw1pack, const void* dw2pack,
-                                    const float* bias, void* out, int B, int H, int W, int C, void* stream) {
-    if (!ctx) return AVX_ERR_INVALID;
+template <bool DWS>
+static int attn_tail_mx_launch(avx_ctx* ctx, const void* x, const void* wvpack16, const void* mpack_mx, const void* dw1pack, const void* dw2pack, const float* bias, void* out,
+                               int B, int H, int W, int C, void* stream) {
     AVX_REQUIRE(ctx, x && wvpack16 && mpack_mx && dw1pack && dw2pack && out && B > 0 && H > 0 && W > 0, "avx_mst_attn_tail_mx: NULL pointer or empty tensor");
     AVX_REQUIRE(ctx, C == 32 || C == 64 || C == 128, "avx_mst_attn_tail_mx: C=%d (32, 64 or 128)", C);
     AVX_REQUIRE(ctx, ((((uintptr_t)x | (uintptr_t)wvpack16 | (uintptr_t)mpack_mx | (uintptr_t)out | (uintptr_t)dw1pack | (uintptr_t)dw2pack)) & 15u) == 0,
@@ -1512,10 +1534,20 @@
     AVX_REQUIRE(ctx, x != out, "avx_mst_attn_tail_mx: tiles read their neighbours' rows of x: the output cannot be x");
     AVX_HIP(ctx, hipSetDevice(ctx->device));
     hipStream_t s = avx_pick_stream(ctx, stream);
-    if (C == 32) return launch_attn_tail_mx<32, 16, 4>(ctx, x, wvpack16, mpack_mx, dw1pack, dw2pack, bias, out, B, H, W, s);
-    if (C == 128) return launch_attn_tail_mx<128, 8, 2>(ctx, x, wvpack16, mpack_mx, dw1pack, dw2pack, bias, out, B, H, W, s);
-    if (getenv("AVX_MST_TAIL_NW") && atoi(getenv("AVX_MST_TAIL_NW")) == 16) return launch_attn_tail_mx<64, 16, 1, 16>(ctx, x, wvpack16, mpack_mx, dw1pack, dw2pack, bias, out, B, H, W, s);
-    return launch_attn_tail_mx<64, 16, 2>(ctx, x, wvpack16, mpack_mx, dw1pack, dw2pack, bias, out, B, H, W, s);
+    if (C == 32) return launch_attn_tail_mx<32, 16, 4, 8, DWS>(ctx, x, wvpack16, mpack_mx, dw1pack, dw2pack, bias, out, B, H, W, s);
+    if (C == 128) return launch_attn_tail_mx<128, 8, 2, 8, DWS>(ctx, x, wvpack16, mpack_mx, dw1pack, dw2pack, bias, out, B, H, W, s);
+    if (getenv("AVX_MST_TAIL_NW") && atoi(getenv("AVX_MST_TAIL_NW")) == 16) return launch_attn_tail_mx<64, 16, 1, 16, DWS>(ctx, x, wvpack16, mpack_mx, dw1pack, dw2pack, bias, out, B, H, W, s);
+    return launch_attn_tail_mx<64, 16, 2, 8, DWS>(ctx, x, wvpack16, mpack_mx, dw1pack, dw2pack, bias, out, B, H, W, s);
+}
+extern "C" int avx_mst_attn_tail_mx(avx_ctx* ctx, const void* x, const void* wvpack16, const void* mpack_mx, const void* dw1pack, const void* dw2pack,
+                                    const float* bias, void* out, int B, int H, int W, int C, void* stream) {
+    if (!ctx) return AVX_ERR_INVALID;
+    return attn_tail_mx_launch<false>(ctx, x, wvpack16, mpack_mx, dw1pack, dw2pack, bias, out, B, H, W, C, stream);
+}
+extern "C" int avx_mst_attn_tail_sp(avx_ctx* ctx, const void* x, const void* wvpack16, const void* mpack_mx, const void* dw1pack, const void* dw2pack,
+                                    const float* bias, void* out, int B, int H, int W, int C, void* stream) {
+    if (!ctx) return AVX_ERR_INVALID;
+    return attn_tail_mx_launch<true>(ctx, x, wvpack16, mpack_mx, dw1pack, dw2pack, bias, out, B, H, W, C, stream);
 }
 
 extern "C" int avx_mst_conv3x3_lds(avx_ctx* ctx, const void* x, const void* wpack16, const void* add, void* out, int B, int H, int W, int C, void* stream) {
diff --git a/animal-vision_amd/ml/mst_plus_plus.py b/animal-vision_amd/ml/mst_plus_plus.py
--- a/animal-vision_amd/ml/mst_plus_plus.py
+++ b/animal-vision_amd/ml/mst_plus_plus.py
@@ -112,6 +112,34 @@
     return out.contiguous()
 
 
+def pack_dw_smfmac(w: torch.Tensor) -> torch.Tensor:
+    ch = w.shape[0]
+    assert ch % 8 == 0 and tuple(w.shape[1:]) == (1, 3, 3)
+    dev = w.device
+    lane = torch.arange(64, device=dev)
+    m, qa = lane % 16, lane // 16
+    s_, c = m // 8, m % 8
+    w8 = w.reshape(ch // 8, 8, 3, 3)
+    out = torch.zeros((ch // 8, 3, 64, 8), dtype=w.dtype, device=dev)
+    out[:, 1] = pack_dw_mfma(w)[:, 2]
+    t = c % 4
+    idx = torch.full((64,), 0x4444, dtype=torch.int64, device=dev)
+    for hh in range(2):
+        r = 2 * (qa % 2) + hh
+        dy = r - s_
+        ok = (dy >= 0) & (dy <= 2)
+        vals = w8[:, c, dy.clamp(0, 2), qa // 2]
+        vals = torch.where(ok[None, :], vals, torch.zeros_like(vals))
+        e = 4 * hh + 2 * (c // 4) + (t == 3).long()
+        out[:, 0, lane, e] = vals
+        pair = torch.where(t == 3, 2 | (3 << 2), t | (3 << 2))
+        sh = 4 * (2 * hh + c // 4)
+        idx = (idx & ~(0xF << sh)) | (pair << sh)
+    lo = (((idx & 0xFFFF) ^ 0x8000) - 0x8000).to(torch.int16)
+    out.view(torch.int16)[:, 2, :, 0] = lo[None]
+    return out.contiguous()
+
+
 def fold_layernorm(w1_kn: torch.Tensor, gamma: torch.Tensor, beta: torch.Tensor, scale: float) -> torch.Tensor:
     w = w1_kn.float()
     out = w * gamma.float()[:, None]
@@ -143,6 +171,9 @@
         self._ffn = os.environ.get("AVX_MST_NO_FFN_FUSED", "") == ""
         self._gelu_pre = None
         self._dwmx = os.environ.get("AVX_MST_NO_DW_MFMA", "") == ""
+        self._dwsp = os.environ.get("AVX_MST_NO_DW_SPARSE", "") == ""
+        self.DW_SPARSE_FFN_C = (32, 64, 128)
+        self.DW_SPARSE_TAIL_C = (32, 64)
         self._specfuse = os.environ.get("AVX_MST_NO_SPEC_FUSE", "") == ""
         self.FFN_FUSED_C = tuple(int(v) for v in os.environ.get("AVX_MST_FFN_FUSED_C", "32,64,128").split(",") if v)
         self._ctx = {}
@@ -378,15 +409,16 @@
         return out
 
     def attn_tail_mx(self, x: torch.Tensor, wvpack16: torch.Tensor, mpack_mx: torch.Tensor, dw1: torch.Tensor, dw2: torch.Tensor, bias: torch.Tensor,
-                     out: torch.Tensor = None) -> torch.Tensor:
+                     out: torch.Tensor = None, sparse: bool = False) -> torch.Tensor:
         from .._lib import lib
 
         h, w, c = x.shape
         assert x.is_contiguous()
         out = torch.empty_like(x) if out is None else out
         ctx = self.ctx(x.device)
-        ctx._check(lib.avx_mst_attn_tail_mx(ctx._h, x.data_ptr(), wvpack16.data_ptr(), mpack_mx.data_ptr(), dw1.data_ptr(), dw2.data_ptr(), bias.data_ptr(),
-                                            out.data_ptr(), 1, h, w, c, torch.cuda.current_stream(x.device).cuda_stream))
+        fn = lib.avx_mst_attn_tail_sp if sparse else lib.avx_mst_attn_tail_mx
+        ctx._check(fn(ctx._h, x.data_ptr(), wvpack16.data_ptr(), mpack_mx.data_ptr(), dw1.data_ptr(), dw2.data_ptr(), bias.data_ptr(),
+                      out.data_ptr(), 1, h, w, c, torch.cuda.current_stream(x.device).cuda_stream))
         return out
 
     def attn_tail(self, v: torch.Tensor, x: torch.Tensor, mpack16: torch.Tensor, taps1: torch.Tensor, taps2: torch.Tensor, bias: torch.Tensor,
@@ -426,7 +458,7 @@
         return out
 
     def ffn_fused(self, x: torch.Tensor, gamma: torch.Tensor, beta: torch.Tensor, w1p: torch.Tensor, taps: torch.Tensor, w2p: torch.Tensor,
-                  eps: float = 1e-5, dwpack: torch.Tensor = None) -> torch.Tensor:
+                  eps: float = 1e-5, dwpack: torch.Tensor = None, sparse: bool = False) -> torch.Tensor:
         from .._lib import lib
 
         b, h, w, c = x.shape
@@ -435,8 +467,8 @@
         ctx = self.ctx(x.device)
         st = torch.cuda.current_stream(x.device).cuda_stream
         if dwpack is not None:
-            ctx._check(lib.avx_mst_ffn_fused_mx(ctx._h, x.data_ptr(), gamma.data_ptr(), beta.data_ptr(), eps, w1p.data_ptr(), dwpack.data_ptr(), w2p.data_ptr(),
-                                                out.data_ptr(), b, h, w, c, st))
+            fn = lib.avx_mst_ffn_fused_sp if sparse else lib.avx_mst_ffn_fused_mx
+            ctx._check(fn(ctx._h, x.data_ptr(), gamma.data_ptr(), beta.data_ptr(), eps, w1p.data_ptr(), dwpack.data_ptr(), w2p.data_ptr(), out.data_ptr(), b, h, w, c, st))
         else:
             ctx._check(lib.avx_mst_ffn_fused(ctx._h, x.data_ptr(), gamma.data_ptr(), beta.data_ptr(), eps, w1p.data_ptr(), taps.data_ptr(), w2p.data_ptr(),
                                              out.data_ptr(), b, h, w, c, st))
@@ -636,10 +668,12 @@
                 if tailx and _AVX._dwmx:
                     wv16 = self._prep(p + ".wv.frag16h", lambda: pack_fragments16(wqkv[:, 2 * c :].contiguous(), halfrow=True))
                     gs = _AVX.gelu_prescale()
-                    d1 = self._prep(k1 + f".dwmx/{gs}", lambda: pack_dw_mfma((self._w(k1, (0,)).float() / gs).to(x.dtype)))
-                    d2 = self._prep(k2 + f".dwmx*{gs}", lambda: pack_dw_mfma((self._w(k2, (0,)).float() * gs).to(x.dtype)))
+                    sp = _AVX._dwsp and c in _AVX.DW_SPARSE_TAIL_C
+                    pk, tag = (pack_dw_smfmac, ".dwsp") if sp else (pack_dw_mfma, ".dwmx")
+                    d1 = self._prep(k1 + f"{tag}/{gs}", lambda: pk((self._w(k1, (0,)).float() / gs).to(x.dtype)))
+                    d2 = self._prep(k2 + f"{tag}*{gs}", lambda: pk((self._w(k2, (0,)).float() * gs).to(x.dtype)))
                     for i in range(b):
-                        _AVX.attn_tail_mx(xc[i], wv16, _AVX.attn_pack_mx(gram[i], nq[i], nk[i], resc, wpt), d1, d2, bias32, out[i])
+                        _AVX.attn_tail_mx(xc[i], wv16, _AVX.attn_pack_mx(gram[i], nq[i], nk[i], resc, wpt), d1, d2, bias32, out[i], sparse=sp)
                     return out
                 if tailx:
                     wv16 = self._prep(p + ".wv.frag16", lambda: pack_fragments16(wqkv[:, 2 * c :].contiguous()))
@@ -707,6 +741,8 @@
                 gs = _AVX.gelu_prescale()
                 w1s = self._prep(p + f".w1.frag16.ln/{gs}", lambda: pack_fragments16(fold_layernorm(self._w(p + ".fn.net.0.weight", (0, 1)).reshape(4 * c, c).t(), g32, b32, gs).to(x.dtype)))
                 w2s = self._prep(p + f".w2.frag16*{gs}", lambda: pack_fragments16((w2.float() * gs).to(x.dtype).contiguous()))
+                if _AVX._dwsp and c in _AVX.DW_SPARSE_FFN_C:
+                    return _AVX.ffn_fused(x, g32, b32, w1s, None, w2s, dwpack=self._prep(key + ".dwsp", lambda: pack_dw_smfmac(self._w(key, (0,)))), sparse=True)
                 return _AVX.ffn_fused(x, g32, b32, w1s, None, w2s, dwpack=self._prep(key + ".dwmx", lambda: pack_dw_mfma(self._w(key, (0,)))))
             w1q = self._prep(p + ".w1.frag16", lambda: pack_fragments16(self._w(p + ".fn.net.0.weight", (0, 1)).reshape(4 * c, c).t().contiguous()))
             w2q = self._prep(p + ".w2.frag16", lambda: pack_fragments16(w2))
diff --git a/include/avx.h b/include/avx.h
--- a/include/avx.h
+++ b/include/avx.h
@@ -355,6 +355,8 @@
                         const float* bias, void* out, int B, int H, int W, int C, void* stream);
 int avx_mst_attn_tail_mx(avx_ctx* ctx, const void* x, const void* wvpack16, const void* mpack_mx, const void* dw1pack, const void* dw2pack,
                          const float* bias, void* out, int B, int H, int W, int C, void* stream);
+int avx_mst_attn_tail_sp(avx_ctx* ctx, const void* x, const void* wvpack16, const void* mpack_mx, const void* dw1pack, const void* dw2pack,
+                         const float* bias, void* out, int B, int H, int W, int C, void* stream);
 int avx_mst_attn_pack_mx(avx_ctx* ctx, const float* gram, const float* nq, const float* nk, const float* rescale, const float* wproj_t, int C, void* mpack,
                          void* stream);
 
@@ -366,6 +368,8 @@
                       const void* w2pack, void* out, int B, int H, int W, int C, void* stream);
 int avx_mst_ffn_fused_mx(avx_ctx* ctx, const void* x, const float* gamma, const float* beta, float eps, const void* w1pack, const void* dwpack,
                          const void* w2pack, void* out, int B, int H, int W, int C, void* stream);
+int avx_mst_ffn_fused_sp(avx_ctx* ctx, const void* x, const float* gamma, const float* beta, float eps, const void* w1pack, const void* dwpack,
+                         const void* w2pack, void* out, int B, int H, int W, int C, void* stream);
 float avx_mst_gelu_prescale(void);
 
 int avx_mst_tile_order(int frames, int ty, int tx, int nwg, int raster, long long* visit, int steps_cap, int* steps_out);
```
